# DredderGun/accbpg_and_fw

Measured on AMD Instinct MI355X. Metric: D-opt iters/sec (m=2048,n=32768), higher is better.
Workload: dtype f64; 1 GPU; D_opt_design(2048,32768) abpg_gain gamma=2 fp64, one independent instance per GPU; instances=1, instances_per_gpu=1, seeds=1..1, window=transient: iterations 5..161 from x0 = 1/n, linear_gram=False

## Files before the change

### accbpg_and_fw_amd/_lib.py

```python
from __future__ import annotations

import ctypes as C
import os

_HERE = os.path.dirname(os.path.abspath(__file__))
LIB_PATH = os.environ.get("ACCBPG_HIP_LIB") or os.path.join(_HERE, "lib", "libaccbpg_hip.so")

OK, ERR_ASSERT, ERR_NOT_PD, ERR_HIP, ERR_ARG = 0, 1, 2, 3, 4

_lib = None


class FwProbe(C.Structure):
    _fields_ = [("i", C.c_int64), ("j", C.c_int64), ("w_i", C.c_double), ("w_j", C.c_double),
                ("x_j", C.c_double), ("logdet_H", C.c_double), ("q_prev", C.c_double)]


class FwDivProbe(C.Structure):
    _fields_ = [("i", C.c_int64), ("w_i", C.c_double), ("x_i", C.c_double), ("sum_w", C.c_double),
                ("sum_w2", C.c_double), ("slope", C.c_double), ("div", C.c_double), ("min_x", C.c_double),
                ("sum_u2", C.c_double)]


class FwStep(C.Structure):
    _fields_ = [("i", C.c_int64), ("j", C.c_int64), ("w_i", C.c_double), ("w_j", C.c_double), ("x_j", C.c_double),
                ("q_prev", C.c_double), ("p", C.c_int64), ("xscale", C.c_double), ("xadd", C.c_double),
                ("hcoef", C.c_double), ("hdiv", C.c_double), ("kind", C.c_int32), ("status", C.c_int32)]


FW_RUN_MAX = 1024
FW_APPLIED, FW_STOPPED, FW_BAD_PIVOT, FW_NOT_RUN = 0, 1, 2, 3

_P = C.c_void_p
_SIGS = {
    "accbpg_abi_version": (C.c_int, []),
    "accbpg_last_error": (C.c_char_p, []),
    "accbpg_dopt_create": (C.c_int, [_P, C.c_int64, C.c_int64, C.c_int64, _P, C.POINTER(_P), C.c_int]),
    "accbpg_dopt_destroy": (C.c_int, [_P]),
    "accbpg_dopt_set_stream": (C.c_int, [_P, _P]),
    "accbpg_dopt_func_grad": (C.c_int, [_P, _P, C.c_int, C.POINTER(C.c_double), _P]),
    "accbpg_dopt_func_grad_begin": (C.c_int, [_P, _P, C.c_int, _P]),
    "accbpg_dopt_func_grad_end": (C.c_int, [_P, C.POINTER(C.c_double)]),
    "accbpg_dopt_eval_gap_ms": (C.c_int, [_P, _P, C.POINTER(C.c_double)]),
    "accbpg_dopt_value_reuse": (C.c_int, [_P, C.c_int]),
    "accbpg_dopt_value_reuse_stats": (C.c_int, [_P, C.POINTER(C.c_int64), C.POINTER(C.c_int64)]),
    "accbpg_dopt_value_peer": (C.c_int, [_P, _P]),
    "accbpg_dopt_gram": (C.c_int, [_P, _P, _P]),
    "accbpg_dopt_factor": (C.c_int, [_P, _P, C.POINTER(C.c_double)]),
    "accbpg_dopt_grad": (C.c_int, [_P, _P]),
    "accbpg_tri_pack": (C.c_int, [_P, C.c_int64, _P, _P]),
    "accbpg_tri_unpack": (C.c_int, [_P, C.c_int64, _P, _P]),
    "accbpg_vec_count_bad": (C.c_int, [_P, C.c_int64, _P, _P]),
    "accbpg_dopt_shard_bounds": (C.c_int, [C.c_int64, C.c_int, C.c_int, C.POINTER(C.c_int64), C.POINTER(C.c_int64)]),
    "accbpg_shard_unique_id": (C.c_int, [_P]),
    "accbpg_dopt_shard_create": (C.c_int, [_P, C.c_int64, C.c_int, C.c_int, _P, _P, C.POINTER(_P)]),
    "accbpg_dopt_shard_func_grad": (C.c_int, [_P, _P, C.c_int, C.POINTER(C.c_double), _P]),
    "accbpg_dopt_shard_destroy": (C.c_int, [_P]),
    "accbpg_debug_shard_pad": (C.c_int, [_P, C.c_int64]),
    "accbpg_dopt_gram_lincomb": (C.c_int, [_P, C.c_double, _P, C.c_double, _P, _P]),
    "accbpg_dopt_eval_gram": (C.c_int, [_P, _P, C.c_int, C.POINTER(C.c_double), _P]),
    "accbpg_dopt_batch_create": (C.c_int, [C.POINTER(_P), C.c_int, C.c_int64, C.c_int64, C.c_int64, _P, C.POINTER(_P)]),
    "accbpg_dopt_batch_destroy": (C.c_int, [_P]),
    "accbpg_dopt_batch_set_stream": (C.c_int, [_P, _P]),
    "accbpg_dopt_batch_size": (C.c_int, [_P]),
    "accbpg_dopt_batch_is_fused": (C.c_int, [_P]),
    "accbpg_dopt_batch_chunk": (C.c_int, [_P]),
    "accbpg_dopt_batch_instance": (_P, [_P, C.c_int]),
    "accbpg_dopt_batch_func_grad": (C.c_int, [_P, _P, C.c_int64, C.POINTER(C.c_int), C.c_int, C.POINTER(C.c_double), _P,
                                              C.c_int64, C.POINTER(C.c_int)]),
    "accbpg_dopt_batch_func_grad_begin": (C.c_int, [_P, _P, C.c_int64, C.POINTER(C.c_int), C.c_int, _P, C.c_int64]),
    "accbpg_dopt_batch_func_grad_end": (C.c_int, [_P, C.POINTER(C.c_double), C.POINTER(C.c_int)]),
    "accbpg_dopt_batch_burg_simplex_div_prox": (C.c_int, [_P, _P, _P, C.c_int64, C.POINTER(C.c_double), C.c_double, _P,
                                                          C.POINTER(C.c_int), C.POINTER(C.c_int), C.POINTER(C.c_int)]),
    "accbpg_dopt_batch_ls_terms": (C.c_int, [_P, _P, _P, _P, _P, _P, C.c_int64, C.POINTER(C.c_int), C.POINTER(C.c_double),
                                             C.POINTER(C.c_int)]),
    "accbpg_dopt_batch_axpby": (C.c_int, [_P, C.POINTER(C.c_double), _P, C.POINTER(C.c_double), _P, C.c_int64,
                                          C.POINTER(C.c_int), _P]),
    "accbpg_vec_workspace_doubles": (C.c_int64, [C.c_int64]),
    "accbpg_burg_simplex_div_prox": (C.c_int, [_P, _P, C.c_double, C.c_double, C.c_int64, _P, _P,
                                               C.POINTER(C.c_int), _P]),
    "accbpg_burg_divergence": (C.c_int, [_P, _P, C.c_int64, C.POINTER(C.c_double), _P, _P]),
    "accbpg_ls_terms": (C.c_int, [_P, _P, _P, _P, _P, C.c_int64, C.POINTER(C.c_double), _P, _P]),
    "accbpg_vec_axpby": (C.c_int, [C.c_double, _P, C.c_double, _P, C.c_int64, _P, _P]),
    "accbpg_vec_dot_diff": (C.c_int, [_P, _P, _P, C.c_int64, C.POINTER(C.c_double), _P, _P]),
    "accbpg_vec_min_sum": (C.c_int, [_P, C.c_int64, C.POINTER(C.c_double), _P, _P]),
    "accbpg_vec_div_scalar": (C.c_int, [_P, C.c_double, C.c_int64, _P, _P]),
    "accbpg_vec_vertex": (C.c_int, [C.c_int64, C.c_double, C.c_double, C.c_int64, _P, _P]),
    "accbpg_vec_argminmax": (C.c_int, [_P, C.c_int64, C.POINTER(C.c_int64), C.POINTER(C.c_double), _P, _P]),
    "accbpg_dopt_vt_times": (C.c_int, [_P, _P, _P]),
    "accbpg_dopt_get_column": (C.c_int, [_P, C.c_int64, _P]),
    "accbpg_dopt_kyinit": (C.c_int, [_P, _P, C.POINTER(C.c_int64), _P]),
    "accbpg_fw_init": (C.c_int, [_P, _P, C.POINTER(C.c_double)]),
    "accbpg_fw_probe_step": (C.c_int, [_P, C.c_int, C.c_int, C.POINTER(FwProbe)]),
    "accbpg_fw_logdet_flush": (C.c_int, [_P, C.POINTER(C.c_double)]),
    "accbpg_fw_logdet_ring": (C.c_int, [_P, C.c_int, C.c_int]),
    "accbpg_fw_logdet_pending": (C.c_int, [_P]),
    "accbpg_fw_update": (C.c_int, [_P, C.c_int64, C.c_double, C.c_double, C.c_double, C.c_double]),
    "accbpg_fw_get_state": (C.c_int, [_P, _P, _P, _P]),
    "accbpg_fw_div_probe_step": (C.c_int, [_P, C.c_double, C.c_double, C.POINTER(FwDivProbe)]),
    "accbpg_fw_div_apply": (C.c_int, [_P, C.c_int64, C.c_double, C.c_double, C.c_double, C.c_double, C.c_double]),
    "accbpg_fw_logdet_snapshot": (C.c_int, [_P, C.POINTER(C.c_double)]),
    "accbpg_fw_run": (C.c_int, [_P, C.c_int, C.c_double, C.c_int, C.POINTER(FwStep), C.POINTER(C.c_int)]),
    "accbpg_dopt_batch_fw_init": (C.c_int, [_P, _P, C.c_int64, C.POINTER(C.c_int), C.POINTER(C.c_double),
                                            C.POINTER(C.c_int)]),
    "accbpg_dopt_batch_fw_probe": (C.c_int, [_P, C.c_int, C.POINTER(C.c_int), C.POINTER(FwProbe)]),
    "accbpg_dopt_batch_fw_update": (C.c_int, [_P, C.POINTER(C.c_int), C.POINTER(C.c_int64), C.POINTER(C.c_double),
                                              C.POINTER(C.c_double), C.POINTER(C.c_double), C.POINTER(C.c_double)]),
    "accbpg_dopt_batch_fw_run": (C.c_int, [_P, C.c_int, C.POINTER(C.c_double), C.c_int, C.POINTER(C.c_int),
                                           C.POINTER(FwStep), C.POINTER(C.c_int)]),
    "accbpg_dopt_batch_kyinit": (C.c_int, [_P, _P, C.POINTER(C.c_int64), _P]),
    "accbpg_poisson_create": (C.c_int, [_P, C.c_int64, C.c_int64, C.c_int64, _P, _P, C.POINTER(_P)]),
    "accbpg_poisson_destroy": (C.c_int, [_P]),
    "accbpg_poisson_set_stream": (C.c_int, [_P, _P]),
    "accbpg_poisson_func_grad": (C.c_int, [_P, _P, C.c_int, C.POINTER(C.c_double), _P]),
    "accbpg_poisson_get_ax": (C.c_int, [_P, _P]),
    "accbpg_kldiv_create": (C.c_int, [_P, C.c_int64, C.c_int64, C.c_int64, _P, _P, C.POINTER(_P)]),
    "accbpg_kldiv_destroy": (C.c_int, [_P]),
    "accbpg_kldiv_set_stream": (C.c_int, [_P, _P]),
    "accbpg_kldiv_func_grad": (C.c_int, [_P, _P, C.c_int, C.POINTER(C.c_double), _P]),
    "accbpg_kldiv_get_ax": (C.c_int, [_P, _P]),
    "accbpg_shannon_div_prox": (C.c_int, [C.c_int, _P, _P, C.c_double, C.c_double, C.c_int64, _P, _P, _P]),
    "accbpg_shannon_ls_terms": (C.c_int, [_P, _P, _P, _P, _P, C.c_int64, C.c_double, C.POINTER(C.c_double), _P, _P]),
    "accbpg_shannon_divergence": (C.c_int, [_P, _P, C.c_int64, C.c_double, C.POINTER(C.c_double), _P, _P]),
    "accbpg_symnmf_create": (C.c_int, [_P, C.c_int64, C.c_int64, C.c_int64, C.c_double, _P, C.POINTER(_P)]),
    "accbpg_symnmf_destroy": (C.c_int, [_P]),
    "accbpg_symnmf_set_stream": (C.c_int, [_P, _P]),
    "accbpg_symnmf_func_grad": (C.c_int, [_P, _P, C.c_int, C.POINTER(C.c_double), _P]),
    "accbpg_symnmf_plan": (C.c_int, [_P, C.POINTER(C.c_int64)]),
    "accbpg_quartic_prox_stage": (C.c_int, [_P, _P, C.c_double, C.c_double, C.c_int, C.c_double, C.c_int64, _P,
                                            C.POINTER(C.c_double), _P, _P]),
    "accbpg_quartic_ls_terms": (C.c_int, [_P, _P, _P, _P, _P, C.c_int64, C.POINTER(C.c_double), _P, _P]),
    "accbpg_lmo_l2_ball": (C.c_int, [_P, C.c_int, _P, C.c_double, C.c_double, C.c_double, C.c_int64, _P,
                                     C.POINTER(C.c_double), _P, _P]),
    "accbpg_lmo_linf_ball": (C.c_int, [_P, C.c_int, _P, C.c_double, C.c_double, C.c_int64, _P, _P]),
    "accbpg_burg_reg_div_prox": (C.c_int, [C.c_int, _P, _P, C.c_double, C.c_double, C.c_int64, _P, _P]),
    "accbpg_vec_dot": (C.c_int, [_P, _P, C.c_int64, C.POINTER(C.c_double), _P, _P]),
    "accbpg_combine_ls_terms": (C.c_int, [C.c_int, C.c_double, _P, C.c_double, _P, C.c_double, _P, _P, C.c_int64, _P,
                                          C.POINTER(C.c_double), _P, _P]),
    "accbpg_burg_simplex_prox_acc": (C.c_int, [_P, C.c_double, _P, C.c_double, C.c_double, C.c_int64, _P, _P, _P,
                                               C.POINTER(C.c_int), _P]),
    "accbpg_lmo_l2_ball_pos": (C.c_int, [_P, _P, C.c_double, C.c_double, C.c_int64, _P, C.POINTER(C.c_double), _P, _P]),
    "accbpg_dopt_profile_enable": (C.c_int, [_P, C.c_int]),
    "accbpg_dopt_profile_read": (C.c_int, [_P, C.c_int, C.POINTER(C.c_double), C.POINTER(C.c_int64)]),
    "accbpg_dopt_profile_reset": (C.c_int, [_P]),
    "accbpg_debug_pipe_probe": (C.c_int, [C.c_int, C.c_int, C.POINTER(C.c_double), _P]),
    "accbpg_mfma_f64_peak": (C.c_int, [C.c_int, C.POINTER(C.c_double), _P]),
    "accbpg_dopt_factor_in_small_launches": (C.c_int, [_P, C.c_int]),
    "accbpg_debug_chol_variant": (C.c_int, [_P, C.c_int]),
    "accbpg_debug_plan_flags": (C.c_int, [C.c_int]),
    "accbpg_debug_gemm_loop": (C.c_int, [C.c_int]),
    "accbpg_debug_prox_variant": (C.c_int, [C.c_int]),
    "accbpg_debug_prox_state": (C.c_int, [C.POINTER(C.c_int)]),
    "accbpg_debug_chol_trace": (C.c_int, [_P, _P, C.c_int, C.POINTER(C.c_int64)]),
    "accbpg_debug_gram_variant": (C.c_int, [_P, _P, C.c_int, C.c_int, C.POINTER(C.c_double)]),
    "accbpg_debug_grad_variant": (C.c_int, [_P, _P, C.c_int, C.c_int, C.POINTER(C.c_double)]),
    "accbpg_test_gemm": (C.c_int, [_P, C.c_int64, _P, C.c_int64, _P, C.c_int64, C.c_int64, C.c_int64,
                                   C.c_int64, C.c_int, C.c_double, C.c_double, C.c_int, _P]),
}

EXPORTS = tuple(sorted(_SIGS))


def load():
    global _lib
    if _lib is not None:
        return _lib
    if not os.path.exists(LIB_PATH):
        raise ImportError(
            "accbpg_and_fw_amd: %s is missing -- build it with "
            "`make -C accbpg_and_fw_amd/csrc` or `python -c 'import __graft_entry__ as g; g.build()'`. "
            "There is no CPU fallback." % LIB_PATH)
    lib = C.CDLL(LIB_PATH)
    for name, (res, args) in _SIGS.items():
        fn = getattr(lib, name)
        fn.restype = res
        fn.argtypes = args
    _lib = lib
    return lib


def last_error():
    msg = load().accbpg_last_error()
    return msg.decode() if msg else ""


def check(rc, what, assert_msg=None):
    if rc == OK:
        return
    if rc == ERR_ASSERT:
        raise AssertionError(assert_msg or last_error() or what)
    if rc == ERR_NOT_PD:
        raise ValueError("HXHT is singular or not positive definite")
    if rc == ERR_ARG:
        raise ValueError("%s: bad argument (%s)" % (what, last_error()))
    raise RuntimeError("%s: HIP error: %s" % (what, last_error()))
```

### accbpg_and_fw_amd/algorithms.py

```python
from __future__ import annotations

import math
import time

import numpy as np
import torch

from .functions import (BurgEntropy, BurgEntropySimplex, ShannonEntropy, SquaredL2Norm, SumOf2nd4thPowers,
                        combine_ls_terms, from_dev, ls_terms, shannon_ls_terms, to_dev, vec_axpby, vec_div_scalar,
                        vec_dot_diff)
from .utils import get_random_float


def _divergences(h, g, x, y, z, z_prev):
    if isinstance(h, BurgEntropy):
        return ls_terms(g, x, y, z, z_prev)
    if isinstance(h, ShannonEntropy):
        return shannon_ls_terms(g, x, y, z, z_prev, h.delta)
    if isinstance(h, SumOf2nd4thPowers):
        return h.ls_terms(g, x, y, z, z_prev)
    lin = vec_dot_diff(g, x, y) if g is not None else 0.0
    return lin, h.divergence(x, y), (h.divergence(z, z_prev) if z is not None else 0.0)


def _lin(f):
    return bool(getattr(f, "_lin", False))


def _value(f, x, combo=None):
    return f.func_grad_combo(x, combo, 0) if _lin(f) else f(x)


def _value_begin(f, x, combo):
    if (not _lin(f)) and getattr(f, "_overlap", False) and not getattr(f, "_prof", False) \
            and isinstance(x, torch.Tensor) and x.is_cuda:
        if getattr(f, "_memo_on", False):
            hit = f._memo_get(x)
            if hit is not None:
                return ("value", hit)
        return ("ticket", f.value_async(x))
    return ("value", _value(f, x, combo))


def _can_speculate(f, x, checkdiv):
    return (not checkdiv) and (not _lin(f)) and getattr(f, "_spec", False) and getattr(f, "_overlap", False) \
        and not getattr(f, "_prof", False) and hasattr(f, "grad_async") and isinstance(x, torch.Tensor) and x.is_cuda


def _value_end(f, pending):
    kind, payload = pending
    return f.value_wait(payload) if kind == "ticket" else payload


def _stamp(f, pending, t_start, t_known):
    if pending[0] == "ticket":
        return time.time() - t_start - f.value_lead_seconds()
    return t_known - t_start


def _drain(gen):
    while True:
        try:
            next(gen)
        except StopIteration as stop:
            return stop.value


def BPG(f, h, L, x0, maxitrs, epsilon=1e-14, linesearch=True, ls_ratio=1.2,
        verbose=True, verbskip=1):
    return _drain(BPG_steps(f, h, L, x0, maxitrs, epsilon, linesearch, ls_ratio, verbose, verbskip))


def BPG_steps(f, h, L, x0, maxitrs, epsilon=1e-14, linesearch=True, ls_ratio=1.2,
              verbose=True, verbskip=1):
    if verbose:
        print("\nBPG_LS method for min_{x in C} F(x) = f(x) + Psi(x)")
        print("     k      F(x)         Lk       time")

    t_start = time.time()
    F = np.zeros(maxitrs)
    Ls = np.ones(maxitrs) * L
    T = np.zeros(maxitrs)

    x, as_numpy = to_dev(x0)
    x = x.clone()
    k = -1
    for k in range(maxitrs):
        fx, g = f.func_grad(x)
        F[k] = fx + h.extra_Psi(x)
        T[k] = time.time() - t_start

        if linesearch:
            L = L / ls_ratio
            trial = h.div_prox_map(x, g, L)
            while True:
                lin, dist, _ = _divergences(h, g, trial, x, None, None)
                if not (f(trial) > fx + lin + L * dist):
                    break
                L = L * ls_ratio
                trial = h.div_prox_map(x, g, L)
            x = trial
        else:
            x = h.div_prox_map(x, g, L)

        Ls[k] = L
        if verbose and k % verbskip == 0:
            print("{0:6d}  {1:10.3e}  {2:10.3e}  {3:6.1f}".format(k, F[k], L, T[k]))

        if k > 0 and abs(F[k] - F[k - 1]) < epsilon:
            break
        yield k

    return from_dev(x, as_numpy), F[0:k + 1], Ls[0:k + 1], T[0:k + 1]


def solve_theta(theta, gamma, gainratio=1):
    ckg = theta ** gamma / gainratio
    cta = theta
    eps = 1e-6 * theta
    phi = cta ** gamma - ckg * (1 - cta)
    while abs(phi) > eps:
        drv = gamma * cta ** (gamma - 1) + ckg
        cta = cta - phi / drv
        phi = cta ** gamma - ckg * (1 - cta)
    return cta


def ABPG(f, h, L, x0, gamma, maxitrs, epsilon=1e-14, theta_eq=False,
         restart=False, restart_rule='g', verbose=True, verbskip=1):
    return _drain(ABPG_steps(f, h, L, x0, gamma, maxitrs, epsilon, theta_eq, restart, restart_rule,
                             verbose, verbskip))


def ABPG_steps(f, h, L, x0, gamma, maxitrs, epsilon=1e-14, theta_eq=False,
               restart=False, restart_rule='g', verbose=True, verbskip=1):
    if verbose:
        print("\nABPG method for minimize_{x in C} F(x) = f(x) + Psi(x)")
        print("     k      F(x)       theta" +
              "        TSG       D(x+,y)     D(z+,z)     time")

    t_start = time.time()
    F = np.zeros(maxitrs)
    G = np.zeros(maxitrs)
    T = np.zeros(maxitrs)

    x, as_numpy = to_dev(x0)
    x = x.clone()
    z = x.clone()
    theta = 1.0
    kk = 0
    xcombo = None
    k = -1
    for k in range(maxitrs):
        pending = _value_begin(f, x, xcombo)
        t_known = time.time()

        z_prev, x_prev = z, x
        if theta_eq and kk > 0:
            theta = solve_theta(theta, gamma)
        else:
            theta = gamma / (kk + gamma)

        y = vec_axpby(1 - theta, x, theta, z_prev)
        if _lin(f):
            g = f.func_grad_combo(y, (1 - theta, x_prev, theta, z_prev), 1)
        else:
            g = f.gradient(y)
        F[k] = _value_end(f, pending) + h.extra_Psi(x_prev)
        T[k] = _stamp(f, pending, t_start, t_known)
        z = h.div_prox_map(z_prev, g, theta ** (gamma - 1) * L)
        x = vec_axpby(1 - theta, x, theta, z)
        if _lin(f):
            f.ensure_gram(z)
            xcombo = (1 - theta, x_prev, theta, z)

        _, dxy, dzz = _divergences(h, None, x, y, z, z_prev)
        Gdr = dxy / dzz / theta ** gamma

        G[k] = Gdr
        if verbose and k % verbskip == 0:
            print("{0:6d}  {1:10.3e}  {2:10.3e}  {3:10.3e}  {4:10.3e}  {5:10.3e}  {6:6.1f}".format(
                k, F[k], theta, Gdr, dxy, dzz, T[k]))

        kk += 1
        if restart and k > 0:
            if (restart_rule == 'f' and F[k] > F[k - 1]) or \
               (restart_rule == 'g' and vec_dot_diff(g, x, x_prev) > 0):
                theta = 1.0
                kk = 0
                z = x

        if dzz < epsilon:
            break
        yield k

    return from_dev(x, as_numpy), F[0:k + 1], G[0:k + 1], T[0:k + 1]


def ABPG_gain(f, h, L, x0, gamma, maxitrs, epsilon=1e-14, G0=1,
              ls_inc=1.2, ls_dec=1.2, theta_eq=True, checkdiv=False,
              restart=False, restart_rule='g', verbose=True, verbskip=1):
    return _drain(ABPG_gain_steps(f, h, L, x0, gamma, maxitrs, epsilon, G0, ls_inc, ls_dec, theta_eq,
                                  checkdiv, restart, restart_rule, verbose, verbskip))


def ABPG_gain_steps(f, h, L, x0, gamma, maxitrs, epsilon=1e-14, G0=1,
                    ls_inc=1.2, ls_dec=1.2, theta_eq=True, checkdiv=False,
                    restart=False, restart_rule='g', verbose=True, verbskip=1):
    if verbose:
        print("\nABPG_gain method for min_{x in C} F(x) = f(x) + Psi(x)")
        print("     k      F(x)       theta         Gk" +
              "         TSG       D(x+,y)     D(z+,z)      Gavg       time")

    t_start = time.time()
    F = np.zeros(maxitrs)
    Gain = np.ones(maxitrs) * G0
    Gdiv = np.zeros(maxitrs)
    Gavg = np.zeros(maxitrs)
    T = np.zeros(maxitrs)

    x, as_numpy = to_dev(x0)
    x = x.clone()
    z = x.clone()
    G = G0
    sumlogG = gamma * np.log(G)
    theta = 1.0
    kk = 0
    Gdr = 0.0
    xcombo = None
    retries_before = 0
    k = -1
    for k in range(maxitrs):
        pending = _value_begin(f, x, xcombo)
        t_known = time.time()

        z_prev, x_prev = z, x
        G_prev, theta_prev = G, theta
        G = G / ls_dec

        def theta_for(Gt):
            if kk == 0:
                return theta
            if theta_eq:
                return solve_theta(theta_prev, gamma, Gt / G_prev)
            alpha = Gt / G_prev
            return theta_prev * ((1 + alpha * (gamma - 1)) / (gamma * alpha + theta_prev))

        ahead = _can_speculate(f, x_prev, checkdiv)
        started = None
        failed = 0
        searching = True
        while searching:
            theta = theta_for(G)
            if started is not None:
                y, ticket = started
                started = None
                fy, g = f.grad_wait(ticket)
            else:
                y = vec_axpby(1 - theta, x_prev, theta, z_prev)
                if _lin(f):
                    fy, g = f.func_grad_combo(y, (1 - theta, x_prev, theta, z_prev), 2)
                else:
                    fy, g = f.func_grad(y)
            if pending is not None:
                F[k] = _value_end(f, pending) + h.extra_Psi(x_prev)
                T[k] = _stamp(f, pending, t_start, t_known)
                pending = None
            z = h.div_prox_map(z_prev, g, theta ** (gamma - 1) * G * L)
            x = vec_axpby(1 - theta, x_prev, theta, z)
            if _lin(f):
                f.ensure_gram(z)
                xcombo = (1 - theta, x_prev, theta, z)

            lin, dxy, dzz = _divergences(h, g, x, y, z, z_prev)
            if dzz < epsilon:
                break

            Gdr = dxy / dzz / theta ** gamma

            if checkdiv:
                searching = (Gdr > G)
            else:
                if ahead and failed < retries_before:
                    theta_next = theta_for(G * ls_inc)
                    y_next = vec_axpby(1 - theta_next, x_prev, theta_next, z_prev)
                    started = (y_next, f.grad_async(y_next))
                searching = (_value(f, x, xcombo) > fy + lin + theta ** gamma * G * L * dzz)

            if searching:
                G = G * ls_inc
                failed += 1
            elif started is not None:
                f.grad_drop(started[1])
                started = None
        retries_before = failed

        Gain[k] = G
        Gdiv[k] = Gdr
        sumlogG += np.log(G)
        Gavg[k] = np.exp(sumlogG / (gamma + k))
        if verbose and k % verbskip == 0:
            print("{0:6d}  {1:10.3e}  {2:10.3e}  {3:10.3e}  {4:10.3e}  {5:10.3e}  {6:10.3e}  {7:10.3e}  {8:6.1f}".format(
                k, F[k], theta, G, Gdr, dxy, dzz, Gavg[k], T[k]))

        kk += 1
        if restart:
            if (restart_rule == 'f' and F[k] > F[k - 1]) or \
               (restart_rule == 'g' and vec_dot_diff(g, x, x_prev) > 0):
                theta = 1.0
                kk = 0
                z = x

        if dzz < epsilon:
            break
        yield k

    return (from_dev(x, as_numpy), F[0:k + 1], Gain[0:k + 1], Gdiv[0:k + 1],
            Gavg[0:k + 1], T[0:k + 1])


def ABPG_expo(f, h, L, x0, gamma0, maxitrs, epsilon=1e-14, delta=0.2,
              theta_eq=True, checkdiv=False, Gmargin=10, restart=False,
              restart_rule='g', verbose=True, verbskip=1):
    return _drain(ABPG_expo_steps(f, h, L, x0, gamma0, maxitrs, epsilon, delta, theta_eq, checkdiv, Gmargin,
                                  restart, restart_rule, verbose, verbskip))


def ABPG_expo_steps(f, h, L, x0, gamma0, maxitrs, epsilon=1e-14, delta=0.2,
                    theta_eq=True, checkdiv=False, Gmargin=10, restart=False,
                    restart_rule='g', verbose=True, verbskip=1):
    if verbose:
        print("\nABPG_expo method for min_{x in C} F(x) = f(x) + Psi(x)")
        print("     k      F(x)       theta       gamma" +
              "        TSG       D(x+,y)     D(z+,z)     time")

    t_start = time.time()
    F = np.zeros(maxitrs)
    G = np.zeros(maxitrs)
    Gamma = np.ones(maxitrs) * gamma0
    T = np.zeros(maxitrs)

    gamma = gamma0
    x, as_numpy = to_dev(x0)
    x = x.clone()
    z = x.clone()
    theta = 1.0
    kk = 0
    k = -1
    for k in range(maxitrs):
        F[k] = f(x) + h.extra_Psi(x)
        T[k] = time.time() - t_start

        z_prev, x_prev = z, x
        if theta_eq and kk > 0:
            theta = solve_theta(theta, gamma)
        else:
            theta = gamma / (kk + gamma)

        y = vec_axpby(1 - theta, x_prev, theta, z_prev)
        fy, g = f.func_grad(y)

        trying = True
        while trying:
            z = h.div_prox_map(z_prev, g, theta ** (gamma - 1) * L)
            x = vec_axpby(1 - theta, x_prev, theta, z)
            lin, dxy, dzz = _divergences(h, g, x, y, z, z_prev)
            Gdr = dxy / dzz / theta ** gamma

            if checkdiv:
                trying = (dxy > Gmargin * (theta ** gamma) * dzz)
            else:
                trying = (f(x) > fy + lin + theta ** gamma * L * dzz)

            if trying and gamma > 1:
                gamma = max(gamma - delta, 1)
            else:
                trying = False

        G[k] = Gdr
        Gamma[k] = gamma
        if verbose and k % verbskip == 0:
            print("{0:6d}  {1:10.3e}  {2:10.3e}  {3:10.3e}  {4:10.3e}  {5:10.3e}  {6:10.3e}  {7:6.1f}".format(
                k, F[k], theta, gamma, Gdr, dxy, dzz, T[k]))

        kk += 1
        if restart:
            if (restart_rule == 'f' and F[k] > F[k - 1]) or \
               (restart_rule == 'g' and vec_dot_diff(g, x, x_prev) > 0):
                theta = 1.0
                kk = 0
                z = x

        if dzz < epsilon:
            break
        yield k

    return from_dev(x, as_numpy), F[0:k + 1], Gamma[0:k + 1], G[0:k + 1], T[0:k + 1]


def ABDA(f, h, L, x0, gamma, maxitrs, epsilon=1e-14, theta_eq=True,
         verbose=True, verbskip=1):
    return _drain(ABDA_steps(f, h, L, x0, gamma, maxitrs, epsilon, theta_eq, verbose, verbskip))


def ABDA_steps(f, h, L, x0, gamma, maxitrs, epsilon=1e-14, theta_eq=True,
               verbose=True, verbskip=1):
    if verbose:
        print("\nABDA method for min_{x in C} F(x) = f(x) + Psi(x)")
        print("     k      F(x)       theta" +
              "        TSG       D(x+,y)     D(z+,z)     time")

    t_start = time.time()
    F = np.zeros(maxitrs)
    G = np.zeros(maxitrs)
    T = np.zeros(maxitrs)

    x, as_numpy = to_dev(x0)
    x = x.clone()
    z = x.clone()
    theta = 1.0
    kk = 0
    gavg = torch.zeros_like(x)
    csum = 0
    k = -1
    for k in range(maxitrs):
        F[k] = f(x) + h.extra_Psi(x)
        T[k] = time.time() - t_start

        z_prev, x_prev = z, x
        if theta_eq and kk > 0:
            theta = solve_theta(theta, gamma)
        else:
            theta = gamma / (kk + gamma)

        y = vec_axpby(1 - theta, x_prev, theta, z_prev)
        g = f.gradient(y)
        wgt = theta ** (1 - gamma)
        gavg = vec_axpby(1.0, gavg, wgt, g)
        csum = csum + wgt
        z = h.prox_map(vec_div_scalar(gavg, csum), L / csum)
        x = vec_axpby(1 - theta, x_prev, theta, z)

        _, dxy, dzz = _divergences(h, None, x, y, z, z_prev)
        Gdr = dxy / dzz / theta ** gamma

        G[k] = Gdr
        if verbose and k % verbskip == 0:
            print("{0:6d}  {1:10.3e}  {2:10.3e}  {3:10.3e}  {4:10.3e}  {5:10.3e}  {6:6.1f}".format(
                k, F[k], theta, Gdr, dxy, dzz, T[k]))

        kk += 1
        if dzz < epsilon:
            break
        yield k

    return from_dev(x, as_numpy), F[0:k + 1], G[0:k + 1], T[0:k + 1]


FUSED_INEXACT = True


def _fusable(h):
    return FUSED_INEXACT and isinstance(h, (BurgEntropy, SquaredL2Norm))


def _combine(h, a, u, b, v, c, g=None, x=None):
    if _fusable(h):
        return combine_ls_terms(h, a, u, b, v, c, g, x)
    w = vec_axpby(a, u, b, v)
    if c != 1:
        w = vec_div_scalar(w, c)
    if x is None:
        return w, None, None
    lin, dist, _ = _divergences(h, g, w, x, None, None)
    return w, lin, dist


def _doubled(L):
    L = L * 2
    if L is None or not math.isfinite(L):
        raise ValueError("L cannot be None or infinity")
    return L


def AIBM(f, h, L, x0, gamma, maxitrs, epsilon=1e-14, verbose=True, noise=0, verbskip=1):
    return _drain(AIBM_steps(f, h, L, x0, gamma, maxitrs, epsilon, verbose, noise, verbskip))


def AIBM_steps(f, h, L, x0, gamma, maxitrs, epsilon=1e-14, verbose=True, noise=0, verbskip=1):
    if verbose:
        print("\nAIBM method for min_{x in C} F(x) = f(x) + Psi(x)")
        print("     k      F(x)       L       time")

    t_start = time.time()
    F = np.zeros(maxitrs)
    G = np.zeros(maxitrs)
    T = np.zeros(maxitrs)
    p = 2

    x0d, as_numpy = to_dev(x0)
    x = z = h.prox_map(torch.zeros(x0d.shape[0], dtype=torch.float64, device=x0d.device), 1)

    delta = get_random_float(noise)
    fx, g = f.func_grad(x, flag=2)
    y = h.prox_map(g, 1)
    lin, dist, _ = _divergences(h, g, y, x, None, None)
    fy = f(y)
    while True:
        alpha = 1 / L
        if fy <= fx + lin + L * dist + epsilon + delta:
            break
        L = _doubled(L)

    B = A = alpha
    xi_grad = vec_axpby(alpha, g, 0.0, g)

    F[0] = fx + h.extra_Psi(x)
    G[0] = L
    T[0] = time.time() - t_start

    acc_prox = FUSED_INEXACT and isinstance(h, BurgEntropySimplex)
    k = 0
    for k in range(1, maxitrs):
        L /= 2
        delta = get_random_float(noise)
        while True:
            alpha = (1 / L) * (1 + k / (2 * p)) ** ((p - 1) * (gamma - 1))
            B = (L * alpha ** gamma) ** (1 / (gamma - 1))
            x = vec_axpby(alpha / B, z, 1 - alpha / B, y)
            fx, grad_x = f.func_grad(x, flag=2)
            if acc_prox:
                xi_grad, z_k = h.prox_map_acc(xi_grad, alpha, grad_x)
            else:
                xi_grad = vec_axpby(1.0, xi_grad, alpha, grad_x)
                z_k = h.prox_map(xi_grad, 1)
            w, lin, dist = _combine(h, alpha / B, z_k, 1 - alpha / B, y, 1, grad_x, x)
            if f(w) <= fx + lin + L * dist + delta:
                break
            xi_grad = vec_axpby(1.0, xi_grad, -alpha, grad_x)
            L = _doubled(L)

        F[k] = fx + h.extra_Psi(x)
        T[k] = time.time() - t_start

        A += alpha
        y = vec_axpby(B / A, w, 1 - B / A, y)
        z = z_k

        if verbose and k % verbskip == 0:
            print("{0:6d}  {1:10.3e}  {2:10.3e}  {3:6.1f}".format(k, F[k], L, T[k]))

        if abs(F[k] - F[k - 1]) < 1e-9:
            break
        yield k

    return from_dev(x, as_numpy), F[0:k + 1], G[0:k + 1], T[0:k + 1]


def AdaptFGM(f, h, L, x0, maxitrs, epsilon=1e-14, verbose=True, noise=0, verbskip=1):
    return _drain(AdaptFGM_steps(f, h, L, x0, maxitrs, epsilon, verbose, noise, verbskip))


def AdaptFGM_steps(f, h, L, x0, maxitrs, epsilon=1e-14, verbose=True, noise=0, verbskip=1):
    if verbose:
        print("\nAdaptFGM method for min_{x in C} F(x) = f(x) + Psi(x)")
        print("     k      F(x)       L       time")

    t_start = time.time()
    F = np.zeros(maxitrs)
    G = np.zeros(maxitrs)
    T = np.zeros(maxitrs)

    x0d, as_numpy = to_dev(x0)
    x_k = u_k = torch.ones(x0d.shape, dtype=torch.float64, device=x0d.device)
    A_k = 0

    fxk, g = f.func_grad(x_k, flag=2)

    F[0] = fxk + h.extra_Psi(x_k)
    G[0] = L
    T[0] = time.time() - t_start

    k = 0
    for k in range(1, maxitrs):
        L /= 2
        delta = get_random_float(noise)
        while True:
            alpha = (1 + math.sqrt(1 + 4 * L * A_k)) / (2 * L)
            A = L * alpha ** 2
            y, _, _ = _combine(h, alpha, u_k, A_k, x_k, A)
# ... 89 lines not shown
```

### accbpg_and_fw_amd/csrc/capi.hip

```cpp
#include <stdarg.h>
#include <string.h>
#include <stdlib.h>
#include <algorithm>

#include "internal.h"
#include "reduce.hpp"

namespace accbpg {

static thread_local char g_err[512] = "";

void set_last_error(const char* fmt, ...) {
    va_list ap;
    va_start(ap, fmt);
    vsnprintf(g_err, sizeof(g_err), fmt, ap);
    va_end(ap);
}

void note_tiles_fallback(const char* where) {
    static bool said = false;
    if (said) return;
    said = true;
    fprintf(stderr, "libaccbpg_hip: %s: the one-launch Cholesky abandoned a wait (another process on this GPU, or fewer "
                    "workgroups resident than the occupancy query promised); this handle factors with one launch per block "
                    "column from now on\n", where);
}

static int read_status(accbpg_dopt* h) {
    ACC_HIP(hipMemcpyAsync(h->hpin, h->dscal, sizeof(double) * STATUS_DOUBLES, hipMemcpyDeviceToHost, h->stream));
    ACC_HIP(hipStreamSynchronize(h->stream));
    return ACCBPG_OK;
}

}

using namespace accbpg;

extern "C" int accbpg_abi_version(void) { return 3; }
extern "C" const char* accbpg_last_error(void) { return g_err; }

namespace accbpg {
int dopt_init(accbpg_dopt* h) {
    const int64_t m = h->m, n = h->n;
    ACC_HIP(hipGetDevice(&h->device));
    hipDeviceProp_t prop;
    ACC_HIP(hipGetDeviceProperties(&prop, h->device));
    h->num_cu = prop.multiProcessorCount;
    h->vec_ok = ((reinterpret_cast<uintptr_t>(h->V) & 15) == 0) && ((h->ldv & 1) == 0);
    h->big = (m >= 768) || (h->force_big && h->vec_ok && m >= 256 && (m % 256 == 0) && (n % 128 == 0));
    const size_t mm = sizeof(double) * (size_t)m * (size_t)m;
    ACC_HIP(hipMalloc(&h->Lbuf, mm));
    ACC_HIP(hipMalloc(&h->Wbuf, mm));
    ACC_HIP(hipMalloc(&h->Tbuf, mm));
    ACC_HIP(hipMemset(h->Lbuf, 0, mm));
    ACC_HIP(hipMemset(h->Wbuf, 0, mm));
    ACC_HIP(hipMemset(h->Tbuf, 0, mm));
    if (h->dscal_ext) {
        h->dscal = h->dscal_ext;
    } else {
        ACC_HIP(hipMalloc(&h->dscal, sizeof(double) * 24));
        ACC_HIP(hipMemset(h->dscal, 0, sizeof(double) * 24));
    }
    h->dflag = reinterpret_cast<int*>(h->dscal + 16);
    ACC_HIP(hipHostMalloc(&h->hpin, sizeof(double) * 32, hipHostMallocDefault));
    const int64_t vws = std::max<int64_t>(vec_ws_doubles(n), 64 * n);
    ACC_HIP(hipMalloc(&h->vws, sizeof(double) * (size_t)vws));
    ACC_HIP(hipEventCreate(&h->ev_done));
    return build_plans(h);
}
}

extern "C" int accbpg_dopt_create(const double* V_dev, int64_t m, int64_t n, int64_t ldv, void* stream,
                                  accbpg_dopt** out, int is_shard) {
    if (!V_dev || !out || m <= 0 || n <= 0 || ldv < n) {
        set_last_error("accbpg_dopt_create: bad arguments (m=%lld n=%lld ldv=%lld)", (long long)m, (long long)n,
                       (long long)ldv);
        return ACCBPG_ERR_ARG;
    }
    if (!is_shard && !(m < n)) {
        set_last_error("DOptimalObj: need m < n");
        return ACCBPG_ERR_ASSERT;
    }
    accbpg_dopt* h = new accbpg_dopt();
    h->V = V_dev; h->m = m; h->n = n; h->ldv = ldv; h->stream = (hipStream_t)stream;
    const int rc = dopt_init(h);
    if (rc != ACCBPG_OK) {
        accbpg_dopt_destroy(h);
        return rc;
    }
    *out = h;
    return ACCBPG_OK;
}

extern "C" int accbpg_dopt_destroy(accbpg_dopt* h) {
    if (!h) return ACCBPG_OK;
    for (accbpg_dopt* l : h->val_linked) l->val_peer = nullptr;
    if (h->val_peer) {
        auto& lk = h->val_peer->val_linked;
        lk.erase(std::remove(lk.begin(), lk.end(), h), lk.end());
    }
    hipFree(h->val_copy);
    hipFree(h->Vblk);
    hipFree(h->Lbuf); hipFree(h->Wbuf); hipFree(h->Tbuf); hipFree(h->slabs); hipFree(h->tiles); hipFree(h->wg_ranges); hipFree(h->gram_cstart); hipFree(h->gram_contrib);
    if (!h->dscal_ext) hipFree(h->dscal);
    hipFree(h->vws); hipFree(h->xbuf); hipFree(h->ops); hipFree(h->chol_op); hipFree(h->red); hipFree(h->Pbuf);
    hipFree(h->fw_x); hipFree(h->fw_w); hipFree(h->fw_H); hipFree(h->fw_hv);
    hipFree(h->chol_jobs); hipFree(h->chol_ready); hipFree(h->chol_aux); hipFree(h->chol_hand); hipFree(h->Gbuf);
    hipFree(h->fw_run);
    if (h->fw_steps_pin) hipHostFree(h->fw_steps_pin);
    hipFree(h->fw_div_ws);
    if (h->fw_div_pin) hipHostFree(h->fw_div_pin);
    if (h->hpin) hipHostFree(h->hpin);
    if (h->ev_done) hipEventDestroy(h->ev_done);
    for (auto& sl : h->fw_ring) {
        if (sl.stream) hipStreamSynchronize(sl.stream);
        if (sl.aux) accbpg_dopt_destroy(sl.aux);
        if (sl.stream) hipStreamDestroy(sl.stream);
        if (sl.ev_snap) hipEventDestroy(sl.ev_snap);
    }
    for (auto& p : h->prof)
        for (auto e : p.ev) hipEventDestroy(e);
    delete h;
    return ACCBPG_OK;
}

extern "C" int accbpg_dopt_set_stream(accbpg_dopt* h, void* stream) {
    if (!h) return ACCBPG_ERR_ARG;
    h->stream = (hipStream_t)stream;
    return ACCBPG_OK;
}

extern "C" int accbpg_dopt_gram(accbpg_dopt* h, const double* x_dev, double* gram_dev) {
    if (!h || !x_dev || !gram_dev) return ACCBPG_ERR_ARG;
    return launch_gram(h, x_dev, gram_dev);
}

extern "C" int accbpg_dopt_factor(accbpg_dopt* h, const double* gram_dev, double* f_host) {
    if (!h || !gram_dev) return ACCBPG_ERR_ARG;
    ACC_TRY(launch_cholesky(h, h->Lbuf, nullptr, nullptr, gram_dev));
    ACC_TRY(read_status(h));
    const int* fl = reinterpret_cast<const int*>(h->hpin + 16);
    if (fl[FLAG_ABORT]) {
        if (gram_dev == h->Lbuf) {
            set_last_error("accbpg_dopt_factor: in-place factorisation was abandoned; pass the Gram matrix in a buffer of its own");
            return ACCBPG_ERR_HIP;
        }
        h->chol_tiles_off = true;
        note_tiles_fallback("accbpg_dopt_factor");
        return accbpg_dopt_factor(h, gram_dev, f_host);
    }
    if (fl[FLAG_NOT_PD]) {
        set_last_error("HXHT is singular or not positive definite");
        return ACCBPG_ERR_NOT_PD;
    }
    if (f_host) *f_host = -h->hpin[0];
    return ACCBPG_OK;
}

extern "C" int accbpg_dopt_grad(accbpg_dopt* h, double* g_dev) {
    if (!h || !g_dev) return ACCBPG_ERR_ARG;
    ACC_TRY(launch_trtri(h));
    ACC_TRY(launch_colnorm(h, h->Wbuf, g_dev, -1.0));
    return ACCBPG_OK;
}

namespace accbpg {
__global__ __launch_bounds__(256) void value_compare_kernel(const unsigned long long* __restrict__ a,
                                                           const unsigned long long* __restrict__ b, int64_t n, int stamp,
                                                           int* __restrict__ word) {
    const int64_t stride = (int64_t)gridDim.x * 256;
    bool differ = false;
    for (int64_t i = (int64_t)blockIdx.x * 256 + threadIdx.x; i < n; i += stride) differ |= a[i] != b[i];
    if (differ) *word = stamp;
}

static void value_forget(accbpg_dopt* h) {
    h->val_valid = false;
    h->val_pending = false;
}

static int value_alloc(accbpg_dopt* h) {
    if (h->val_copy) return ACCBPG_OK;
    double* p = nullptr;
    ACC_HIP(hipMalloc(&p, sizeof(double) * ((size_t)h->n + 2)));
    if (hipMemsetAsync(p + h->n, 0, sizeof(double) * 2, h->stream) != hipSuccess) {
        hipFree(p);
        set_last_error("accbpg_dopt_func_grad: could not clear the compare word");
        return ACCBPG_ERR_HIP;
    }
    h->val_copy = p;
    return ACCBPG_OK;
}

static int value_matches(accbpg_dopt* h, const accbpg_dopt* rec, const double* x, bool* same) {
    ACC_TRY(value_alloc(h));
    int* word = reinterpret_cast<int*>(h->val_copy + h->n);
    int* pin = reinterpret_cast<int*>(h->hpin + 28);
    const int stamp = h->val_gen = h->val_gen % 1000000000 + 1;
    const int64_t nb = std::min<int64_t>((h->n + 255) / 256, 1024);
    value_compare_kernel<<<(unsigned)nb, 256, 0, h->stream>>>(reinterpret_cast<const unsigned long long*>(x),
                                                             reinterpret_cast<const unsigned long long*>(rec->val_copy),
                                                             h->n, stamp, word);
    ACC_HIP(hipGetLastError());
    ACC_HIP(hipMemcpyAsync(pin, word, sizeof(int), hipMemcpyDeviceToHost, h->stream));
    ACC_HIP(hipStreamSynchronize(h->stream));
    ++h->val_compares;
    *same = *pin != stamp;
    return ACCBPG_OK;
}

static int func_grad_begin(accbpg_dopt* h, const double* x_dev, int flag, double* g_dev, bool lookup) {
    h->last_x = x_dev; h->last_flag = flag; h->last_g = g_dev;
    h->val_pending = false;
    h->val_hit = false;
    const bool record = flag == 0 && h->val_reuse;
    if (record) {
        accbpg_dopt* const recs[2] = {h, h->val_peer};
        for (int r = 0; lookup && r < 2; ++r) {
            const accbpg_dopt* rec = recs[r];
            if (!rec || !rec->val_valid || rec->val_x != x_dev) continue;
            bool same = false;
            ACC_TRY(value_matches(h, rec, x_dev, &same));
            if (!same) continue;
            h->val_hit = true;
            h->val_answer = rec->val_f;
            ++h->val_answered;
            ACC_HIP(hipEventRecord(h->ev_done, h->stream));
            return ACCBPG_OK;
        }
        h->val_valid = false;
    }
    double* gram = chol_tiles_usable(h) ? h->Gbuf : h->Lbuf;
    ACC_TRY(launch_gram(h, x_dev, gram));
    if (record) ACC_TRY(value_alloc(h));
    ACC_TRY(launch_cholesky(h, h->Lbuf, flag != 0 ? h->Wbuf : nullptr, x_dev, gram, record ? h->val_copy : nullptr));
    if (flag != 0) {
        ACC_TRY(launch_trtri(h));
        ACC_TRY(launch_colnorm(h, h->Wbuf, g_dev, -1.0));
    }
    h->val_pending = record;
    ACC_HIP(hipMemcpyAsync(h->hpin, h->dscal, sizeof(double) * STATUS_DOUBLES, hipMemcpyDeviceToHost, h->stream));
    ACC_HIP(hipEventRecord(h->ev_done, h->stream));
    return ACCBPG_OK;
}

static int func_grad_end(accbpg_dopt* h, double* f_host) {
    if (h->val_hit) {
        h->val_hit = false;
        ACC_HIP(hipEventSynchronize(h->ev_done));
        if (f_host) *f_host = h->val_answer;
        return ACCBPG_OK;
    }
    ACC_HIP(hipStreamSynchronize(h->stream));
    const int* fl = reinterpret_cast<const int*>(h->hpin + 16);
    if (fl[FLAG_ABORT] && !h->chol_tiles_off) {
        h->chol_tiles_off = true;
        note_tiles_fallback("accbpg_dopt_func_grad");
        ACC_TRY(func_grad_begin(h, h->last_x, h->last_flag, h->last_g, false));
        return func_grad_end(h, f_host);
    }
    if (fl[FLAG_NEG_X]) {
        set_last_error("DOptimalObj: x needs to be nonnegative");
        return ACCBPG_ERR_ASSERT;
    }
    if (fl[FLAG_NOT_PD]) {
        set_last_error("HXHT is singular or not positive definite");
        return ACCBPG_ERR_NOT_PD;
    }
    if (h->val_pending) {
        h->val_pending = false;
        h->val_x = h->last_x;
        h->val_f = -h->hpin[0];
        h->val_valid = true;
    }
    if (f_host) *f_host = -h->hpin[0];
    return ACCBPG_OK;
}
}

extern "C" int accbpg_dopt_func_grad_begin(accbpg_dopt* h, const double* x_dev, int flag, double* g_dev) {
    if (!h || !x_dev || flag < 0 || flag > 2) return ACCBPG_ERR_ARG;
    if (flag != 0 && !g_dev) return ACCBPG_ERR_ARG;
    const int rc = func_grad_begin(h, x_dev, flag, g_dev, true);
    if (rc != ACCBPG_OK) {
        value_forget(h);
        h->val_hit = false;
    }
    return rc;
}

extern "C" int accbpg_dopt_eval_gap_ms(accbpg_dopt* first, accbpg_dopt* second, double* ms_host) {
    if (!first || !second || !ms_host) return ACCBPG_ERR_ARG;
    float ms = 0.f;
    const hipError_t e = hipEventElapsedTime(&ms, first->ev_done, second->ev_done);
    if (e != hipSuccess) {
        (void)hipGetLastError();
        float back = 0.f;
        if (hipEventElapsedTime(&back, second->ev_done, first->ev_done) != hipSuccess) {
            (void)hipGetLastError();
            set_last_error("accbpg_dopt_eval_gap_ms: no completed evaluation on one of the handles");
            return ACCBPG_ERR_ARG;
        }
        ms = -back;
    }
    *ms_host = (double)ms;
    return ACCBPG_OK;
}

extern "C" int accbpg_dopt_func_grad_end(accbpg_dopt* h, double* f_host) {
    if (!h) return ACCBPG_ERR_ARG;
    const int rc = func_grad_end(h, f_host);
    if (rc != ACCBPG_OK) value_forget(h);
    return rc;
}

extern "C" int accbpg_dopt_func_grad(accbpg_dopt* h, const double* x_dev, int flag, double* f_host, double* g_dev) {
    ACC_TRY(accbpg_dopt_func_grad_begin(h, x_dev, flag, g_dev));
    return accbpg_dopt_func_grad_end(h, f_host);
}

extern "C" int accbpg_dopt_value_reuse(accbpg_dopt* h, int on) {
    if (!h) return ACCBPG_ERR_ARG;
    h->val_reuse = on != 0;
    value_forget(h);
    return ACCBPG_OK;
}

extern "C" int accbpg_dopt_value_reuse_stats(accbpg_dopt* h, int64_t* compares_host, int64_t* answered_host) {
    if (!h) return ACCBPG_ERR_ARG;
    if (compares_host) *compares_host = h->val_compares;
    if (answered_host) *answered_host = h->val_answered;
    return ACCBPG_OK;
}

extern "C" int accbpg_dopt_value_peer(accbpg_dopt* h, accbpg_dopt* peer) {
    if (!h || peer == h) return ACCBPG_ERR_ARG;
    if (peer && (peer->V != h->V || peer->m != h->m || peer->n != h->n || peer->ldv != h->ldv)) {
        set_last_error("accbpg_dopt_value_peer: the two handles are not over the same matrix");
        return ACCBPG_ERR_ARG;
    }
    if (h->val_peer) {
        auto& lk = h->val_peer->val_linked;
        lk.erase(std::remove(lk.begin(), lk.end(), h), lk.end());
    }
    h->val_peer = peer;
    if (peer) peer->val_linked.push_back(h);
    return ACCBPG_OK;
}

namespace accbpg {
__global__ void lincomb_kernel(double a, const double* __restrict__ G1, double b, const double* __restrict__ G2,
                               int64_t total, double* __restrict__ out) {
    const int64_t stride = (int64_t)gridDim.x * blockDim.x * 2;
    for (int64_t e = 2 * ((int64_t)blockIdx.x * blockDim.x + threadIdx.x); e < total; e += stride) {
        if (e + 1 < total) {
            const double2 u = *reinterpret_cast<const double2*>(G1 + e);
            const double2 v = *reinterpret_cast<const double2*>(G2 + e);
            double2 r;
            r.x = a * u.x + b * v.x;
            r.y = a * u.y + b * v.y;
            *reinterpret_cast<double2*>(out + e) = r;
        } else {
            out[e] = a * G1[e] + b * G2[e];
        }
    }
}
}

namespace accbpg {
__global__ __launch_bounds__(256) void tri_pack_kernel(const double* __restrict__ G, int64_t m, double* __restrict__ packed,
                                                      int unpack, double* __restrict__ Gout) {
    const int64_t r = blockIdx.x;
    const int64_t base = r * (r + 1) / 2;
    for (int64_t c = threadIdx.x; c <= r; c += 256) {
        if (unpack) Gout[r * m + c] = packed[base + c];
        else packed[base + c] = G[r * m + c];
    }
}
__global__ __launch_bounds__(1024) void count_bad_kernel(const double* __restrict__ x, int64_t n, double* __restrict__ count) {
    __shared__ int sh[16];
    int c = 0;
    for (int64_t i = threadIdx.x; i < n; i += 1024) c += !(x[i] >= 0.0);
    c = wave_sum(c);
    if ((threadIdx.x & 63) == 0) sh[threadIdx.x >> 6] = c;
    __syncthreads();
    if (threadIdx.x == 0) {
        int t = 0;
        for (int i = 0; i < 16; ++i) t += sh[i];
        count[0] = (double)t;
    }
}
}

extern "C" int accbpg_tri_pack(const double* G_dev, int64_t m, double* packed_dev, void* stream) {
    if (!G_dev || !packed_dev || m <= 0) return ACCBPG_ERR_ARG;
    tri_pack_kernel<<<(unsigned)m, 256, 0, (hipStream_t)stream>>>(G_dev, m, packed_dev, 0, nullptr);
    ACC_HIP(hipGetLastError());
    return ACCBPG_OK;
}

extern "C" int accbpg_tri_unpack(const double* packed_dev, int64_t m, double* G_dev, void* stream) {
    if (!G_dev || !packed_dev || m <= 0) return ACCBPG_ERR_ARG;
    tri_pack_kernel<<<(unsigned)m, 256, 0, (hipStream_t)stream>>>(nullptr, m, const_cast<double*>(packed_dev), 1, G_dev);
    ACC_HIP(hipGetLastError());
    return ACCBPG_OK;
}

extern "C" int accbpg_vec_count_bad(const double* x_dev, int64_t n, double* count_dev, void* stream) {
    if (!x_dev || !count_dev || n <= 0) return ACCBPG_ERR_ARG;
    count_bad_kernel<<<1, 1024, 0, (hipStream_t)stream>>>(x_dev, n, count_dev);
    ACC_HIP(hipGetLastError());
    return ACCBPG_OK;
}

extern "C" int accbpg_dopt_gram_lincomb(accbpg_dopt* h, double a, const double* G1_dev, double b,
                                        const double* G2_dev, double* out_dev) {
    if (!h || !G1_dev || !G2_dev || !out_dev) return ACCBPG_ERR_ARG;
    const int64_t total = h->m * h->m;
    lincomb_kernel<<<2048, 256, 0, h->stream>>>(a, G1_dev, b, G2_dev, total, out_dev);
    ACC_HIP(hipGetLastError());
    return ACCBPG_OK;
}

extern "C" int accbpg_dopt_eval_gram(accbpg_dopt* h, const double* gram_dev, int flag, double* f_host, double* g_dev) {
    if (!h || !gram_dev || flag < 0 || flag > 2) return ACCBPG_ERR_ARG;
    if (flag != 0 && !g_dev) return ACCBPG_ERR_ARG;
    ACC_TRY(launch_cholesky(h, h->Lbuf, flag != 0 ? h->Wbuf : nullptr, nullptr, gram_dev));
    if (flag != 0) {
        ACC_TRY(launch_trtri(h));
        ACC_TRY(launch_colnorm(h, h->Wbuf, g_dev, -1.0));
    }
    ACC_TRY(read_status(h));
    const int* fl = reinterpret_cast<const int*>(h->hpin + 16);
    if (fl[FLAG_ABORT]) {
        if (gram_dev == h->Lbuf) {
            set_last_error("accbpg_dopt_eval_gram: in-place factorisation was abandoned; pass the Gram matrix in a buffer of its own");
            return ACCBPG_ERR_HIP;
        }
        h->chol_tiles_off = true;
        note_tiles_fallback("accbpg_dopt_eval_gram");
        return accbpg_dopt_eval_gram(h, gram_dev, flag, f_host, g_dev);
    }
    if (fl[FLAG_NOT_PD]) {
        set_last_error("HXHT is singular or not positive definite");
        return ACCBPG_ERR_NOT_PD;
    }
    if (f_host) *f_host = -h->hpin[0];
    return ACCBPG_OK;
}

extern "C" int accbpg_dopt_profile_enable(accbpg_dopt* h, int enable) {
    if (!h) return ACCBPG_ERR_ARG;
    h->prof_on = enable != 0;
    return ACCBPG_OK;
}

extern "C" int accbpg_dopt_profile_reset(accbpg_dopt* h) {
    if (!h) return ACCBPG_ERR_ARG;
    ACC_HIP(hipStreamSynchronize(h->stream));
    for (auto& p : h->prof) { p.used = 0; p.total_ms = 0.0; p.launches = 0; }
    return ACCBPG_OK;
}

extern "C" int accbpg_dopt_profile_read(accbpg_dopt* h, int which, double* total_ms_host, int64_t* launches_host) {
    if (!h || which < 0 || which >= PROF_COUNT) return ACCBPG_ERR_ARG;
    ACC_HIP(hipStreamSynchronize(h->stream));
    ProfSlot& p = h->prof[which];
    double tot = 0.0;
    for (size_t i = 0; i + 1 < p.used; i += 2) {
        float ms = 0.f;
        ACC_HIP(hipEventElapsedTime(&ms, p.ev[i], p.ev[i + 1]));
        tot += ms;
    }
    p.total_ms = tot;
    if (total_ms_host) *total_ms_host = tot;
    if (launches_host) *launches_host = p.launches;
    return ACCBPG_OK;
}

extern "C" int accbpg_mfma_f64_peak(int iters, double* tflops_host, void* stream) {
    if (!tflops_host || iters <= 0) return ACCBPG_ERR_ARG;
    return mfma_peak(iters, tflops_host, (hipStream_t)stream);
}

extern "C" int accbpg_debug_pipe_probe(int iters, int mode, double* ms_host, void* stream) {
    if (!ms_host || iters <= 0) return ACCBPG_ERR_ARG;
    return pipe_probe(iters, mode, ms_host, (hipStream_t)stream);
}

extern "C" int accbpg_test_gemm(const double* A_dev, int64_t lda, const double* B_dev, int64_t ldb, double* C_dev,
                                int64_t ldc, int64_t M, int64_t N, int64_t K, int b_kmajor, double alpha,
                                double beta, int config, void* stream) {
    if (!A_dev || !B_dev || !C_dev || M <= 0 || N <= 0 || K <= 0) return ACCBPG_ERR_ARG;
    return launch_test_gemm(A_dev, lda, B_dev, ldb, C_dev, ldc, M, N, K, b_kmajor, alpha, beta, config,
                            (hipStream_t)stream);
}

extern "C" int accbpg_dopt_factor_in_small_launches(accbpg_dopt* h, int on) {
    if (!h || on < 0 || on > 2) return ACCBPG_ERR_ARG;
    const int64_t T = (h->m + NB - 1) / NB;
    value_forget(h);
    h->chol_tiles_off = on == 1 || (on == 2 && T * (T + 1) / 2 >= h->num_cu);
    return ACCBPG_OK;
}

extern "C" int accbpg_debug_plan_flags(int flags) {
    set_plan_flags(flags);
    return ACCBPG_OK;
}

extern "C" int accbpg_debug_gemm_loop(int variant) {
    return set_gemm_loop(variant);
}

extern "C" int accbpg_debug_chol_variant(accbpg_dopt* h, int bits) {
    if (!h) return ACCBPG_ERR_ARG;
    value_forget(h);
    h->chol_dbg = bits & 63;
    h->chol_tiles_off = (bits & 64) != 0;
    if (bits & 2048) h->chol_tiles_off = true;
    h->chol_stall_test = (bits & 128) ? 1 : 0;
    h->chol_spin_limit = (bits & 128) ? 200000 : 20000000;
    h->kern_variant = (bits >> 30) & 3;
    if (bits & 256) h->use_glds = false;
    if (bits & 512) h->use_glds = true;
    if (bits & 2048) {
        h->chol_two_level_T = (bits >> 12) & 0xfff;
        if ((bits >> 24) & 0x3f) h->chol_nk = (bits >> 24) & 0x3f;
    }
    return ACCBPG_OK;
}

extern "C" int accbpg_debug_chol_trace(accbpg_dopt* h, const double* gram_dev, int with_inverse, int64_t* stamps_host) {
    if (!h || !gram_dev || !stamps_host) return ACCBPG_ERR_ARG;
    if (!chol_tiles_usable(h)) {
        set_last_error("accbpg_debug_chol_trace: the one-launch Cholesky is not in use for this handle");
        return ACCBPG_ERR_ARG;
    }
    const int T = (int)((h->m + NB - 1) / NB);
    const size_t bytes = sizeof(long long) * (size_t)T * 32;
    if (!h->chol_trace) ACC_HIP(hipMalloc(&h->chol_trace, bytes));
    ACC_HIP(hipMemsetAsync(h->chol_trace, 0, bytes, h->stream));
    int rc = launch_cholesky(h, h->Lbuf, with_inverse ? h->Wbuf : nullptr, nullptr, gram_dev);
    if (rc == ACCBPG_OK) {
        hipError_t e = hipMemcpyAsync(stamps_host, h->chol_trace, bytes, hipMemcpyDeviceToHost, h->stream);
        if (e == hipSuccess) e = hipStreamSynchronize(h->stream);
        if (e != hipSuccess) rc = ACCBPG_ERR_HIP;
    }
    hipFree(h->chol_trace);
    h->chol_trace = nullptr;
    return rc;
}

extern "C" int accbpg_debug_gram_variant(accbpg_dopt* h, const double* x_dev, int variant, int iters, double* ms_host) {
    if (!h || !x_dev || !ms_host || iters <= 0) return ACCBPG_ERR_ARG;
    value_forget(h);
    return debug_gram_variant(h, x_dev, variant, iters, ms_host);
}

extern "C" int accbpg_debug_grad_variant(accbpg_dopt* h, double* g_dev, int variant, int iters, double* ms_host) {
    if (!h || !g_dev || !ms_host || iters <= 0) return ACCBPG_ERR_ARG;
    value_forget(h);
    return debug_grad_variant(h, g_dev, variant, iters, ms_host);
}
```

### accbpg_and_fw_amd/csrc/dopt_kernels.hip

```cpp
#include <atomic>
#include <mutex>
#include <unordered_map>
#include <type_traits>

#include "internal.h"
#include "mfma_tile.hpp"

namespace accbpg {

struct GramSeg {
    int64_t row0, col0, kb, ke;
    bool dual, whole;
};
constexpr int GRAM_RMAX = 4;
template <class T>
__device__ __forceinline__ GramSeg gram_segment(const TileRC* __restrict__ tiles, int64_t kiters, int64_t it,
                                                int64_t it1) {
    const int e = (int)(it / kiters);
    const int64_t off = it - (int64_t)e * kiters;
    const TileRC tr = tiles[e];
    GramSeg g;
    if (tr.d1 < 0) {
        g.row0 = (int64_t)tr.rb * T::BM; g.col0 = (int64_t)tr.cb * T::BN;
        g.kb = off; g.ke = min(kiters, off + (it1 - it));
// ... 2255 lines not shown
                    it += ue - off;
                    ++seg;
                }
            }
            nslot = std::max(nslot, seg);
        }
        h->gram_nslot = nslot;
        std::vector<int32_t> cstart(cl.size() + 1, 0), contrib;
        for (size_t i = 0; i < cl.size(); ++i) {
            std::sort(cl[i].begin(), cl[i].end(), [](const Contrib& a, const Contrib& b) { return a.kb < b.kb; });
            for (const Contrib& c : cl[i]) { contrib.push_back(c.w); contrib.push_back(c.slot); }
            cstart[i + 1] = (int32_t)(contrib.size() / 2);
        }
        if (contrib.empty()) contrib.push_back(0);
        ACC_HIP(hipMalloc(&h->wg_ranges, sizeof(int64_t) * ranges.size()));
        ACC_HIP(hipMemcpy(h->wg_ranges, ranges.data(), sizeof(int64_t) * ranges.size(), hipMemcpyHostToDevice));
        ACC_HIP(hipMalloc(&h->gram_cstart, sizeof(int32_t) * cstart.size()));
        ACC_HIP(hipMemcpy(h->gram_cstart, cstart.data(), sizeof(int32_t) * cstart.size(), hipMemcpyHostToDevice));
        ACC_HIP(hipMalloc(&h->gram_contrib, sizeof(int32_t) * contrib.size()));
        ACC_HIP(hipMemcpy(h->gram_contrib, contrib.data(), sizeof(int32_t) * contrib.size(), hipMemcpyHostToDevice));
    }
    ACC_HIP(hipMalloc(&h->slabs, sizeof(double) * (size_t)grid * h->gram_nslot * BM * BN));

    const int T = (int)((m + NB - 1) / NB);
    h->ops_host.clear();
    h->merge_stages.clear();
    std::vector<RedOp> reds;
    constexpr int64_t KP = 256, KSPLIT_MIN = 512;
    ACC_HIP(hipMalloc(&h->Pbuf, sizeof(double) * (size_t)m * m));
    for (int span = 1; span < T; span *= 2) {
        std::vector<GemmOp> first, second;
        for (int g = 0; g + span < T; g += 2 * span) {
            const int64_t r1 = (int64_t)g * NB;
            const int64_t s1 = (int64_t)span * NB;
            const int64_t r2 = r1 + s1;
            const int64_t s2 = std::min<int64_t>((int64_t)span * NB, m - r2);
            GemmOp a{};
            a.A = h->Lbuf + r2 * m + r1; a.lda = m;
            a.B = h->Wbuf + r1 * m + r1; a.ldb = m;
            a.C = h->Tbuf + r2 * m + r1; a.ldc = m;
            a.M = (int)s2; a.N = (int)s1; a.K = (int)s1; a.lower_only = 0; a.alpha = 1.0; a.beta = 0.0;
            a.tri = 1;
            GemmOp b{};
            b.A = h->Wbuf + r2 * m + r2; b.lda = m;
            b.B = h->Tbuf + r2 * m + r1; b.ldb = m;
            b.C = h->Wbuf + r2 * m + r1; b.ldc = m;
            b.M = (int)s2; b.N = (int)s1; b.K = (int)s2; b.lower_only = 0; b.alpha = -1.0; b.beta = 0.0;
            b.tri = 2;
            first.push_back(a);
            second.push_back(b);
        }
        for (std::vector<GemmOp>* list : {&first, &second}) {
            bool split = !list->empty();
            size_t pdoubles = 0;
            for (const GemmOp& o : *list) {
                split = split && o.K >= KSPLIT_MIN && o.K % KP == 0 && (o.N % 2 == 0) && (o.ldc % 2 == 0);
                pdoubles += (size_t)(o.K / KP) * o.M * o.N;
            }
            split = split && pdoubles <= (size_t)m * m;
            accbpg_dopt::MergeStage st{0, (int)h->ops_host.size(), 0, 0, 0};
            accbpg_dopt::MergeStage rs{1, (int)reds.size(), 0, 0, 0};
            double* pb = h->Pbuf;
            for (const GemmOp& o : *list) {
                st.maxm = std::max(st.maxm, o.M); st.maxn = std::max(st.maxn, o.N);
                if (!split) { h->ops_host.push_back(o); continue; }
                const int ns = (int)(o.K / KP);
                RedOp r{o.C, pb, o.ldc, o.M, o.N, ns, 0};
                reds.push_back(r);
                rs.maxm = std::max(rs.maxm, o.M * o.N);
                for (int p = 0; p < ns; ++p) {
                    GemmOp q = o;
                    q.A = o.A + p * KP;
                    q.B = o.B + p * KP * o.ldb;
                    q.K = (int)KP;
                    q.koff = (int)(p * KP);
                    q.C = pb; q.ldc = o.N;
                    pb += (size_t)o.M * o.N;
                    h->ops_host.push_back(q);
                }
            }
            st.end = (int)h->ops_host.size();
            h->merge_stages.push_back(st);
            if (split) { rs.end = (int)reds.size(); h->merge_stages.push_back(rs); }
        }
    }
    if (!h->ops_host.empty()) {
        ACC_HIP(hipMalloc(&h->ops, sizeof(GemmOp) * h->ops_host.size()));
        ACC_HIP(hipMemcpy(h->ops, h->ops_host.data(), sizeof(GemmOp) * h->ops_host.size(), hipMemcpyHostToDevice));
    }
    h->red_host = reds;
    if (!reds.empty()) {
        ACC_HIP(hipMalloc(&h->red, sizeof(RedOp) * reds.size()));
        ACC_HIP(hipMemcpy(h->red, reds.data(), sizeof(RedOp) * reds.size(), hipMemcpyHostToDevice));
    }
    ACC_HIP(hipMalloc(&h->chol_op, sizeof(GemmOp) * (size_t)(T + 1)));

    if (T <= CT_TMAX) {
        std::vector<CholJob> jobs;
        for (int d2 = 0; d2 < T; ++d2) jobs.push_back(CholJob{d2, d2});
        for (int j = 0; j < T; ++j)
            for (int i = j + 2; i < T; ++i) jobs.push_back(CholJob{i, j});
        ACC_TRY(set_lds(chol_tiles_kernel, CT_LDS_BYTES));
        int per_cu = 0;
        ACC_HIP(hipOccupancyMaxActiveBlocksPerMultiprocessor(&per_cu, chol_tiles_kernel, NTHREADS, CT_LDS_BYTES));
        h->chol_tiles_grid = (int)jobs.size();
        h->chol_slots = std::min(per_cu, 2) * h->num_cu;
        h->chol_tiles_ok = per_cu >= 1 && (int64_t)jobs.size() <= (int64_t)h->chol_slots;
        if (h->chol_tiles_ok) {
            ACC_HIP(hipMalloc(&h->chol_jobs, sizeof(CholJob) * jobs.size()));
            ACC_HIP(hipMemcpy(h->chol_jobs, jobs.data(), sizeof(CholJob) * jobs.size(), hipMemcpyHostToDevice));
            ACC_HIP(hipMalloc(&h->chol_ready, sizeof(int) * (size_t)(T * T + 5 * T)));
            ACC_HIP(hipMemset(h->chol_ready, 0, sizeof(int) * (size_t)(T * T + 5 * T)));
            ACC_HIP(hipMalloc(&h->chol_hand, sizeof(double) * (size_t)T * NB * NB));
            ACC_HIP(hipMalloc(&h->chol_aux, sizeof(double) * (size_t)T * CT_AUX));
            ACC_HIP(hipMalloc(&h->Gbuf, sizeof(double) * (size_t)m * m));
            ACC_HIP(hipMemset(h->Gbuf, 0, sizeof(double) * (size_t)m * m));
        }
    }

    ACC_TRY(set_lds(gram_streamk_kernel<TileBig<false, true>>, TileBig<false>::LDS_BYTES));
    ACC_TRY(set_lds(gram_streamk_kernel<TileBig<false, false>>, TileBig<false>::LDS_BYTES));
    ACC_TRY(set_lds(gram_streamk_kernel<TileSmall<false, true>>, TileSmall<false>::LDS_BYTES));
    ACC_TRY(set_lds(gram_streamk_kernel<TileSmall<false, false>>, TileSmall<false>::LDS_BYTES));
    ACC_TRY(set_lds(colnorm_kernel<TileBig<true, true>>, TileBig<true>::LDS_BYTES));
    ACC_TRY(set_lds(colnorm_kernel<TileBig<true, false>>, TileBig<true>::LDS_BYTES));
    ACC_TRY(set_lds(colnorm_kernel<TileSmall<true, true>>, TileSmall<true>::LDS_BYTES));
    ACC_TRY(set_lds(colnorm_kernel<TileSmall<true, false>>, TileSmall<true>::LDS_BYTES));
    ACC_TRY(set_lds_gemm_ops());
    ACC_TRY(set_lds(chol_step_kernel, CHOL_LDS_BYTES));
    ACC_TRY(set_lds(chol_syrk_kernel, SYRK_LDS_BYTES));
    ACC_TRY(set_lds(gemm_big_kernel<TileBig<true>>, TileBig<true>::LDS_BYTES));
    ACC_TRY(set_lds(gemm_big_kernel<TileBig<false>>, TileBig<false>::LDS_BYTES));
    return ACCBPG_OK;
}

template <class T>
static int gram_launch_t(accbpg_dopt* h, const double* x, double* gram) {
    if constexpr (!T::EDGE && T::BM == 256) {
        if (h->use_glds || h->has_duals) {
            const int64_t nc = h->gram_chunks > 1 ? h->gram_nc : h->n;
            for (int c = 0; c < h->gram_chunks; ++c) {
                const double* Vc = h->Vblk ? h->Vblk + (int64_t)c * h->m * nc : h->V + (int64_t)c * nc;
                const int64_t ldc = h->Vblk ? nc : h->ldv;
                const double* xc = x + (int64_t)c * nc;
                const double beta = c == 0 ? 0.0 : 1.0;
                const int all_slabs = h->gram_chunks > 1 ? 1 : 0;
                prof_begin(h, PROF_GRAM);
#define ACC_GRAM_ARGS Vc, ldc, h->m, nc, xc, h->tiles, h->wg_ranges, h->kiters, h->gram_nslot, h->slabs, gram, h->m, all_slabs
                if (h->kern_variant == 1)
                    ACC_LAUNCH_LDS((gram_streamk_glds_kernel<T, GRAM_GV ^ 128>), h->gram_grid, NTHREADS, T::G_LDS_BYTES, h->stream, ACC_GRAM_ARGS);
                else if (h->kern_variant == 3)
                    ACC_LAUNCH_LDS((gram_streamk_glds_kernel<T, 0>), h->gram_grid, NTHREADS, T::G_LDS_BYTES, h->stream, ACC_GRAM_ARGS);
                else if (h->kern_variant == 2)
                    ACC_LAUNCH_LDS((gram_streamk_glds_kernel<T, (GRAM_GV ^ 128) | 256>), h->gram_grid, NTHREADS, T::G_LDS_BYTES, h->stream, ACC_GRAM_ARGS);
                else
                    ACC_LAUNCH_LDS((gram_streamk_glds_kernel<T, GRAM_GV>), h->gram_grid, NTHREADS, T::G_LDS_BYTES, h->stream, ACC_GRAM_ARGS);
#undef ACC_GRAM_ARGS
                ACC_HIP(hipGetLastError());
                prof_end(h, PROF_GRAM);
                prof_begin(h, PROF_GRAMFIX);
                gram_fixup_kernel<T><<<h->ntiles * 2 * T::MI * FIX_PJ, NTHREADS, 0, h->stream>>>(
                    h->tiles, h->gram_cstart, h->gram_contrib, h->gram_nslot, h->slabs, gram, h->m, h->m, beta);
                prof_end(h, PROF_GRAMFIX);
            }
            return ACCBPG_OK;
        }
    }
    prof_begin(h, PROF_GRAM);
    gram_streamk_kernel<T><<<h->gram_grid, NTHREADS, T::LDS_BYTES, h->stream>>>(
        h->V, h->ldv, h->m, h->n, x, h->tiles, h->wg_ranges, h->kiters, h->gram_nslot, h->slabs, gram, h->m, h->vec_ok);
    ACC_HIP(hipGetLastError());
    prof_end(h, PROF_GRAM);
    prof_begin(h, PROF_GRAMFIX);
    gram_fixup_kernel<T><<<h->ntiles * 2 * T::MI * FIX_PJ, NTHREADS, 0, h->stream>>>(h->tiles, h->gram_cstart, h->gram_contrib, h->gram_nslot,
                                                                h->slabs, gram, h->m, h->m, 0.0);
    prof_end(h, PROF_GRAMFIX);
    return ACCBPG_OK;
}

int debug_gram_variant(accbpg_dopt* h, const double* x, int var, int iters, double* ms_out) {
    using T = TileBig<false, false>;
    if (!h->big) return ACCBPG_ERR_ARG;
    if (h->has_duals && var < 10) return ACCBPG_ERR_ARG;
    hipEvent_t a, b;
    ACC_HIP(hipEventCreate(&a));
    ACC_HIP(hipEventCreate(&b));
    auto launch = [&]() -> int {
#define ACC_LAUNCH_VAR(VV)                                                                                       \
    gram_streamk_kernel<T, VV><<<h->gram_grid, NTHREADS, T::LDS_BYTES, h->stream>>>(                             \
        h->V, h->ldv, h->m, h->n, x, h->tiles, h->wg_ranges, h->kiters, h->gram_nslot, h->slabs, h->Tbuf, h->m, h->vec_ok)
#define ACC_LAUNCH_G(GG)                                                                                         \
    ACC_LAUNCH_LDS((gram_streamk_glds_kernel<T, GG>), h->gram_grid, NTHREADS, T::G_LDS_BYTES, h->stream,          \
        h->V, h->ldv, h->m, h->n, x, h->tiles, h->wg_ranges, h->kiters, h->gram_nslot, h->slabs, h->Tbuf, h->m, 0)
        switch (var) {
            case 10: ACC_LAUNCH_G(0); break;
            case 11: ACC_LAUNCH_G(1); break;
            case 12: ACC_LAUNCH_G(2); break;
            case 13: ACC_LAUNCH_G(3); break;
            case 14: ACC_LAUNCH_G(4); break;
            case 15: ACC_LAUNCH_G(8); break;
            case 16: ACC_LAUNCH_G(7); break;
            case 17: ACC_LAUNCH_G(16); break;
            case 18: ACC_LAUNCH_G(32); break;
            case 19: ACC_LAUNCH_G(96); break;
            case 20: ACC_LAUNCH_G(97); break;
            case 21: ACC_LAUNCH_G(98); break;
            case 22: ACC_LAUNCH_G(100); break;
            case 23: ACC_LAUNCH_G(104); break;
            case 24: ACC_LAUNCH_G(103); break;
            case 25: ACC_LAUNCH_G(102); break;
            case 26: ACC_LAUNCH_G(101); break;
            case 27: ACC_LAUNCH_G(99); break;
            case 28: ACC_LAUNCH_G(224); break;
            case 29: ACC_LAUNCH_G(352); break;
            case 0: ACC_LAUNCH_VAR(0); break;
            case 1: ACC_LAUNCH_VAR(1); break;
            case 2: ACC_LAUNCH_VAR(2); break;
            case 3: ACC_LAUNCH_VAR(3); break;
            default: ACC_LAUNCH_VAR(4); break;
        }
#undef ACC_LAUNCH_VAR
        return ACCBPG_OK;
    };
    ACC_TRY(set_lds(gram_streamk_kernel<T, 1>, T::LDS_BYTES));
    ACC_TRY(set_lds(gram_streamk_kernel<T, 2>, T::LDS_BYTES));
    ACC_TRY(set_lds(gram_streamk_kernel<T, 3>, T::LDS_BYTES));
    ACC_TRY(set_lds(gram_streamk_kernel<T, 4>, T::LDS_BYTES));
    ACC_TRY(launch());
    ACC_HIP(hipEventRecord(a, h->stream));
    for (int i = 0; i < iters; ++i) ACC_TRY(launch());
    ACC_HIP(hipEventRecord(b, h->stream));
    ACC_HIP(hipEventSynchronize(b));
    float ms = 0.f;
    ACC_HIP(hipEventElapsedTime(&ms, a, b));
    *ms_out = ms / iters;
    hipEventDestroy(a);
    hipEventDestroy(b);
    ACC_HIP(hipGetLastError());
    return ACCBPG_OK;
}

int launch_gram(accbpg_dopt* h, const double* x, double* gram) {
    bool xal = (reinterpret_cast<uintptr_t>(x) & 15) == 0;
    if (!xal && (h->has_duals || h->gram_chunks > 1)) {
        if (!h->xbuf) ACC_HIP(hipMalloc(&h->xbuf, sizeof(double) * (size_t)h->n));
        ACC_TRY(device_copy(h->xbuf, x, (size_t)h->n, h->stream));
        x = h->xbuf;
        xal = true;
    }
    if (h->big) {
        const bool interior = h->vec_ok && xal && (h->m % 256 == 0) && (h->n % BK == 0);
        if (interior) ACC_TRY((gram_launch_t<TileBig<false, false>>(h, x, gram)));
        else ACC_TRY((gram_launch_t<TileBig<false, true>>(h, x, gram)));
    } else {
        const bool interior = h->vec_ok && xal && (h->m % 64 == 0) && (h->n % BK == 0);
        if (interior) ACC_TRY((gram_launch_t<TileSmall<false, false>>(h, x, gram)));
        else ACC_TRY((gram_launch_t<TileSmall<false, true>>(h, x, gram)));
    }
    ACC_HIP(hipGetLastError());
    return ACCBPG_OK;
}

__global__ __launch_bounds__(256) void copy_kernel(double* __restrict__ dst, const double* __restrict__ src, size_t n) {
    const size_t stride = (size_t)gridDim.x * 256;
    for (size_t i = (size_t)blockIdx.x * 256 + threadIdx.x; i < n; i += stride) dst[i] = src[i];
}
int device_copy(double* dst, const double* src, size_t ndoubles, hipStream_t s) {
    if (ndoubles == 0 || dst == src) return ACCBPG_OK;
    size_t nb = (ndoubles + 255) / 256;
    if (nb > 4096) nb = 4096;
    copy_kernel<<<(unsigned)nb, 256, 0, s>>>(dst, src, ndoubles);
    ACC_HIP(hipGetLastError());
    return ACCBPG_OK;
}

int launch_gemm_ops(const GemmOp* ops_dev, int nops, int maxM, int maxN, bool b_kmajor, hipStream_t s) {
    if (nops <= 0 || maxM <= 0 || maxN <= 0) return ACCBPG_OK;
    dim3 grid((maxN + 63) / 64, (maxM + 63) / 64, nops);
    return with_gemm_loop([&](auto loop) -> int {
        constexpr int LOOP = decltype(loop)::value;
        if (b_kmajor)
            gemm_ops_kernel<TileSmall<true>, LOOP><<<grid, NTHREADS, TileSmall<true>::LDS_BYTES, s>>>(ops_dev);
        else
            gemm_ops_kernel<TileSmall<false>, LOOP><<<grid, NTHREADS, TileSmall<false>::LDS_BYTES, s>>>(ops_dev);
        ACC_HIP(hipGetLastError());
        return ACCBPG_OK;
    });
}

static std::mutex g_tiles_mu;
constexpr int TILES_RING = 16;
struct TilesRing {
    hipEvent_t ev[TILES_RING] = {};
    hipStream_t stream[TILES_RING] = {};
    int grid[TILES_RING] = {};
    long long issued = 0;
};
static TilesRing g_tiles[64];

bool chol_tiles_usable(const accbpg_dopt* h) {
    return h->chol_tiles_ok && !h->chol_tiles_off && (h->chol_dbg & 63) == 0;
}

static int launch_chol_tiles(accbpg_dopt* h, const double* src, double* A, double* Winv) {
    const int64_t m = h->m;
    const int T = (int)((m + NB - 1) / NB);
    CholInst ci;
    ci.src = src; ci.L = A; ci.Ldiag = h->Tbuf; ci.Winv = Winv; ci.logdet = h->dscal; ci.flags = h->dflag;
    ci.ready = h->chol_ready; ci.aux = h->chol_aux; ci.hand = h->chol_hand; ci.trace = h->chol_trace;
    const int dev = (h->device >= 0 && h->device < 64) ? h->device : 0;
    std::lock_guard<std::mutex> lk(g_tiles_mu);
    TilesRing& ring = g_tiles[dev];
    {
        int gmax = h->chol_tiles_grid;
        for (int i = 0; i < TILES_RING; ++i) gmax = std::max(gmax, ring.grid[i]);
        int together = std::max(1, h->chol_slots) / std::max(1, gmax);
        if (together > TILES_RING - 1) together = TILES_RING - 1;
        if (together < 1) together = 1;
        for (long long back = together; back <= TILES_RING && back <= ring.issued; ++back) {
            const int slot = (int)((ring.issued - back) % TILES_RING);
            if (ring.ev[slot] && ring.stream[slot] != h->stream) ACC_HIP(hipStreamWaitEvent(h->stream, ring.ev[slot], 0));
        }
    }
    chol_tiles_kernel<<<dim3(h->chol_tiles_grid, 1), NTHREADS, CT_LDS_BYTES, h->stream>>>(
        ci, nullptr, reinterpret_cast<const CholJob*>(h->chol_jobs), m, m, T, h->chol_spin_limit, h->chol_stall_test, BatchAct{});
    ACC_HIP(hipGetLastError());
    {
        const int slot = (int)(ring.issued % TILES_RING);
        if (!ring.ev[slot]) ACC_HIP(hipEventCreateWithFlags(&ring.ev[slot], hipEventDisableTiming));
        ACC_HIP(hipEventRecord(ring.ev[slot], h->stream));
        ring.stream[slot] = h->stream;
        ring.grid[slot] = h->chol_tiles_grid;
        ++ring.issued;
    }
    return ACCBPG_OK;
}

int launch_cholesky(accbpg_dopt* h, double* A, double* Winv, const double* xcheck, const double* src, double* xkeep) {
    const int64_t m = h->m;
    const int T = (int)((m + NB - 1) / NB);
    if (src == nullptr) src = A;
    const bool tiles = chol_tiles_usable(h);
    prof_begin(h, PROF_CHOL);
    zero_scalars_kernel<<<1, (xcheck || tiles) ? 512 : 64, 0, h->stream>>>(h->dscal, h->dflag, xcheck, h->n,
                                                                         tiles ? h->chol_ready : nullptr, tiles ? T * T + 5 * T : 0,
                                                                         xcheck ? xkeep : nullptr);
    if (tiles) {
        ACC_TRY(launch_chol_tiles(h, src, A, Winv));
        h->diag_inv_ready = (Winv != nullptr);
        prof_end(h, PROF_CHOL);
        return ACCBPG_OK;
    }
    if (src != A) ACC_TRY(device_copy(A, src, (size_t)m * m, h->stream));
    const int nkp = (T >= h->chol_two_level_T) ? h->chol_nk : T;
    for (int k0 = 0; k0 < T; k0 += nkp) {
        const int kend = std::min(k0 + nkp, T) - 1;
        for (int kc = k0; kc <= kend; ++kc) {
            const int pend = (kc > k0) ? 1 : 0;
            const int npanel = T - kc;
            const int R = T - (kc + 1);
            int nupd = 0;
            if (pend) nupd = (kend >= T - 1) ? R * (R + 1) / 2 : R * (kend - kc);
            chol_step_kernel<<<npanel + nupd, NTHREADS, CHOL_LDS_BYTES, h->stream>>>(
                A, m, m, kc, pend, kend, T, h->dscal, h->dflag, h->chol_dbg, Winv, h->Tbuf);
        }
        const int Rr = T - (kend + 1);
        if (Rr > 0)
            chol_syrk_kernel<<<Rr * (Rr + 1) / 2, NTHREADS, SYRK_LDS_BYTES, h->stream>>>(A, m, m, k0, kend - k0 + 1, T);
    }
    h->diag_inv_ready = (Winv != nullptr);
    prof_end(h, PROF_CHOL);
    ACC_HIP(hipGetLastError());
    return ACCBPG_OK;
}

int launch_trtri(accbpg_dopt* h) {
    const int64_t m = h->m;
    const int T = (int)((m + NB - 1) / NB);
    prof_begin(h, PROF_TRTRI);
    if (!h->diag_inv_ready) trtri_diag_kernel<<<T, 64, 0, h->stream>>>(h->Tbuf, m, h->Wbuf, m, m);
    h->diag_inv_ready = false;
    for (const accbpg_dopt::MergeStage& st : h->merge_stages) {
        if (st.kind == 0) {
            ACC_TRY(launch_gemm_ops(h->ops + st.begin, st.end - st.begin, st.maxm, st.maxn, true, h->stream));
        } else {
            int gx = (int)std::min<int64_t>(1024, ((int64_t)st.maxm / 2 + 255) / 256);
            gemm_reduce_kernel<<<dim3(gx, st.end - st.begin), 256, 0, h->stream>>>(h->red + st.begin);
        }
    }
    prof_end(h, PROF_TRTRI);
    ACC_HIP(hipGetLastError());
    return ACCBPG_OK;
}

template <class T>
static void colnorm_launch_t(accbpg_dopt* h, const double* W, double* out, double sign, bool vw) {
    const int grid = (int)((h->n + T::BN - 1) / T::BN);
    colnorm_kernel<T><<<grid, NTHREADS, T::LDS_BYTES, h->stream>>>(W, h->m, h->V, h->ldv, h->m, h->n, out, sign, vw,
                                                                  h->vec_ok);
}

int launch_colnorm(accbpg_dopt* h, const double* W, double* out, double sign) {
    prof_begin(h, PROF_GRAD);
    const bool vw = ((reinterpret_cast<uintptr_t>(W) & 15) == 0) && ((h->m & 1) == 0);
    if (h->big) {
        const bool interior = vw && h->vec_ok && (h->m % 256 == 0) && (h->n % 128 == 0);
        if (interior && h->use_glds) {
            using T = TileBig<true, false>;
            const int grid = (int)(h->n / T::BN), lds = T::G_LDS_BYTES + 4 * T::BN * 8;
            if (h->kern_variant == 1)
                ACC_LAUNCH_LDS((colnorm_glds_kernel<T, COLNORM_CV ^ 256>), grid, NTHREADS, lds, h->stream, W, h->m, h->V, h->ldv, h->m, h->n, out, sign);
            else if (h->kern_variant == 2)
                ACC_LAUNCH_LDS((colnorm_glds_kernel<T, 96>), grid, NTHREADS, lds, h->stream, W, h->m, h->V, h->ldv, h->m, h->n, out, sign);
            else if (h->kern_variant == 3)
                ACC_LAUNCH_LDS((colnorm_glds_kernel<T, COLNORM_CV | 512>), grid, NTHREADS, lds, h->stream, W, h->m, h->V, h->ldv, h->m, h->n, out, sign);
            else
                ACC_LAUNCH_LDS((colnorm_glds_kernel<T, COLNORM_CV>), grid, NTHREADS, lds, h->stream, W, h->m, h->V, h->ldv, h->m, h->n, out, sign);
        } else if (interior) colnorm_launch_t<TileBig<true, false>>(h, W, out, sign, vw);
        else colnorm_launch_t<TileBig<true, true>>(h, W, out, sign, vw);
    } else {
        const bool interior = vw && h->vec_ok && (h->m % 64 == 0) && (h->n % 64 == 0);
        if (interior) colnorm_launch_t<TileSmall<true, false>>(h, W, out, sign, vw);
        else colnorm_launch_t<TileSmall<true, true>>(h, W, out, sign, vw);
    }
    prof_end(h, PROF_GRAD);
    ACC_HIP(hipGetLastError());
    return ACCBPG_OK;
}

int launch_gram_batch(accbpg_dopt_batch* b, const BatchAct& act, const double* xbase, int64_t ldx) {
    using T = TileBig<false, false>;
    accbpg_dopt* h0 = b->inst[0];
    static bool lds_set = false;
    if (!lds_set) {
        ACC_TRY(set_lds(gram_streamk_glds_batch_kernel<T>, T::G_LDS_BYTES));
        lds_set = true;
    }
    prof_begin(h0, PROF_GRAM);
    gram_streamk_glds_batch_kernel<T><<<dim3(h0->gram_grid, act.n), NTHREADS, T::G_LDS_BYTES, b->stream>>>(
        b->table, act, h0->ldv, h0->m, h0->n, xbase, ldx, h0->tiles, h0->wg_ranges, h0->kiters, h0->gram_nslot, h0->m);
    prof_end(h0, PROF_GRAM);
    prof_begin(h0, PROF_GRAMFIX);
    gram_fixup_batch_kernel<T><<<dim3(h0->ntiles * 2 * T::MI * FIX_PJ, act.n), NTHREADS, 0, b->stream>>>(
        b->table, act, h0->tiles, h0->gram_cstart, h0->gram_contrib, h0->gram_nslot, h0->m, h0->m);
    prof_end(h0, PROF_GRAMFIX);
    ACC_HIP(hipGetLastError());
    return ACCBPG_OK;
}

int launch_cholesky_batch(accbpg_dopt_batch* b, const BatchAct& act, bool with_inverse, const double* xbase, int64_t ldx) {
    accbpg_dopt* h0 = b->inst[0];
    const int64_t m = h0->m;
    const int T = (int)((m + NB - 1) / NB);
    prof_begin(h0, PROF_CHOL);
    zero_scalars_batch_kernel<<<act.n, 512, 0, b->stream>>>(b->table, act, xbase, ldx, h0->n, T * T + 5 * T);
    const int dev = (b->device >= 0 && b->device < 64) ? b->device : 0;
    const int grid_all = h0->chol_tiles_grid * act.n;
    std::lock_guard<std::mutex> lk(g_tiles_mu);
    TilesRing& ring = g_tiles[dev];
    {
        int gmax = grid_all;
        for (int i = 0; i < TILES_RING; ++i) gmax = std::max(gmax, ring.grid[i]);
        int together = std::max(1, h0->chol_slots) / std::max(1, gmax);
        if (together > TILES_RING - 1) together = TILES_RING - 1;
        if (together < 1) together = 1;
        for (long long back = together; back <= TILES_RING && back <= ring.issued; ++back) {
            const int slot = (int)((ring.issued - back) % TILES_RING);
            if (ring.ev[slot] && ring.stream[slot] != b->stream) ACC_HIP(hipStreamWaitEvent(b->stream, ring.ev[slot], 0));
        }
    }
    chol_tiles_kernel<<<dim3(h0->chol_tiles_grid, act.n), NTHREADS, CT_LDS_BYTES, b->stream>>>(
        CholInst{}, b->chol_table[with_inverse ? 1 : 0], reinterpret_cast<const CholJob*>(h0->chol_jobs), m, m, T,
        h0->chol_spin_limit, 0, act);
    prof_end(h0, PROF_CHOL);
    ACC_HIP(hipGetLastError());
    {
        const int slot = (int)(ring.issued % TILES_RING);
        if (!ring.ev[slot]) ACC_HIP(hipEventCreateWithFlags(&ring.ev[slot], hipEventDisableTiming));
        ACC_HIP(hipEventRecord(ring.ev[slot], b->stream));
        ring.stream[slot] = b->stream;
        ring.grid[slot] = grid_all;
        ++ring.issued;
    }
    return ACCBPG_OK;
}

int launch_trtri_batch(accbpg_dopt_batch* b, const BatchAct& act) {
    accbpg_dopt* h0 = b->inst[0];
    prof_begin(h0, PROF_TRTRI);
    for (const accbpg_dopt::MergeStage& st : h0->merge_stages) {
        const int count = st.end - st.begin;
        if (count <= 0) continue;
        if (st.kind == 0) {
            dim3 grid((st.maxn + 63) / 64, (st.maxm + 63) / 64, count * act.n);
            ACC_TRY(with_gemm_loop([&](auto loop) -> int {
                gemm_ops_batch_kernel<TileSmall<true>, decltype(loop)::value><<<grid, NTHREADS, TileSmall<true>::LDS_BYTES, b->stream>>>(
                    b->ops_all, b->ops_per_inst, st.begin, count, act);
                return ACCBPG_OK;
            }));
        } else {
            int gx = (int)std::min<int64_t>(1024, ((int64_t)st.maxm / 2 + 255) / 256);
            gemm_reduce_batch_kernel<<<dim3(gx, count * act.n), 256, 0, b->stream>>>(b->red_all, b->red_per_inst, st.begin, count, act);
        }
    }
    prof_end(h0, PROF_TRTRI);
    ACC_HIP(hipGetLastError());
    return ACCBPG_OK;
}

int debug_grad_variant(accbpg_dopt* h, double* out, int var, int iters, double* ms_out) {
    using T = TileBig<true, false>;
    const bool vw = ((reinterpret_cast<uintptr_t>(h->Wbuf) & 15) == 0) && ((h->m & 1) == 0);
    if (!h->big || !h->use_glds || !vw || !h->vec_ok || h->m % 256 != 0 || h->n % 128 != 0) return ACCBPG_ERR_ARG;
    const int grid = (int)(h->n / T::BN), lds = T::G_LDS_BYTES + 4 * T::BN * 8;
    if (var != 0 && var != 3 && (var < 10 || var > 13)) return ACCBPG_ERR_ARG;
    hipEvent_t a, b;
    ACC_HIP(hipEventCreate(&a));
    if (hipEventCreate(&b) != hipSuccess) {
        hipEventDestroy(a);
        return ACCBPG_ERR_HIP;
    }
    auto launch = [&]() -> int {
#define ACC_LAUNCH_C(CC) \
    ACC_LAUNCH_LDS((colnorm_glds_kernel<T, CC>), grid, NTHREADS, lds, h->stream, h->Wbuf, h->m, h->V, h->ldv, h->m, h->n, out, -1.0)
        switch (var) {
            case 0: ACC_LAUNCH_C(COLNORM_CV); break;
            case 3: ACC_LAUNCH_C(COLNORM_CV | 512); break;
            case 10: ACC_LAUNCH_C(COLNORM_CV | 512 | 1); break;
            case 11: ACC_LAUNCH_C(COLNORM_CV | 512 | 2); break;
            case 12: ACC_LAUNCH_C(COLNORM_CV | 512 | 4); break;
            case 13: ACC_LAUNCH_C(COLNORM_CV | 512 | 8); break;
            default: return ACCBPG_ERR_ARG;
        }
#undef ACC_LAUNCH_C
        return ACCBPG_OK;
    };
    auto timed = [&]() -> int {
        ACC_TRY(launch());
        ACC_HIP(hipEventRecord(a, h->stream));
        for (int i = 0; i < iters; ++i) ACC_TRY(launch());
        ACC_HIP(hipEventRecord(b, h->stream));
        ACC_HIP(hipEventSynchronize(b));
        float ms = 0.f;
        ACC_HIP(hipEventElapsedTime(&ms, a, b));
        *ms_out = ms / iters;
        ACC_HIP(hipGetLastError());
        return ACCBPG_OK;
    };
    const int rc = timed();
    hipEventDestroy(a);
    hipEventDestroy(b);
    return rc;
}

int launch_colnorm_batch(accbpg_dopt_batch* b, const BatchAct& act, double* gbase, int64_t ldg, double sign) {
    using T = TileBig<true, false>;
    accbpg_dopt* h0 = b->inst[0];
    static bool lds_set = false;
    if (!lds_set) {
        ACC_TRY(set_lds(colnorm_glds_batch_kernel<T>, T::G_LDS_BYTES + 4 * T::BN * 8));
        lds_set = true;
    }
    prof_begin(h0, PROF_GRAD);
    colnorm_glds_batch_kernel<T><<<dim3((unsigned)(h0->n / T::BN), act.n), NTHREADS, T::G_LDS_BYTES + 4 * T::BN * 8, b->stream>>>(
        b->table, act, h0->m, h0->ldv, h0->m, h0->n, gbase, ldg, sign);
    prof_end(h0, PROF_GRAD);
    ACC_HIP(hipGetLastError());
    return ACCBPG_OK;
}

int launch_test_gemm(const double* A, int64_t lda, const double* B, int64_t ldb, double* C, int64_t ldc, int64_t M,
                     int64_t N, int64_t K, int b_kmajor, double alpha, double beta, int config, hipStream_t s) {
    GemmOp op{};
    op.A = A; op.B = B; op.C = C; op.lda = lda; op.ldb = ldb; op.ldc = ldc;
    op.M = (int)M; op.N = (int)N; op.K = (int)K; op.lower_only = 0; op.alpha = alpha; op.beta = beta;
    if (config == 1) {
        if (b_kmajor) {
            using T = TileBig<true>;
            ACC_TRY(set_lds(gemm_big_kernel<T>, T::LDS_BYTES));
            dim3 grid((unsigned)((N + T::BN - 1) / T::BN), (unsigned)((M + T::BM - 1) / T::BM));
            gemm_big_kernel<T><<<grid, NTHREADS, T::LDS_BYTES, s>>>(op);
        } else {
            using T = TileBig<false>;
            ACC_TRY(set_lds(gemm_big_kernel<T>, T::LDS_BYTES));
            dim3 grid((unsigned)((N + T::BN - 1) / T::BN), (unsigned)((M + T::BM - 1) / T::BM));
            gemm_big_kernel<T><<<grid, NTHREADS, T::LDS_BYTES, s>>>(op);
        }
    } else {
        GemmOp* d = nullptr;
        ACC_HIP(hipMalloc(&d, sizeof(GemmOp)));
        ACC_HIP(hipMemcpyAsync(d, &op, sizeof(GemmOp), hipMemcpyHostToDevice, s));
        ACC_TRY(set_lds_gemm_ops());
        int rc = launch_gemm_ops(d, 1, (int)M, (int)N, b_kmajor != 0, s);
        hipStreamSynchronize(s);
        hipFree(d);
        return rc;
    }
    ACC_HIP(hipGetLastError());
    return ACCBPG_OK;
}

int pipe_probe(int iters, int mode, double* ms_out, hipStream_t s) {
    int dev = 0;
    hipDeviceProp_t prop;
    ACC_HIP(hipGetDevice(&dev));
    ACC_HIP(hipGetDeviceProperties(&prop, dev));
    double* sink = nullptr;
    ACC_HIP(hipMalloc(&sink, 8));
    hipEvent_t a, b;
    ACC_HIP(hipEventCreate(&a));
    ACC_HIP(hipEventCreate(&b));
    pipe_probe_kernel<<<prop.multiProcessorCount, NTHREADS, 0, s>>>(iters / 10 + 1, mode, sink);
    ACC_HIP(hipEventRecord(a, s));
    pipe_probe_kernel<<<prop.multiProcessorCount, NTHREADS, 0, s>>>(iters, mode, sink);
    ACC_HIP(hipEventRecord(b, s));
    ACC_HIP(hipEventSynchronize(b));
    float ms = 0.f;
    ACC_HIP(hipEventElapsedTime(&ms, a, b));
    *ms_out = ms;
    hipEventDestroy(a); hipEventDestroy(b); hipFree(sink);
    return ACCBPG_OK;
}

int mfma_peak(int iters, double* tflops, hipStream_t s) {
    int dev = 0;
    hipDeviceProp_t prop;
    ACC_HIP(hipGetDevice(&dev));
    ACC_HIP(hipGetDeviceProperties(&prop, dev));
    const int blocks = prop.multiProcessorCount;
    double* sink = nullptr;
    ACC_HIP(hipMalloc(&sink, 8));
    hipEvent_t a, b;
    ACC_HIP(hipEventCreate(&a));
    ACC_HIP(hipEventCreate(&b));
    mfma_peak_kernel<<<blocks, NTHREADS, 0, s>>>(iters / 10 + 1, sink);
    ACC_HIP(hipEventRecord(a, s));
    mfma_peak_kernel<<<blocks, NTHREADS, 0, s>>>(iters, sink);
    ACC_HIP(hipEventRecord(b, s));
    ACC_HIP(hipEventSynchronize(b));
    float ms = 0.f;
    ACC_HIP(hipEventElapsedTime(&ms, a, b));
    const double flops = (double)blocks * 4.0 * (double)iters * 8.0 * 2048.0;
    *tflops = flops / (ms * 1e-3) * 1e-12;
    hipEventDestroy(a);
    hipEventDestroy(b);
    hipFree(sink);
    return ACCBPG_OK;
}

}
```

### accbpg_and_fw_amd/csrc/internal.h

```cpp
#pragma once
#include <hip/hip_runtime.h>
#include <stdint.h>
#include <stdio.h>
#include <vector>

#include "../../include/accbpg_hip.h"

namespace accbpg {

void set_last_error(const char* fmt, ...);
void note_tiles_fallback(const char* where);

#define ACC_HIP(call)                                                                         \
    do {                                                                                      \
        hipError_t e__ = (call);                                                              \
        if (e__ != hipSuccess) {                                                              \
            ::accbpg::set_last_error("%s:%d: %s -> %s", __FILE__, __LINE__, #call,            \
                                     hipGetErrorString(e__));                                 \
            return ACCBPG_ERR_HIP;                                                            \
        }                                                                                     \
    } while (0)

#define ACC_TRY(call)                       \
    do {                                    \
        int rc__ = (call);                  \
        if (rc__ != ACCBPG_OK) return rc__; \
    } while (0)

struct GemmOp {
    const double* A;
    const double* B;
    double* C;
    int64_t lda, ldb, ldc;
    int32_t M, N, K;
    int32_t lower_only;
    int32_t tri;
    int32_t koff;
    double alpha, beta;
};

struct RedOp {
    double* C;
    const double* P;
    int64_t ldc;
    int32_t M, N, ns, pad;
};

struct TileRC {
    int32_t rb, cb;
    int32_t d1 = -1, d2 = -1;
};

constexpr int BATCH_MAX = ACCBPG_BATCH_MAX;
struct BatchAct {
    int n = 0;
    int idx[BATCH_MAX] = {};
};
struct BatchInst {
    const double* V;
    double* slabs;
    double* gram;
    double* Lbuf;
    double* Wbuf;
    double* Tbuf;
    double* dscal;
    int* dflag;
    int* chol_ready;
};

struct FwInst {
    double* x;
    double* w;
    double* H;
    double* hv;
    const double* V;
    double* vws;
    double* q;
    double* rec;
    int64_t vec_ok;
};
struct ValIdx {
    double v;
    int64_t i;
};
constexpr int FW_PART_MAX = 512;
constexpr int AWAY_NB = 128;
constexpr int FW_DIV_CAP = 512;
__host__ __device__ inline double* fw_vp_of(const FwInst& t, int64_t m) { return t.hv + m; }
__host__ __device__ inline ValIdx* fw_part_of(const FwInst& t, int64_t m) { return reinterpret_cast<ValIdx*>(t.hv + 2 * m); }
__host__ __device__ inline ValIdx* fw_part2_of(const FwInst& t, int64_t m) { return fw_part_of(t, m) + 2 * FW_PART_MAX; }
__host__ __device__ inline ValIdx* fw_mxslot_of(const FwInst& t, int64_t m) { return fw_part2_of(t, m) + AWAY_NB; }
constexpr size_t fw_scratch_doubles(int64_t m) { return (size_t)(2 * m + 2 * (2 * FW_PART_MAX) + 16 + 2 * AWAY_NB + 4); }
__host__ __device__ inline double* fw_rec_d(double* rec) { return rec + 4; }
__host__ __device__ inline int64_t* fw_rec_i(double* rec) { return reinterpret_cast<int64_t*>(rec + 8); }

struct FwProbeArgs {
    int n = 0;
    int idx[BATCH_MAX] = {};
    int nblk[BATCH_MAX] = {};
};
struct FwUpdArgs {
    int n = 0;
    int idx[BATCH_MAX] = {};
    unsigned long long awaymask = 0;
    int64_t p[BATCH_MAX] = {};
    double xscale[BATCH_MAX] = {}, xadd[BATCH_MAX] = {}, hcoef[BATCH_MAX] = {}, hdiv[BATCH_MAX] = {};
};

struct MinMaxRec;
struct KyInst {
    const double* V;
    double* vws;
    int64_t vec_ok;
    const double* B;
    double* Q;
    double* w;
    double* q;
    double* v;
    double* c;
    MinMaxRec* part;
    int64_t* picked;
};

struct FwRun {
    int32_t stop;
    int32_t pad;
    int64_t p;
    double xscale, xadd, hcoef, hdiv;
};

struct FwRunSlot {
    FwRun run;
    double rec[16];
};

struct CholJob { int i, j; };
struct CholInst {
    const double* src;
    double* L;
    double* Ldiag;
    double* Winv;
    double* logdet;
    int* flags;
    int* ready;
    double* aux;
    double* hand;
    long long* trace;
};

constexpr int NB = 64;
constexpr int FLAG_NOT_PD = 0;
constexpr int FLAG_NEG_X = 1;
constexpr int FLAG_NONPOS = 2;
constexpr int FLAG_BAD_G = 3;
constexpr int FLAG_ABORT = 4;
constexpr int STATUS_DOUBLES = 20;
constexpr int ACCBPG_RETRY = 100;

enum ProfKind { PROF_GRAM = 0, PROF_CHOL = 1, PROF_TRTRI = 2, PROF_GRAD = 3, PROF_GRAMFIX = 4, PROF_FWV = 5, PROF_COUNT = 6 };

struct ProfSlot {
    std::vector<hipEvent_t> ev;
    size_t used = 0;
    double total_ms = 0.0;
    int64_t launches = 0;
};

}

struct accbpg_dopt {
    const double* V = nullptr;
    int64_t m = 0, n = 0, ldv = 0;
    hipStream_t stream = nullptr;
    int device = 0;
    int num_cu = 256;
    bool big = false;
    bool force_big = false;
    int gram_grid_cap = 0;
    double* dscal_ext = nullptr;
    bool vec_ok = false;

    double* Lbuf = nullptr;
    double* Wbuf = nullptr;
    double* Tbuf = nullptr;
    double* slabs = nullptr;
    accbpg::TileRC* tiles = nullptr;
    int64_t* wg_ranges = nullptr;
    int32_t* gram_cstart = nullptr;
    int32_t* gram_contrib = nullptr;
    int ntiles = 0, gram_grid = 0, gram_per = 0, gram_nslot = 2;
    int64_t kiters = 0;
    int gram_chunks = 1;
    int64_t gram_nc = 0;
    double* Vblk = nullptr;
    double* dscal = nullptr;
    int* dflag = nullptr;
    double* hpin = nullptr;
    double* vws = nullptr;
    double* xbuf = nullptr;

    accbpg::GemmOp* ops = nullptr;
    std::vector<accbpg::GemmOp> ops_host;
    std::vector<accbpg::RedOp> red_host;
    struct MergeStage { int kind, begin, end, maxm, maxn; };
    std::vector<MergeStage> merge_stages;
    accbpg::RedOp* red = nullptr;
    double* Pbuf = nullptr;
    accbpg::GemmOp* chol_op = nullptr;

    double *fw_x = nullptr, *fw_w = nullptr, *fw_H = nullptr, *fw_hv = nullptr;
    double* fw_hpin_dev = nullptr;
    accbpg::FwInst fw{};
    bool fw_ready = false;
    struct FwSlot {
        accbpg_dopt* aux = nullptr;
        hipStream_t stream = nullptr;
        hipEvent_t ev_snap = nullptr;
        bool pending = false;
    };
    std::vector<FwSlot> fw_ring;
    int fw_ring_depth = 1;
    int fw_ring_small = 2;
    long long fw_ring_issued = 0, fw_ring_collected = 0;
    int fw_part_nblk = 0;
    bool fw_part_away = false;
    accbpg::FwRunSlot* fw_run = nullptr;
    accbpg_fw_step* fw_steps_pin = nullptr;
    accbpg_fw_step* fw_steps_dev = nullptr;
    double* fw_div_ws = nullptr;
    double* fw_div_pin = nullptr;
    double* fw_div_pin_dev = nullptr;
    int64_t fw_div_i = -1;

    bool use_glds = true;
    int kern_variant = 0;
    bool diag_inv_ready = false;
    bool has_duals = false;
    int chol_nk = 8;
    int chol_two_level_T = 64;
    int chol_dbg = 0;
    bool chol_tiles_ok = false;
    bool chol_tiles_off = false;
    int chol_stall_test = 0;
    long long chol_spin_limit = 20000000;
    int chol_tiles_grid = 0;
    int chol_slots = 0;
    void* chol_jobs = nullptr;
    int* chol_ready = nullptr;
    double* chol_aux = nullptr;
    double* chol_hand = nullptr;
    long long* chol_trace = nullptr;
    double* Gbuf = nullptr;
    const double* last_x = nullptr;
    double* last_g = nullptr;
    int last_flag = 0;
    hipEvent_t ev_done = nullptr;
    bool val_reuse = true;
    bool val_valid = false;
    bool val_pending = false;
    bool val_hit = false;
    const double* val_x = nullptr;
    double* val_copy = nullptr;
    double val_f = 0.0;
    double val_answer = 0.0;
    int val_gen = 0;
    int64_t val_compares = 0, val_answered = 0;
    accbpg_dopt* val_peer = nullptr;
    std::vector<accbpg_dopt*> val_linked;
    bool prof_on = false;
    accbpg::ProfSlot prof[accbpg::PROF_COUNT];
};

struct accbpg_dopt_batch {
    int K = 0;
    std::vector<accbpg_dopt*> inst;
    hipStream_t stream = nullptr;
    int device = 0;
    bool fast = false;
    int chunk = 0;
    accbpg::BatchInst* table = nullptr;
    accbpg::CholInst* chol_table[2] = {nullptr, nullptr};
    accbpg::GemmOp* ops_all = nullptr;
    accbpg::RedOp* red_all = nullptr;
    int ops_per_inst = 0, red_per_inst = 0;
    double* dscal_all = nullptr;
    double* hpin = nullptr;
    int* vflags = nullptr;
    double* vout = nullptr;
    double* vpart = nullptr;
    double* vws = nullptr;
    double* vpin = nullptr;
    accbpg::FwInst* fw_table = nullptr;
    accbpg::FwRunSlot* fw_runs = nullptr;
    accbpg_fw_step* fw_bsteps_pin = nullptr;
    accbpg_fw_step* fw_bsteps_dev = nullptr;
    accbpg::BatchAct pend_act;
    const double* pend_x = nullptr;
    double* pend_g = nullptr;
    int64_t pend_ldx = 0, pend_ldg = 0;
    int pend_flag = 0;
    bool pend_fused = false;
};
struct BatchVals { double v[accbpg::BATCH_MAX]; };

namespace accbpg {

int launch_gram_batch(accbpg_dopt_batch* b, const BatchAct& act, const double* xbase, int64_t ldx);
int launch_cholesky_batch(accbpg_dopt_batch* b, const BatchAct& act, bool with_inverse, const double* xbase, int64_t ldx);
int launch_trtri_batch(accbpg_dopt_batch* b, const BatchAct& act);
int launch_colnorm_batch(accbpg_dopt_batch* b, const BatchAct& act, double* gbase, int64_t ldg, double sign);

int dopt_init(accbpg_dopt* h);
int launch_gram(accbpg_dopt* h, const double* x, double* gram);
int launch_cholesky(accbpg_dopt* h, double* A , double* Winv = nullptr ,
                    const double* xcheck = nullptr ,
                    const double* src = nullptr ,
                    double* xkeep = nullptr );
bool chol_tiles_usable(const accbpg_dopt* h);
int launch_trtri(accbpg_dopt* h);
int launch_colnorm(accbpg_dopt* h, const double* W, double* out, double sign);
int launch_gemm_ops(const GemmOp* ops_dev, int nops, int maxM, int maxN, bool b_kmajor, hipStream_t s);
int launch_test_gemm(const double* A, int64_t lda, const double* B, int64_t ldb, double* C, int64_t ldc,
                     int64_t M, int64_t N, int64_t K, int b_kmajor, double alpha, double beta, int config,
                     hipStream_t s);
int build_plans(accbpg_dopt* h);
void set_plan_flags(int flags);
int set_gemm_loop(int variant);
int debug_gram_variant(accbpg_dopt* h, const double* x, int var, int iters, double* ms_out);
int debug_grad_variant(accbpg_dopt* h, double* out, int var, int iters, double* ms_out);
int mfma_peak(int iters, double* tflops, hipStream_t s);
int pipe_probe(int iters, int mode, double* ms_out, hipStream_t s);

int64_t vec_ws_doubles(int64_t n);
int vec_scratch(double** pin, int** flags, double** out);

int vt_nsplit(int64_t m, int64_t n, int num_cu);
int launch_vt_times(const double* V, int64_t ldv, int64_t m, int64_t n, const double* q, double* upart, int nsplit,
                    double* u, bool vec_ok, hipStream_t s);
int launch_vt_times_batch(const KyInst* tab, int K, int64_t ldv, int64_t m, int64_t n, bool first, int nsplit,
                          hipStream_t s);
constexpr int VT_MAXSPLIT = 64;

int device_copy(double* dst, const double* src, size_t ndoubles, hipStream_t s);

void prof_begin(accbpg_dopt* h, ProfKind k);
void prof_end(accbpg_dopt* h, ProfKind k);

}
```

### accbpg_and_fw_amd/csrc/vec_kernels.hip

```cpp
#include <atomic>
#include <mutex>

#include "internal.h"
#include "reduce.hpp"

namespace accbpg {

constexpr int PB = 1024;
constexpr int RB = RED_THREADS;
constexpr int RMAXBLK = 1024;

__device__ __forceinline__ double block_sum_bcast(double v, double* sh) {
    v = wave_sum(v);
    const int lane = threadIdx.x & 63, w = threadIdx.x >> 6;
    __syncthreads();
    if (lane == 0) sh[w] = v;
    __syncthreads();
    double s = 0.0;
#pragma unroll
    for (int i = 0; i < PB / 64; ++i) s += sh[i];
    return s;
}
__device__ __forceinline__ double block_min_bcast(double v, double* sh) {
    v = wave_min(v);
// ... 205 lines not shown
    const int tid = threadIdx.x;
    const int64_t base = (int64_t)blockIdx.x * PB * EPT;
    double gg[EPT];
    const double inf = __builtin_inf();
    double lmin = inf;
    bool bad = false;
#pragma unroll
    for (int e = 0; e < EPT; ++e) {
        const int64_t i = base + tid + (int64_t)PB * e;
        double v = inf;
        if (i < n) {
            double a = g[i];
            if (y != nullptr) {
                const double yi = y[i];
                if (!(yi > 0.0)) bad = true;
                const double t = -1.0 / yi;
                a = a - L * t;
            }
            v = a / L;
        }
        gg[e] = v;
        lmin = min_nan(lmin, v);
    }
    int round = 0;
    double m0 = block_min_bcast(lmin, sh), m1 = 0.0;
    if (!pm_exchange<1>(shm, G, round++, m0, m1, xch, limit)) return;
    const double cmin = -m0;
    auto both = [&](double c, double& fc, double& fpc) -> bool {
        double s = 0.0, d = 0.0;
#pragma unroll
        for (int e = 0; e < EPT; ++e) {
            const double r = gg[e] + c;
            s += 1.0 / r;
            d += -1.0 / (r * r);
        }
        s = block_sum_bcast(s, sh);
        d = block_sum_bcast(d, sh);
        if (!pm_exchange<0>(shm, G, round++, s, d, xch, limit)) return false;
        fc = s - 1.0;
        fpc = d;
        return true;
    };
    double c = cmin + 1.0;
    int nb = 0, nn = 0;
    double fc, fpc;
    if (!both(c, fc, fpc)) return;
    while (fc < 0.0 && nb < 4096) {
        c = (cmin + c) / 2.0;
        if (!both(c, fc, fpc)) return;
        ++nb;
    }
    while (fabs(fc) > eps && nn < 4096) {
        const double step = fc / fpc;
        if ((c - (c - step)) == 0.0) break;
        c = c - step;
        if (!both(c, fc, fpc)) return;
        ++nn;
    }
#pragma unroll
    for (int e = 0; e < EPT; ++e) {
        const int64_t i = base + tid + (int64_t)PB * e;
        if (i < n) xout[i] = 1.0 / (gg[e] + c);
    }
    const int any_bad = __syncthreads_or(bad ? 1 : 0);
    if (tid == 0) {
        if (any_bad) atomicOr(flags + FLAG_NONPOS, 1);
        if (blockIdx.x == 0) { info[0] = nb; info[1] = nn; }
    }
}

__device__ __forceinline__ void ls_terms_partial_body(const double* __restrict__ g,
                                                      const double* __restrict__ x,
                                                      const double* __restrict__ y,
                                                      const double* __restrict__ z,
                                                      const double* __restrict__ z1, int64_t n,
                                                      int want_div_xy, double* __restrict__ part) {
    double s0 = 0.0, s1 = 0.0, s2 = 0.0, mn = __builtin_inf();
    const int64_t stride = (int64_t)gridDim.x * RB;
    for (int64_t i = (int64_t)blockIdx.x * RB + threadIdx.x; i < n; i += stride) {
        if (x != nullptr && y != nullptr) {
            const double xi = x[i], yi = y[i];
            if (g != nullptr) {
                const double d = xi - yi;
                s0 += g[i] * d;
            }
            if (want_div_xy) {
                const double r = xi / yi;
                s1 += r - log(r) - 1.0;
                mn = min_nan(mn, min_nan(xi, yi));
            }
        }
        if (z != nullptr) {
            const double zi = z[i], wi = z1[i];
            const double r = zi / wi;
            s2 += r - log(r) - 1.0;
            mn = min_nan(mn, min_nan(zi, wi));
        }
    }
    double v[4] = {s0, s1, s2, mn};
    block_reduce_store<RB, 4, true>(v, part + blockIdx.x * 4);
}

__global__ __launch_bounds__(RB) void ls_terms_partial_kernel(const double* __restrict__ g,
                                                             const double* __restrict__ x,
                                                             const double* __restrict__ y,
                                                             const double* __restrict__ z,
                                                             const double* __restrict__ z1, int64_t n,
                                                             int want_div_xy, double* __restrict__ part) {
    ls_terms_partial_body(g, x, y, z, z1, n, want_div_xy, part);
}
__global__ __launch_bounds__(RB) void ls_terms_partial_batch_kernel(BatchAct act, const double* __restrict__ g,
                                                                   const double* __restrict__ x,
                                                                   const double* __restrict__ y,
                                                                   const double* __restrict__ z,
                                                                   const double* __restrict__ z1, int64_t ld, int64_t n,
                                                                   double* __restrict__ part, int64_t pstride) {
    const int64_t o = (int64_t)act.idx[blockIdx.y] * ld;
    ls_terms_partial_body(g ? g + o : nullptr, x + o, y + o, z ? z + o : nullptr, z1 ? z1 + o : nullptr, n, 1,
                          part + (int64_t)act.idx[blockIdx.y] * pstride);
}

__global__ __launch_bounds__(RB) void ls_terms_final_kernel(const double* __restrict__ part, int nblk,
                                                           double* __restrict__ out) {
    reduce_final_body<RB, 4, true>(part, nblk, out);
}
__global__ __launch_bounds__(RB) void ls_terms_final_batch_kernel(BatchAct act, const double* __restrict__ part,
                                                                 int64_t pstride, int nblk, double* __restrict__ out) {
    const int inst = act.idx[blockIdx.x];
    reduce_final_body<RB, 4, true>(part + (int64_t)inst * pstride, nblk, out + 4 * inst);
}

__global__ __launch_bounds__(RB) void axpby_batch_kernel(BatchAct act, BatchVals a, const double* __restrict__ x, BatchVals b,
                                                        const double* __restrict__ z, int64_t ld, int64_t n,
                                                        double* __restrict__ out) {
    const int inst = act.idx[blockIdx.y];
    const double ai = a.v[inst], bi = b.v[inst];
    const int64_t o = (int64_t)inst * ld;
    const int64_t stride = (int64_t)gridDim.x * RB;
    for (int64_t i = (int64_t)blockIdx.x * RB + threadIdx.x; i < n; i += stride) {
        const double p = ai * x[o + i];
        const double q = bi * z[o + i];
        out[o + i] = p + q;
    }
}

__global__ __launch_bounds__(RB) void min_sum_partial_kernel(const double* __restrict__ x, int64_t n,
                                                            double* __restrict__ part) {
    double s = 0.0, mn = __builtin_inf();
    const int64_t stride = (int64_t)gridDim.x * RB;
    for (int64_t i = (int64_t)blockIdx.x * RB + threadIdx.x; i < n; i += stride) {
        const double v = x[i];
        s += v;
        mn = min_nan(mn, v);
    }
    double v[2] = {s, mn};
    block_reduce_store<RB, 2, true, 4>(v, part + blockIdx.x * 4);
}

__global__ __launch_bounds__(RB) void axpby_kernel(double a, const double* __restrict__ x, double b,
                                                  const double* __restrict__ z, int64_t n,
                                                  double* __restrict__ out) {
    const int64_t stride = (int64_t)gridDim.x * RB;
    for (int64_t i = (int64_t)blockIdx.x * RB + threadIdx.x; i < n; i += stride) {
        const double p = a * x[i];
        const double q = b * z[i];
        out[i] = p + q;
    }
}

__global__ __launch_bounds__(RB) void div_scalar_kernel(const double* __restrict__ x, double d, int64_t n,
                                                       double* __restrict__ out) {
    const int64_t stride = (int64_t)gridDim.x * RB;
    for (int64_t i = (int64_t)blockIdx.x * RB + threadIdx.x; i < n; i += stride) out[i] = x[i] / d;
}

__global__ __launch_bounds__(RB) void vertex_kernel(int64_t idx, double value, double fill, int64_t n,
                                                   double* __restrict__ out) {
    const int64_t stride = (int64_t)gridDim.x * RB;
    for (int64_t i = (int64_t)blockIdx.x * RB + threadIdx.x; i < n; i += stride) out[i] = (i == idx) ? value : fill;
}

__global__ __launch_bounds__(RB) void dot_partial_kernel(const double* __restrict__ x, const double* __restrict__ y,
                                                        int64_t n, double* __restrict__ part) {
    double s = 0.0;
    const int64_t stride = (int64_t)gridDim.x * RB;
    for (int64_t i = (int64_t)blockIdx.x * RB + threadIdx.x; i < n; i += stride) s += x[i] * y[i];
    double v[1] = {s};
    block_reduce_store<RB, 1, false, 4>(v, part + blockIdx.x * 4);
}

__global__ __launch_bounds__(RB) void burg_reg_prox_kernel(int kind, const double* __restrict__ y,
                                                          const double* __restrict__ g, double L, double lamda,
                                                          int64_t n, double* __restrict__ out,
                                                          int* __restrict__ flags) {
    const int64_t stride = (int64_t)gridDim.x * RB;
    const double lamda_L = lamda / L;
    const double four_l = 4 * lamda_L, two_l = 2 * lamda_L;
    bool bad_y = false, bad_g = false;
    for (int64_t i = (int64_t)blockIdx.x * RB + threadIdx.x; i < n; i += stride) {
        double gt = g[i];
        if (y != nullptr) {
            const double yi = y[i];
            bad_y |= !(yi > 0.0);
            const double hy = -1.0 / yi;
            const double t = L * hy;
            gt = gt - t;
        }
        double r;
        if (kind == 0) {
            bad_g |= !(gt > 0.0);
            r = L / gt;
        } else if (kind == 1) {
            bad_g |= !(gt > -lamda);
            r = L / (lamda + gt);
        } else {
            const double gg = gt / L;
            const double sq = gg * gg;
            r = (sqrt(sq + four_l) - gg) / two_l;
        }
        out[i] = r;
    }
    if (bad_y) flags[FLAG_NONPOS] = 1;
    if (bad_g) flags[FLAG_BAD_G] = 1;
}

__global__ __launch_bounds__(RB) void minmax_partial_kernel(const double* __restrict__ x, int64_t n,
                                                           MinMaxRec* __restrict__ part) {
    minmax_partial_body(x, n, part);
}
__global__ __launch_bounds__(RB) void minmax_final_kernel(const MinMaxRec* __restrict__ part, int nblk,
                                                         MinMaxRec* __restrict__ out) {
    const MinMaxRec a = minmax_final_body(part, nblk);
    if (threadIdx.x == 0) *out = a;
}

struct ScratchBlock {
    double* pin = nullptr;
    int* flags = nullptr;
    double* out = nullptr;
};
constexpr int MAX_DEV = 64;
static std::mutex g_pool_mu;
static std::vector<ScratchBlock> g_pool[MAX_DEV];
struct ThreadScratch {
    ScratchBlock blk[MAX_DEV];
    ~ThreadScratch() {
        std::lock_guard<std::mutex> lk(g_pool_mu);
        for (int d = 0; d < MAX_DEV; ++d)
            if (blk[d].pin) g_pool[d].push_back(blk[d]);
    }
};
static thread_local ThreadScratch g_tls;
static thread_local double* g_pin = nullptr;
static thread_local int* g_flags = nullptr;
static thread_local double* g_out = nullptr;

static int ensure_scratch() {
    int dev = 0;
    ACC_HIP(hipGetDevice(&dev));
    if (dev < 0 || dev >= MAX_DEV) return ACCBPG_ERR_ARG;
    ScratchBlock& b = g_tls.blk[dev];
    if (!b.pin) {
        {
            std::lock_guard<std::mutex> lk(g_pool_mu);
            if (!g_pool[dev].empty()) { b = g_pool[dev].back(); g_pool[dev].pop_back(); }
        }
        if (!b.pin) {
            ScratchBlock nb;
            ACC_HIP(hipHostMalloc(&nb.pin, 32 * sizeof(double), hipHostMallocDefault));
            if (hipMalloc(&nb.flags, 8 * sizeof(int)) != hipSuccess || hipMalloc(&nb.out, 16 * sizeof(double)) != hipSuccess) {
                hipHostFree(nb.pin); hipFree(nb.flags); hipFree(nb.out);
                set_last_error("accbpg: out of device memory for the vector-kernel scratch");
                return ACCBPG_ERR_HIP;
            }
            b = nb;
        }
    }
    g_pin = b.pin; g_flags = b.flags; g_out = b.out;
    return ACCBPG_OK;
}

int vec_scratch(double** pin, int** flags, double** out) {
    ACC_TRY(ensure_scratch());
    *pin = g_pin; *flags = g_flags; *out = g_out;
    return ACCBPG_OK;
}

static bool g_prox_multi_off = false;
static std::atomic<int> g_prox_variant{0};
static thread_local int g_prox_last[2] = {0, 0};

int64_t vec_ws_doubles(int64_t n) { return n + 4 * RMAXBLK + 64; }

static const double* finish4(const double* part, int nb, hipStream_t s) {
    return reduce_finish(ls_terms_final_kernel, part, nb, g_out, g_out, 4, g_pin, s);
}

}

using namespace accbpg;

extern "C" int64_t accbpg_vec_workspace_doubles(int64_t n) { return vec_ws_doubles(n); }

extern "C" int accbpg_burg_simplex_div_prox(const double* y_dev, const double* g_dev, double L, double eps,
                                            int64_t n, double* x_out_dev, double* ws_dev, int* info_host,
                                            void* stream) {
    if (!g_dev || !x_out_dev || n <= 0 || !ws_dev) return ACCBPG_ERR_ARG;
    if (!(L > 0.0)) return ACCBPG_ERR_ASSERT;
    const int forced = g_prox_variant.load(std::memory_order_relaxed);
    bool multi, wide;
    if (forced == 2 || forced == 3) { multi = true; wide = forced == 3; }
    else if (forced == 1) { multi = false; wide = false; }
    else {
        multi = n > (int64_t)PB * 32 && n <= (int64_t)PB * 32 * 128 && !g_prox_multi_off;
        wide = n > (int64_t)PB * 8 * 128;
    }
    const int ept = wide ? 32 : 8;
    const int64_t G64 = (n + (int64_t)PB * ept - 1) / ((int64_t)PB * ept);
    if (multi && G64 > 128) {
        set_last_error("accbpg_burg_simplex_div_prox: the forced multi-workgroup form needs more than 128 workgroups");
        return ACCBPG_ERR_ARG;
    }
    ACC_TRY(ensure_scratch());
    hipStream_t s = (hipStream_t)stream;
    int* g_info = g_flags + 4;
    if (multi) {
        const int G = (int)G64;
        ProxMultiShared shm;
        shm.part = ws_dev;
        shm.epoch = reinterpret_cast<int*>(ws_dev + 4 * G);
        shm.abortw = shm.epoch + G;
        ACC_HIP(hipMemsetAsync(ws_dev, 0, sizeof(double) * 4 * G + sizeof(int) * (G + 4), s));
        ACC_HIP(hipMemsetAsync(g_flags, 0, 8 * sizeof(int), s));
        if (wide)
            burg_prox_multi_kernel<32><<<G, PB, 0, s>>>(y_dev, g_dev, L, eps, n, x_out_dev, shm, G, g_info, g_flags, 20000000LL);
        else
            burg_prox_multi_kernel<8><<<G, PB, 0, s>>>(y_dev, g_dev, L, eps, n, x_out_dev, shm, G, g_info, g_flags, 20000000LL);
        ACC_HIP(hipGetLastError());
        g_prox_last[0] = wide ? 3 : 2; g_prox_last[1] = G;
        int* pin_m = reinterpret_cast<int*>(g_pin);
        ACC_HIP(hipMemcpyAsync(pin_m, g_flags, 6 * sizeof(int), hipMemcpyDeviceToHost, s));
        ACC_HIP(hipMemcpyAsync(pin_m + 8, shm.abortw, sizeof(int), hipMemcpyDeviceToHost, s));
        ACC_HIP(hipStreamSynchronize(s));
        if (pin_m[8] == 0) {
            if (info_host) { info_host[0] = pin_m[4]; info_host[1] = pin_m[5]; }
            if (pin_m[FLAG_NONPOS]) return ACCBPG_ERR_ASSERT;
            return ACCBPG_OK;
        }
        g_prox_multi_off = true;
    }
    int ran;
    if (forced != 1 && n <= (int64_t)PB * 2) {
        burg_prox_kernel<2><<<1, PB, 0, s>>>(y_dev, g_dev, L, eps, n, x_out_dev, ws_dev, g_info, g_flags);
        ran = 10;
    } else if (forced != 1 && n <= (int64_t)PB * 8) {
        burg_prox_kernel<8><<<1, PB, 0, s>>>(y_dev, g_dev, L, eps, n, x_out_dev, ws_dev, g_info, g_flags);
        ran = 11;
    } else if (forced != 1 && n <= (int64_t)PB * 32) {
        burg_prox_kernel<32><<<1, PB, 0, s>>>(y_dev, g_dev, L, eps, n, x_out_dev, ws_dev, g_info, g_flags);
        ran = 12;
    } else {
        burg_prox_kernel<0><<<1, PB, 0, s>>>(y_dev, g_dev, L, eps, n, x_out_dev, ws_dev, g_info, g_flags);
        ran = 1;
    }
    g_prox_last[0] = ran; g_prox_last[1] = 1;
    ACC_HIP(hipGetLastError());
    int* pin_i = reinterpret_cast<int*>(g_pin);
    ACC_HIP(hipMemcpyAsync(pin_i, g_flags, 6 * sizeof(int), hipMemcpyDeviceToHost, s));
    ACC_HIP(hipStreamSynchronize(s));
    if (info_host) { info_host[0] = pin_i[4]; info_host[1] = pin_i[5]; }
    if (pin_i[FLAG_NONPOS]) return ACCBPG_ERR_ASSERT;
    return ACCBPG_OK;
}

extern "C" int accbpg_debug_prox_variant(int variant) {
    if (variant < 0 || variant > 3) return ACCBPG_ERR_ARG;
    g_prox_variant.store(variant, std::memory_order_relaxed);
    return ACCBPG_OK;
}

extern "C" int accbpg_debug_prox_state(int* out3_host) {
    if (!out3_host) return ACCBPG_ERR_ARG;
    out3_host[0] = g_prox_last[0];
    out3_host[1] = g_prox_last[1];
    out3_host[2] = g_prox_multi_off ? 1 : 0;
    return ACCBPG_OK;
}

extern "C" int accbpg_burg_simplex_prox_acc(const double* xi_dev, double alpha, const double* g_dev, double L, double eps,
                                            int64_t n, double* xi_out_dev, double* x_out_dev, double* ws_dev,
                                            int* info_host, void* stream) {
    if (!xi_dev || !g_dev || !xi_out_dev || !x_out_dev || n <= 0 || !ws_dev) return ACCBPG_ERR_ARG;
    if (xi_out_dev == xi_dev || xi_out_dev == g_dev || x_out_dev == xi_out_dev) return ACCBPG_ERR_ARG;
    if (!(L > 0.0)) return ACCBPG_ERR_ASSERT;
    hipStream_t s = (hipStream_t)stream;
    if (n > (int64_t)PB * 32) {
        ACC_TRY(accbpg_vec_axpby(1.0, xi_dev, alpha, g_dev, n, xi_out_dev, stream));
        return accbpg_burg_simplex_div_prox(nullptr, xi_out_dev, L, eps, n, x_out_dev, ws_dev, info_host, stream);
    }
    ACC_TRY(ensure_scratch());
    int* g_info = g_flags + 4;
    if (n <= (int64_t)PB * 2)
        burg_prox_acc_kernel<2><<<1, PB, 0, s>>>(xi_dev, alpha, g_dev, L, eps, n, xi_out_dev, x_out_dev, g_info, g_flags);
    else if (n <= (int64_t)PB * 8)
        burg_prox_acc_kernel<8><<<1, PB, 0, s>>>(xi_dev, alpha, g_dev, L, eps, n, xi_out_dev, x_out_dev, g_info, g_flags);
    else
        burg_prox_acc_kernel<32><<<1, PB, 0, s>>>(xi_dev, alpha, g_dev, L, eps, n, xi_out_dev, x_out_dev, g_info, g_flags);
    ACC_HIP(hipGetLastError());
    if (!info_host) return ACCBPG_OK;
    int* pin_i = reinterpret_cast<int*>(g_pin);
    ACC_HIP(hipMemcpyAsync(pin_i, g_flags, 6 * sizeof(int), hipMemcpyDeviceToHost, s));
    ACC_HIP(hipStreamSynchronize(s));
    info_host[0] = pin_i[4]; info_host[1] = pin_i[5];
    return ACCBPG_OK;
}

extern "C" int accbpg_ls_terms(const double* g_dev, const double* x_dev, const double* y_dev, const double* z_dev,
                               const double* z1_dev, int64_t n, double* out_host, double* ws_dev, void* stream) {
    if (n <= 0 || !out_host || !ws_dev) return ACCBPG_ERR_ARG;
    if ((z_dev == nullptr) != (z1_dev == nullptr)) return ACCBPG_ERR_ARG;
    ACC_TRY(ensure_scratch());
    hipStream_t s = (hipStream_t)stream;
    const int nb = red_blocks(n, RMAXBLK);
    double* part = ws_dev + n;
    ls_terms_partial_kernel<<<nb, RB, 0, s>>>(g_dev, x_dev, y_dev, z_dev, z1_dev, n, 1, part);
    const double* o = finish4(part, nb, s);
    if (!o) return ACCBPG_ERR_HIP;
    out_host[0] = o[0]; out_host[1] = o[1]; out_host[2] = o[2];
    if (!(o[3] > 0.0)) return ACCBPG_ERR_ASSERT;
    return ACCBPG_OK;
}

extern "C" int accbpg_burg_divergence(const double* x_dev, const double* y_dev, int64_t n, double* out_host,
                                      double* ws_dev, void* stream) {
    if (!x_dev || !y_dev) return ACCBPG_ERR_ARG;
    double o[3];
    int rc = accbpg_ls_terms(nullptr, x_dev, y_dev, nullptr, nullptr, n, o, ws_dev, stream);
    if (out_host) out_host[0] = o[1];
    return rc;
}

extern "C" int accbpg_vec_dot_diff(const double* g_dev, const double* x_dev, const double* y_dev, int64_t n,
                                   double* out_host, double* ws_dev, void* stream) {
    if (!g_dev || !x_dev || !y_dev || n <= 0 || !out_host || !ws_dev) return ACCBPG_ERR_ARG;
    ACC_TRY(ensure_scratch());
    hipStream_t s = (hipStream_t)stream;
    const int nb = red_blocks(n, RMAXBLK);
    double* part = ws_dev + n;
    ls_terms_partial_kernel<<<nb, RB, 0, s>>>(g_dev, x_dev, y_dev, nullptr, nullptr, n, 0, part);
    const double* o = finish4(part, nb, s);
    if (!o) return ACCBPG_ERR_HIP;
    out_host[0] = o[0];
    return ACCBPG_OK;
}

extern "C" int accbpg_vec_min_sum(const double* x_dev, int64_t n, double* out_host, double* ws_dev, void* stream) {
    if (!x_dev || n <= 0 || !out_host || !ws_dev) return ACCBPG_ERR_ARG;
    ACC_TRY(ensure_scratch());
    hipStream_t s = (hipStream_t)stream;
    const int nb = red_blocks(n, RMAXBLK);
    double* part = ws_dev + n;
    min_sum_partial_kernel<<<nb, RB, 0, s>>>(x_dev, n, part);
    const double* o = finish4(part, nb, s);
    if (!o) return ACCBPG_ERR_HIP;
    out_host[0] = o[3];
    out_host[1] = o[0];
    return ACCBPG_OK;
}

extern "C" int accbpg_vec_axpby(double a, const double* x_dev, double b, const double* z_dev, int64_t n,
                                double* out_dev, void* stream) {
    if (!x_dev || !z_dev || !out_dev || n <= 0) return ACCBPG_ERR_ARG;
    hipStream_t s = (hipStream_t)stream;
    axpby_kernel<<<ew_blocks(n), RB, 0, s>>>(a, x_dev, b, z_dev, n, out_dev);
    ACC_HIP(hipGetLastError());
    return ACCBPG_OK;
}

extern "C" int accbpg_vec_div_scalar(const double* x_dev, double d, int64_t n, double* out_dev, void* stream) {
    if (!x_dev || !out_dev || n <= 0) return ACCBPG_ERR_ARG;
    div_scalar_kernel<<<ew_blocks(n), RB, 0, (hipStream_t)stream>>>(x_dev, d, n, out_dev);
    ACC_HIP(hipGetLastError());
    return ACCBPG_OK;
}

extern "C" int accbpg_vec_vertex(int64_t idx, double value, double fill, int64_t n, double* out_dev, void* stream) {
    if (!out_dev || n <= 0 || idx < 0 || idx >= n) return ACCBPG_ERR_ARG;
    vertex_kernel<<<ew_blocks(n), RB, 0, (hipStream_t)stream>>>(idx, value, fill, n, out_dev);
    ACC_HIP(hipGetLastError());
    return ACCBPG_OK;
}

extern "C" int accbpg_vec_argminmax(const double* x_dev, int64_t n, int64_t* idx_host, double* val_host,
                                    double* ws_dev, void* stream) {
    if (!x_dev || n <= 0 || !idx_host || !ws_dev) return ACCBPG_ERR_ARG;
    ACC_TRY(ensure_scratch());
    hipStream_t s = (hipStream_t)stream;
    int nb = red_blocks(n, RMAXBLK);
    if (nb > 128) nb = 128;
    MinMaxRec* part = reinterpret_cast<MinMaxRec*>(ws_dev + n + (n & 1));
    MinMaxRec* out = reinterpret_cast<MinMaxRec*>(g_out + 8);
    minmax_partial_kernel<<<nb, RB, 0, s>>>(x_dev, n, part);
    minmax_final_kernel<<<1, RB, 0, s>>>(part, nb, out);
    ACC_HIP(hipGetLastError());
    ACC_HIP(hipMemcpyAsync(g_pin + 16, out, sizeof(MinMaxRec), hipMemcpyDeviceToHost, s));
    ACC_HIP(hipStreamSynchronize(s));
    const MinMaxRec* r = reinterpret_cast<const MinMaxRec*>(g_pin + 16);
    idx_host[0] = r->imin;
    idx_host[1] = r->imax;
    if (val_host) { val_host[0] = r->vmin; val_host[1] = r->vmax; }
    return ACCBPG_OK;
}

extern "C" int accbpg_vec_dot(const double* x_dev, const double* y_dev, int64_t n, double* out_host, double* ws_dev,
                              void* stream) {
    if (!x_dev || !y_dev || n <= 0 || !out_host || !ws_dev) return ACCBPG_ERR_ARG;
    ACC_TRY(ensure_scratch());
    hipStream_t s = (hipStream_t)stream;
    const int nb = red_blocks(n, RMAXBLK);
    double* part = ws_dev + n;
    dot_partial_kernel<<<nb, RB, 0, s>>>(x_dev, y_dev, n, part);
    const double* o = finish4(part, nb, s);
    if (!o) return ACCBPG_ERR_HIP;
    out_host[0] = o[0];
    return ACCBPG_OK;
}

extern "C" int accbpg_burg_reg_div_prox(int kind, const double* y_dev, const double* g_dev, double L, double lamda,
                                        int64_t n, double* x_out_dev, void* stream) {
    if (!g_dev || !x_out_dev || n <= 0 || kind < 0 || kind > 2) return ACCBPG_ERR_ARG;
    if (!(L > 0.0)) {
        set_last_error("prox_map only takes positive L");
        return ACCBPG_ERR_ASSERT;
    }
    if (kind != 0 && !(lamda >= 0.0)) return ACCBPG_ERR_ARG;
    ACC_TRY(ensure_scratch());
    hipStream_t s = (hipStream_t)stream;
    ACC_HIP(hipMemsetAsync(g_flags, 0, 8 * sizeof(int), s));
    burg_reg_prox_kernel<<<ew_blocks(n), RB, 0, s>>>(kind, y_dev, g_dev, L, lamda, n, x_out_dev, g_flags);
    ACC_HIP(hipGetLastError());
    int* pin_i = reinterpret_cast<int*>(g_pin);
    ACC_HIP(hipMemcpyAsync(pin_i, g_flags, 4 * sizeof(int), hipMemcpyDeviceToHost, s));
    ACC_HIP(hipStreamSynchronize(s));
    if (pin_i[FLAG_NONPOS]) {
        set_last_error("Either y or L is not positive.");
        return ACCBPG_ERR_ASSERT;
    }
    if (pin_i[FLAG_BAD_G]) {
        set_last_error(kind == 1 ? "Not getting positive solution." : "BurgEntropy prox_map only takes positive value.");
        return ACCBPG_ERR_ASSERT;
    }
    return ACCBPG_OK;
}


static int batch_vec_scratch(accbpg_dopt_batch* b) {
    if (b->vflags) return ACCBPG_OK;
    ACC_HIP(hipMalloc(&b->vflags, sizeof(int) * 8 * (size_t)b->K));
    ACC_HIP(hipMemset(b->vflags, 0, sizeof(int) * 8 * (size_t)b->K));
    ACC_HIP(hipMalloc(&b->vout, sizeof(double) * 4 * (size_t)b->K));
    ACC_HIP(hipMalloc(&b->vpart, sizeof(double) * 4 * RMAXBLK * (size_t)b->K));
    ACC_HIP(hipHostMalloc(&b->vpin, sizeof(double) * 8 * (size_t)b->K, hipHostMallocDefault));
    return ACCBPG_OK;
}

static BatchAct batch_active(const accbpg_dopt_batch* b, const int* active_host) {
    BatchAct act;
    for (int i = 0; i < b->K && i < BATCH_MAX; ++i)
        if (!active_host || active_host[i]) act.idx[act.n++] = i;
    return act;
}

extern "C" int accbpg_dopt_batch_burg_simplex_div_prox(accbpg_dopt_batch* b, const double* y_dev, const double* g_dev,
                                                       int64_t ld, const double* L_host, double eps, double* x_out_dev,
                                                       const int* active_host, int* status_host, int* info_host) {
    if (!b || !g_dev || !x_out_dev || !L_host || !status_host || b->K > BATCH_MAX) return ACCBPG_ERR_ARG;
    const int64_t n = b->inst[0]->n;
    if (ld < n) return ACCBPG_ERR_ARG;
    ACC_TRY(batch_vec_scratch(b));
    BatchAct all = batch_active(b, active_host), act;
    BatchVals Ls;
    for (int a = 0; a < all.n; ++a) {
        const int i = all.idx[a];
        Ls.v[i] = L_host[i];
        if (!(L_host[i] > 0.0)) status_host[i] = ACCBPG_ERR_ASSERT;
        else { status_host[i] = ACCBPG_OK; act.idx[act.n++] = i; }
    }
    if (act.n == 0) return ACCBPG_OK;
    hipStream_t s = b->stream;
    if (n > (int64_t)PB * 32) {
        if (!b->vws) ACC_HIP(hipMalloc(&b->vws, sizeof(double) * (size_t)vec_ws_doubles(n)));
        for (int a = 0; a < act.n; ++a) {
            const int i = act.idx[a];
            int info[2] = {0, 0};
            const int rc = accbpg_burg_simplex_div_prox(y_dev ? y_dev + (size_t)i * ld : nullptr, g_dev + (size_t)i * ld,
                                                        L_host[i], eps, n, x_out_dev + (size_t)i * ld, b->vws, info, s);
            if (rc == ACCBPG_ERR_ASSERT) status_host[i] = ACCBPG_ERR_ASSERT;
            else if (rc != ACCBPG_OK) return rc;
            if (info_host) { info_host[2 * i] = info[0]; info_host[2 * i + 1] = info[1]; }
        }
        return ACCBPG_OK;
    }
    if (n <= (int64_t)PB * 2)
        burg_prox_batch_kernel<2><<<act.n, PB, 0, s>>>(act, y_dev, g_dev, ld, Ls, eps, n, x_out_dev, nullptr, b->vflags);
    else if (n <= (int64_t)PB * 8)
        burg_prox_batch_kernel<8><<<act.n, PB, 0, s>>>(act, y_dev, g_dev, ld, Ls, eps, n, x_out_dev, nullptr, b->vflags);
    else
        burg_prox_batch_kernel<32><<<act.n, PB, 0, s>>>(act, y_dev, g_dev, ld, Ls, eps, n, x_out_dev, nullptr, b->vflags);
    ACC_HIP(hipGetLastError());
    int* pin_i = reinterpret_cast<int*>(b->vpin);
    ACC_HIP(hipMemcpyAsync(pin_i, b->vflags, sizeof(int) * 8 * (size_t)b->K, hipMemcpyDeviceToHost, s));
    ACC_HIP(hipStreamSynchronize(s));
    for (int a = 0; a < act.n; ++a) {
        const int i = act.idx[a];
        if (pin_i[8 * i + FLAG_NONPOS]) status_host[i] = ACCBPG_ERR_ASSERT;
        if (info_host) { info_host[2 * i] = pin_i[8 * i + 4]; info_host[2 * i + 1] = pin_i[8 * i + 5]; }
    }
    return ACCBPG_OK;
}

extern "C" int accbpg_dopt_batch_ls_terms(accbpg_dopt_batch* b, const double* g_dev, const double* x_dev, const double* y_dev,
                                          const double* z_dev, const double* z1_dev, int64_t ld, const int* active_host,
                                          double* out_host, int* status_host) {
    if (!b || !x_dev || !y_dev || !out_host || !status_host || b->K > BATCH_MAX) return ACCBPG_ERR_ARG;
    if ((z_dev == nullptr) != (z1_dev == nullptr)) return ACCBPG_ERR_ARG;
    const int64_t n = b->inst[0]->n;
    if (ld < n) return ACCBPG_ERR_ARG;
    ACC_TRY(batch_vec_scratch(b));
    const BatchAct act = batch_active(b, active_host);
    if (act.n == 0) return ACCBPG_OK;
    hipStream_t s = b->stream;
    const int nb = red_blocks(n, RMAXBLK);
    ls_terms_partial_batch_kernel<<<dim3(nb, act.n), RB, 0, s>>>(act, g_dev, x_dev, y_dev, z_dev, z1_dev, ld, n, b->vpart,
                                                                4 * RMAXBLK);
    ls_terms_final_batch_kernel<<<act.n, RB, 0, s>>>(act, b->vpart, 4 * RMAXBLK, nb, b->vout);
    ACC_HIP(hipGetLastError());
    ACC_HIP(hipMemcpyAsync(b->vpin, b->vout, sizeof(double) * 4 * (size_t)b->K, hipMemcpyDeviceToHost, s));
    ACC_HIP(hipStreamSynchronize(s));
    for (int a = 0; a < act.n; ++a) {
        const int i = act.idx[a];
        out_host[3 * i] = b->vpin[4 * i]; out_host[3 * i + 1] = b->vpin[4 * i + 1]; out_host[3 * i + 2] = b->vpin[4 * i + 2];
        status_host[i] = (b->vpin[4 * i + 3] > 0.0) ? ACCBPG_OK : ACCBPG_ERR_ASSERT;
    }
    return ACCBPG_OK;
}

extern "C" int accbpg_dopt_batch_axpby(accbpg_dopt_batch* b, const double* a_host, const double* x_dev, const double* b_host,
                                       const double* z_dev, int64_t ld, const int* active_host, double* out_dev) {
    if (!b || !a_host || !b_host || !x_dev || !z_dev || !out_dev || b->K > BATCH_MAX) return ACCBPG_ERR_ARG;
    const int64_t n = b->inst[0]->n;
    if (ld < n) return ACCBPG_ERR_ARG;
    const BatchAct act = batch_active(b, active_host);
    if (act.n == 0) return ACCBPG_OK;
    BatchVals av, bv;
    for (int i = 0; i < b->K; ++i) { av.v[i] = a_host[i]; bv.v[i] = b_host[i]; }
    int64_t nb = (n + RB - 1) / RB;
    if (nb > 256) nb = 256;
    axpby_batch_kernel<<<dim3((unsigned)nb, act.n), RB, 0, b->stream>>>(act, av, x_dev, bv, z_dev, ld, n, out_dev);
    ACC_HIP(hipGetLastError());
    return ACCBPG_OK;
}
```

### accbpg_and_fw_amd/functions.py

```python
from __future__ import annotations

import ctypes as C
import threading

import numpy as np
import torch

from . import _lib


def _device():
    if not torch.cuda.is_available():
        raise RuntimeError("accbpg_and_fw_amd needs an AMD GPU (torch.cuda is not available); "
                           "there is no CPU fallback")
    return torch.device("cuda", torch.cuda.current_device())


def to_dev(a):
    if isinstance(a, torch.Tensor):
        if a.dtype != torch.float64:
            a = a.to(torch.float64)
        if not a.is_cuda:
            return a.to(_device()).contiguous(), False
        return a.contiguous(), False
    arr = np.ascontiguousarray(np.asarray(a, dtype=np.float64))
    return torch.from_numpy(arr).to(_device()), True


def from_dev(t, as_numpy):
    return t.cpu().numpy() if as_numpy else t


def _stream():
    return C.c_void_p(torch.cuda.current_stream().cuda_stream)


def _ptr(t):
    return C.c_void_p(t.data_ptr()) if t is not None else C.c_void_p(0)


class _Workspace:
    _local = threading.local()
    _KEEP = 8

    @classmethod
    def get(cls, n, device):
        cache = getattr(cls._local, "cache", None)
        if cache is None:
            cache = cls._local.cache = {}
        key = (device.index, int(n))
        ws = cache.pop(key, None)
        if ws is None:
            size = _lib.load().accbpg_vec_workspace_doubles(int(n))
            ws = torch.empty(size, dtype=torch.float64, device=device)
            while len(cache) >= cls._KEEP:
                cache.pop(next(iter(cache)))
        cache[key] = ws
        return ws


_WS = object()


def _call(name, ref, *args, assert_msg=None):
    with torch.cuda.device(ref.device):
        args = [_ptr(_Workspace.get(ref.numel(), ref.device)) if a is _WS else a for a in args]
        rc = getattr(_lib.load(), name)(*args, _stream())
    _lib.check(rc, name, assert_msg)


class RSmoothFunction:

    def __call__(self, x):
        assert 0, "RSmoothFunction: __call__(x) is not defined"

    def gradient(self, x):
        assert 0, "RSmoothFunction: gradient(x) is not defined"

    def func_grad(self, x, flag):
        assert 0, "RSmoothFunction: func_grad(x, flag) is not defined"


class DOptimalObj(RSmoothFunction):

    def __init__(self, H, _shard=False, _borrowed=None):
        self.H = H
        self.m = H.shape[0]
        self.n = H.shape[1]
        assert _shard or self.m < self.n, "DOptimalObj: need m < n"
        self._V, _ = to_dev(H)
        lib = _lib.load()
        if _borrowed is not None:
            h, self._owner = _borrowed
            self._owned = False
        else:
            h = C.c_void_p()
            with torch.cuda.device(self._V.device):
                rc = lib.accbpg_dopt_create(_ptr(self._V), self.m, self.n, self._V.stride(0), _stream(), C.byref(h),
                                            1 if _shard else 0)
            _lib.check(rc, "accbpg_dopt_create")
            self._owned = True
        self._h = h
        self._lib = lib
        self.calls = {"value": 0, "grad": 0}
        self._overlap = True
        self._spec = False
        self.spec_unused = 0
        self._prof = False
        self._lin = False
        self._gcache = []
        self._gcache_cap = 5
        self._lin_refresh = 50
        self.gram_launches = 0
        self.gram_combos = 0
        self.value_hits = 0
        self._reuse = True

    def __del__(self):
        for name in ("_h", "_h2"):
            h = getattr(self, name, None)
            if name == "_h" and not getattr(self, "_owned", True):
                continue
            if h:
                try:
                    self._lib.accbpg_dopt_destroy(h)
                except Exception:
                    pass
                setattr(self, name, None)

    def overlap_values(self, enable=True):
        self._overlap = bool(enable)
        return self

    def value_async(self, x):
        assert x.numel() == self.n, "DOptimalObj: x.size not equal to n"
        self._side_handle()
        with torch.cuda.device(self._V.device):
            self._side.wait_stream(torch.cuda.current_stream())
            rc = self._lib.accbpg_dopt_func_grad_begin(self._h2, _ptr(x), 0, None)
        _lib.check(rc, "accbpg_dopt_func_grad_begin")
        return x

    def value_wait(self, ticket):
        fval = C.c_double(0.0)
        with torch.cuda.device(self._V.device):
            rc = self._lib.accbpg_dopt_func_grad_end(self._h2, C.byref(fval))
        _lib.check(rc, "accbpg_dopt_func_grad_end", "DOptimalObj: x needs to be nonnegative")
        self.calls["value"] += 1
        self._memo_put(ticket, fval.value)
        return fval.value

    def speculate(self, enable=True):
        self._spec = bool(enable)
        return self

    def memoize_values(self, enable=True):
        self._memo_on = bool(enable)
        self._memo = None
        return self

    def reuse_values(self, enable=True):
        self._reuse = bool(enable)
        for h in self._handles():
            self._lib.accbpg_dopt_value_reuse(h, 1 if enable else 0)
        return self

    @property
    def values_reused(self):
        total = 0
        for h in self._handles():
            cmp_, ans = C.c_int64(0), C.c_int64(0)
            self._lib.accbpg_dopt_value_reuse_stats(h, C.byref(cmp_), C.byref(ans))
            total += ans.value
        return total

    def _memo_get(self, x):
        memo = getattr(self, "_memo", None)
        if getattr(self, "_memo_on", False) and memo is not None and memo[0] is x and memo[1] == x._version:
            self.value_hits += 1
            self.calls["value"] += 1
            return memo[2]
        return None

    def _memo_put(self, x, value):
        if getattr(self, "_memo_on", False) and isinstance(x, torch.Tensor):
            self._memo = (x, x._version, value)

    def _side_handle(self):
        if getattr(self, "_h2", None) is None:
            h2 = C.c_void_p()
            with torch.cuda.device(self._V.device):
                self._side = torch.cuda.Stream(device=self._V.device)
                rc = self._lib.accbpg_dopt_create(_ptr(self._V), self.m, self.n, self._V.stride(0),
                                                  C.c_void_p(self._side.cuda_stream), C.byref(h2), 1)
            _lib.check(rc, "accbpg_dopt_create")
            self._h2 = h2
            self._lib.accbpg_dopt_factor_in_small_launches(h2, 2)
            self._lib.accbpg_dopt_value_reuse(h2, 1 if self._reuse else 0)
            _lib.check(self._lib.accbpg_dopt_value_peer(h2, self._h), "accbpg_dopt_value_peer")
            _lib.check(self._lib.accbpg_dopt_value_peer(self._h, h2), "accbpg_dopt_value_peer")
            if self._prof:
                self._lib.accbpg_dopt_profile_enable(self._h2, 1)
        return self._h2

    def grad_async(self, y):
        h2 = self._side_handle()
        g = torch.empty(self.n, dtype=torch.float64, device=self._V.device)
        with torch.cuda.device(self._V.device):
            self._side.wait_stream(torch.cuda.current_stream())
            y.record_stream(self._side)
            g.record_stream(self._side)
            rc = self._lib.accbpg_dopt_func_grad_begin(h2, _ptr(y), 2, _ptr(g))
        _lib.check(rc, "accbpg_dopt_func_grad_begin")
        return (y, g)

    def grad_wait(self, ticket):
        y, g = ticket
        fval = C.c_double(0.0)
        with torch.cuda.device(self._V.device):
            rc = self._lib.accbpg_dopt_func_grad_end(self._h2, C.byref(fval))
            torch.cuda.current_stream().wait_stream(self._side)
        _lib.check(rc, "accbpg_dopt_func_grad_end", "DOptimalObj: x needs to be nonnegative")
        self.calls["grad"] += 1
        return fval.value, g

    def grad_drop(self, ticket):
        self.spec_unused += 1

    def value_lead_seconds(self):
        ms = C.c_double(0.0)
        rc = self._lib.accbpg_dopt_eval_gap_ms(self._h2, self._h, C.byref(ms))
        return max(0.0, ms.value * 1e-3) if rc == _lib.OK else 0.0

    @property
    def device(self):
        return self._V.device

    @property
    def V_dev(self):
        return self._V

    def __call__(self, x):
        return self.func_grad(x, flag=0)

    def gradient(self, x):
        return self.func_grad(x, flag=1)

    def func_grad(self, x, flag=2):
        assert (x.numel() if isinstance(x, torch.Tensor) else x.size) == self.n, \
            "DOptimalObj: x.size not equal to n"
        if flag == 0 and isinstance(x, torch.Tensor):
            hit = self._memo_get(x)
            if hit is not None:
                return hit
        xd, was_np = to_dev(x)
        fval = C.c_double(0.0)
        g = None
        with torch.cuda.device(self._V.device):
            self._lib.accbpg_dopt_set_stream(self._h, _stream())
            if flag != 0:
                g = torch.empty(self.n, dtype=torch.float64, device=self._V.device)
            rc = self._lib.accbpg_dopt_func_grad(self._h, _ptr(xd), int(flag), C.byref(fval), _ptr(g))
        _lib.check(rc, "accbpg_dopt_func_grad", "DOptimalObj: x needs to be nonnegative")
        self.calls["value" if flag == 0 else "grad"] += 1
        if flag == 0:
            self._memo_put(x, fval.value)
            return fval.value
        g = from_dev(g, was_np)
        return g if flag == 1 else (fval.value, g)

    def linear_gram(self, enable=True, refresh=50, capacity=5):
        self._lin = bool(enable)
        self._lin_refresh = int(refresh)
        self._gcache_cap = int(capacity)
        self._gcache = []
        return self

    def _gram_lookup(self, vec):
        for idx, ent in enumerate(self._gcache):
            if ent[0] is vec:
                self._gcache.append(self._gcache.pop(idx))
                return ent
        return None

    def ensure_gram(self, x):
        with torch.cuda.device(self._V.device):
            self._lib.accbpg_dopt_set_stream(self._h, _stream())
            if self._gram_lookup(x) is None:
                self._gram_direct(x)

    def _gram_store(self, vec, gram, age):
        self._gcache = [e for e in self._gcache if e[0] is not vec]
        self._gcache.append([vec, gram, age, None])
        if len(self._gcache) > self._gcache_cap:
            self._gcache.pop(0)

    def _gram_buffer(self):
        if len(self._gcache) >= self._gcache_cap:
            return self._gcache.pop(0)[1]
        return torch.empty(self.m, self.m, dtype=torch.float64, device=self._V.device)

    def _gram_direct(self, xd):
        gram = self._gram_buffer()
        rc = self._lib.accbpg_dopt_gram(self._h, _ptr(xd), _ptr(gram))
        _lib.check(rc, "accbpg_dopt_gram")
        self.gram_launches += 1
        self._gram_store(xd, gram, 0)
        return gram

    def func_grad_combo(self, x, combo, flag=2):
        assert x.numel() == self.n, "DOptimalObj: x.size not equal to n"
        fval = C.c_double(0.0)
        g = None
        with torch.cuda.device(self._V.device):
            self._lib.accbpg_dopt_set_stream(self._h, _stream())
            ent = self._gram_lookup(x)
            if ent is not None:
                gram = ent[1]
            else:
                gram = None
                if combo is not None:
                    a, x1, b, x2 = combo
                    e1, e2 = self._gram_lookup(x1), self._gram_lookup(x2)
                    if e1 is not None and e2 is not None and max(e1[2], e2[2]) < self._lin_refresh:
                        g1, g2, age = e1[1], e2[1], max(e1[2], e2[2]) + 1
                        gram = self._gram_buffer()
                        rc = self._lib.accbpg_dopt_gram_lincomb(self._h, float(a), _ptr(g1), float(b), _ptr(g2),
                                                                _ptr(gram))
                        _lib.check(rc, "accbpg_dopt_gram_lincomb")
                        self.gram_combos += 1
                        self._gram_store(x, gram, age)
                if gram is None:
                    gram = self._gram_direct(x)
            ent = self._gram_lookup(x)
            if flag == 0 and ent is not None and ent[3] is not None:
                self.calls["value"] += 1
                self.value_hits += 1
                return ent[3]
            if flag != 0:
                g = torch.empty(self.n, dtype=torch.float64, device=self._V.device)
            mn, _ = vec_min_sum(x)
            assert mn >= 0, "DOptimalObj: x needs to be nonnegative"
            rc = self._lib.accbpg_dopt_eval_gram(self._h, _ptr(gram), int(flag), C.byref(fval), _ptr(g))
        _lib.check(rc, "accbpg_dopt_eval_gram")
        self.calls["value" if flag == 0 else "grad"] += 1
        if ent is not None:
            ent[3] = fval.value
        if flag == 0:
            return fval.value
        return g if flag == 1 else (fval.value, g)

    def gram_into(self, x_dev, gram_dev):
        with torch.cuda.device(self._V.device):
            self._lib.accbpg_dopt_set_stream(self._h, _stream())
            rc = self._lib.accbpg_dopt_gram(self._h, _ptr(x_dev), _ptr(gram_dev))
        _lib.check(rc, "accbpg_dopt_gram")

    def factor(self, gram_dev):
        fval = C.c_double(0.0)
        with torch.cuda.device(self._V.device):
            rc = self._lib.accbpg_dopt_factor(self._h, _ptr(gram_dev), C.byref(fval))
        _lib.check(rc, "accbpg_dopt_factor")
        return fval.value

    def grad_from_factor(self, g_dev):
        with torch.cuda.device(self._V.device):
            rc = self._lib.accbpg_dopt_grad(self._h, _ptr(g_dev))
        _lib.check(rc, "accbpg_dopt_grad")

    def vt_times(self, q):
        qd, _ = to_dev(q)
        u = torch.empty(self.n, dtype=torch.float64, device=self._V.device)
        with torch.cuda.device(self._V.device):
            self._lib.accbpg_dopt_set_stream(self._h, _stream())
            rc = self._lib.accbpg_dopt_vt_times(self._h, _ptr(qd), _ptr(u))
        _lib.check(rc, "accbpg_dopt_vt_times")
        return u

    def column(self, j):
        out = torch.empty(self.m, dtype=torch.float64, device=self._V.device)
        with torch.cuda.device(self._V.device):
            rc = self._lib.accbpg_dopt_get_column(self._h, int(j), _ptr(out))
        _lib.check(rc, "accbpg_dopt_get_column")
        return out.cpu().numpy()

    def kyinit_picks(self, B, Q_out=None):
        Bd, _ = to_dev(B)
        assert Bd.shape == (self.m, self.m), "kyinit_picks: B must be m x m"
        if Q_out is not None:
            assert Q_out.is_cuda and Q_out.dtype == torch.float64 and Q_out.is_contiguous() \
                and Q_out.shape == (self.m, self.m), "kyinit_picks: Q_out must be a contiguous m x m fp64 device tensor"
        picked = np.empty(2 * self.m, dtype=np.int64)
        with torch.cuda.device(self._V.device):
            self._lib.accbpg_dopt_set_stream(self._h, _stream())
            rc = self._lib.accbpg_dopt_kyinit(self._h, _ptr(Bd), picked.ctypes.data_as(C.POINTER(C.c_int64)),
                                              _ptr(Q_out))
        _lib.check(rc, "accbpg_dopt_kyinit")
        return picked

    def _handles(self):
        return [h for h in (self._h, getattr(self, "_h2", None)) if h]

    def profile(self, enable=True):
        self._prof = bool(enable)
        for h in self._handles():
            self._lib.accbpg_dopt_profile_enable(h, 1 if enable else 0)
            self._lib.accbpg_dopt_profile_reset(h)

    def profile_read(self):
        out = {}
        for idx, name in enumerate(["gram", "cholesky", "trtri", "grad", "gram_fixup", "fw_vpass"]):
            tot, num = 0.0, 0
            for h in self._handles():
                ms, cnt = C.c_double(0.0), C.c_int64(0)
                self._lib.accbpg_dopt_profile_read(h, idx, C.byref(ms), C.byref(cnt))
                tot, num = tot + ms.value, num + cnt.value
            out[name] = (tot, num)
        return out


class PoissonRegression(RSmoothFunction):

    _create, _destroy = "accbpg_poisson_create", "accbpg_poisson_destroy"
    _set_stream, _func_grad, _get_ax = "accbpg_poisson_set_stream", "accbpg_poisson_func_grad", "accbpg_poisson_get_ax"
    _size_msg = "PoissonRegression: x.size not equal to n."
    _match_msg = "A and b sizes not matching"

    def __init__(self, A, b):
        assert A.shape[0] == b.shape[0], self._match_msg
        self.A = A
        self.b = b
        self.m = A.shape[0]
        self.n = A.shape[1]
        self._A, _ = to_dev(A)
        self._b, _ = to_dev(b)
        lib = _lib.load()
        h = C.c_void_p()
        with torch.cuda.device(self._A.device):
            rc = getattr(lib, self._create)(_ptr(self._A), self.m, self.n, self._A.stride(0), _ptr(self._b),
                                            _stream(), C.byref(h))
        _lib.check(rc, self._create)
        self._h = h
        self._lib = lib

    def __del__(self):
        h = getattr(self, "_h", None)
        if h:
            try:
                getattr(self._lib, self._destroy)(h)
            except Exception:
                pass
            self._h = None

    def __call__(self, x):
        return self.func_grad(x, flag=0)

    def gradient(self, x):
        return self.func_grad(x, flag=1)

    def func_grad(self, x, flag=2):
        size = x.numel() if isinstance(x, torch.Tensor) else x.size
        assert size == self.n, self._size_msg
        xd, was_np = to_dev(x)
        g = torch.empty(self.n, dtype=torch.float64, device=self._A.device) if flag != 0 else None
        fval = C.c_double(0.0)
        with torch.cuda.device(self._A.device):
            getattr(self._lib, self._set_stream)(self._h, _stream())
            rc = getattr(self._lib, self._func_grad)(self._h, _ptr(xd), int(flag), C.byref(fval), _ptr(g))
        _lib.check(rc, self._func_grad)
        if flag == 0:
            return fval.value
        if flag == 1:
            return from_dev(g, was_np)
        return fval.value, from_dev(g, was_np)

    def fitted(self):
        out = torch.empty(self.m, dtype=torch.float64, device=self._A.device)
# ... 476 lines not shown
```

### include/accbpg_hip.h

```cpp
#ifndef ACCBPG_HIP_H
#define ACCBPG_HIP_H

#include <stdint.h>

#ifdef __cplusplus
extern "C" {
#endif

#define ACCBPG_OK            0
#define ACCBPG_ERR_ASSERT    1
#define ACCBPG_ERR_NOT_PD    2
#define ACCBPG_ERR_HIP       3
#define ACCBPG_ERR_ARG       4

typedef struct accbpg_dopt accbpg_dopt;

int         accbpg_abi_version(void);
const char* accbpg_last_error(void);


int accbpg_dopt_create(const double* V_dev, int64_t m, int64_t n, int64_t ldv,
                       void* stream, accbpg_dopt** out, int is_shard);
int accbpg_dopt_destroy(accbpg_dopt* h);
int accbpg_dopt_set_stream(accbpg_dopt* h, void* stream);

int accbpg_dopt_func_grad(accbpg_dopt* h, const double* x_dev, int flag,
                          double* f_host, double* g_dev);

int accbpg_dopt_func_grad_begin(accbpg_dopt* h, const double* x_dev, int flag, double* g_dev);
int accbpg_dopt_func_grad_end(accbpg_dopt* h, double* f_host);

int accbpg_dopt_eval_gap_ms(accbpg_dopt* first, accbpg_dopt* second, double* ms_host);

int accbpg_dopt_value_reuse(accbpg_dopt* h, int on);
int accbpg_dopt_value_reuse_stats(accbpg_dopt* h, int64_t* compares_host, int64_t* answered_host);
int accbpg_dopt_value_peer(accbpg_dopt* h, accbpg_dopt* peer);

int accbpg_dopt_gram(accbpg_dopt* h, const double* x_dev, double* gram_dev);
int accbpg_dopt_factor(accbpg_dopt* h, const double* gram_dev, double* f_host);
int accbpg_dopt_grad(accbpg_dopt* h, double* g_dev);

int accbpg_tri_pack(const double* G_dev, int64_t m, double* packed_dev, void* stream);
int accbpg_tri_unpack(const double* packed_dev, int64_t m, double* G_dev, void* stream);
int accbpg_vec_count_bad(const double* x_dev, int64_t n, double* count_dev, void* stream);

#define ACCBPG_SHARD_ID_BYTES 128
typedef struct accbpg_dopt_shard accbpg_dopt_shard;
int accbpg_dopt_shard_bounds(int64_t n, int world, int rank, int64_t* lo, int64_t* hi);
int accbpg_shard_unique_id(void* id_out);
int accbpg_dopt_shard_create(accbpg_dopt* local, int64_t n, int world, int rank, const void* unique_id,
                             void* comm, accbpg_dopt_shard** out);
int accbpg_dopt_shard_func_grad(accbpg_dopt_shard* s, const double* x_dev, int flag, double* f_host, double* g_dev);
int accbpg_dopt_shard_destroy(accbpg_dopt_shard* s);
int accbpg_debug_shard_pad(accbpg_dopt_shard* s, int64_t extra);

int accbpg_dopt_gram_lincomb(accbpg_dopt* h, double a, const double* G1_dev, double b,
                             const double* G2_dev, double* out_dev);
int accbpg_dopt_eval_gram(accbpg_dopt* h, const double* gram_dev, int flag, double* f_host, double* g_dev);

#define ACCBPG_BATCH_MAX 64
typedef struct accbpg_dopt_batch accbpg_dopt_batch;

int accbpg_dopt_batch_create(const double* const* V_dev_host, int K, int64_t m, int64_t n, int64_t ldv, void* stream,
                             accbpg_dopt_batch** out);
int accbpg_dopt_batch_destroy(accbpg_dopt_batch* b);
int accbpg_dopt_batch_set_stream(accbpg_dopt_batch* b, void* stream);
int accbpg_dopt_batch_size(accbpg_dopt_batch* b);
int accbpg_dopt_batch_is_fused(accbpg_dopt_batch* b);
int accbpg_dopt_batch_chunk(accbpg_dopt_batch* b);
accbpg_dopt* accbpg_dopt_batch_instance(accbpg_dopt_batch* b, int i);

int accbpg_dopt_batch_func_grad(accbpg_dopt_batch* b, const double* x_dev, int64_t ldx, const int* active_host, int flag,
                                double* f_host, double* g_dev, int64_t ldg, int* status_host);
int accbpg_dopt_batch_func_grad_begin(accbpg_dopt_batch* b, const double* x_dev, int64_t ldx, const int* active_host,
                                      int flag, double* g_dev, int64_t ldg);
int accbpg_dopt_batch_func_grad_end(accbpg_dopt_batch* b, double* f_host, int* status_host);

int accbpg_dopt_batch_burg_simplex_div_prox(accbpg_dopt_batch* b, const double* y_dev, const double* g_dev, int64_t ld,
                                            const double* L_host, double eps, double* x_out_dev, const int* active_host,
                                            int* status_host, int* info_host);

int accbpg_dopt_batch_ls_terms(accbpg_dopt_batch* b, const double* g_dev, const double* x_dev, const double* y_dev,
                               const double* z_dev, const double* z1_dev, int64_t ld, const int* active_host,
                               double* out_host, int* status_host);

int accbpg_dopt_batch_axpby(accbpg_dopt_batch* b, const double* a_host, const double* x_dev, const double* b_host,
                            const double* z_dev, int64_t ld, const int* active_host, double* out_dev);

int64_t accbpg_vec_workspace_doubles(int64_t n);

int accbpg_burg_simplex_div_prox(const double* y_dev, const double* g_dev, double L, double eps,
                                 int64_t n, double* x_out_dev, double* ws_dev,
                                 int* info_host, void* stream);

int accbpg_burg_divergence(const double* x_dev, const double* y_dev, int64_t n,
                           double* out_host, double* ws_dev, void* stream);

int accbpg_ls_terms(const double* g_dev, const double* x_dev, const double* y_dev,
                    const double* z_dev, const double* z1_dev, int64_t n,
                    double* out_host, double* ws_dev, void* stream);

int accbpg_vec_axpby(double a, const double* x_dev, double b, const double* z_dev, int64_t n,
                     double* out_dev, void* stream);

int accbpg_vec_dot_diff(const double* g_dev, const double* x_dev, const double* y_dev, int64_t n,
                        double* out_host, double* ws_dev, void* stream);

int accbpg_vec_min_sum(const double* x_dev, int64_t n, double* out_host, double* ws_dev, void* stream);


int accbpg_vec_div_scalar(const double* x_dev, double d, int64_t n, double* out_dev, void* stream);

int accbpg_vec_vertex(int64_t idx, double value, double fill, int64_t n, double* out_dev, void* stream);

int accbpg_vec_argminmax(const double* x_dev, int64_t n, int64_t* idx_host, double* val_host,
                         double* ws_dev, void* stream);

int accbpg_dopt_vt_times(accbpg_dopt* h, const double* q_dev, double* u_dev);

int accbpg_dopt_get_column(accbpg_dopt* h, int64_t j, double* out_dev);

int accbpg_dopt_kyinit(accbpg_dopt* h, const double* B_dev, int64_t* picked_host, double* Q_dev);


typedef struct accbpg_fw_probe {
    int64_t i;
    int64_t j;
    double  w_i;
    double  w_j;
    double  x_j;
    double  logdet_H;
    double  q_prev;
} accbpg_fw_probe;

int accbpg_fw_init(accbpg_dopt* h, const double* x0_dev, double* logdet_gram_host);

int accbpg_fw_probe_step(accbpg_dopt* h, int away, int refresh_logdet, accbpg_fw_probe* probe_host);

int accbpg_fw_logdet_ring(accbpg_dopt* h, int depth, int small_launches);
int accbpg_fw_logdet_pending(accbpg_dopt* h);
int accbpg_fw_logdet_flush(accbpg_dopt* h, double* logdet_host);

int accbpg_fw_update(accbpg_dopt* h, int64_t p, double xscale, double xadd, double hcoef, double hdiv);

int accbpg_fw_get_state(accbpg_dopt* h, double* x_dev, double* w_dev, double* H_dev);

typedef struct accbpg_fw_div_probe {
    int64_t i;
    double  w_i, x_i;
    double  sum_w, sum_w2;
    double  slope;
    double  div;
    double  min_x;
    double  sum_u2;
} accbpg_fw_div_probe;
int accbpg_fw_div_probe_step(accbpg_dopt* h, double fill, double value, accbpg_fw_div_probe* out_host);
int accbpg_fw_div_apply(accbpg_dopt* h, int64_t p, double a, double fill, double value, double hcoef, double hdiv);

int accbpg_fw_logdet_snapshot(accbpg_dopt* h, double* collected_host);

#define ACCBPG_FW_RUN_MAX 1024
typedef struct accbpg_fw_step {
    int64_t i, j;  double w_i, w_j, x_j, q_prev;
    int64_t p;     double xscale, xadd, hcoef, hdiv;
    int32_t kind;
    int32_t status;
} accbpg_fw_step;
int accbpg_fw_run(accbpg_dopt* h, int away, double eps, int nsteps, accbpg_fw_step* steps_host, int* nrun_host);

int accbpg_dopt_batch_fw_init(accbpg_dopt_batch* b, const double* x0_dev, int64_t ldx, const int* active_host,
                              double* logdet_gram_host, int* status_host);
int accbpg_dopt_batch_fw_probe(accbpg_dopt_batch* b, int away, const int* active_host, accbpg_fw_probe* probes_host);
int accbpg_dopt_batch_fw_update(accbpg_dopt_batch* b, const int* active_host, const int64_t* p_host,
                                const double* xscale_host, const double* xadd_host, const double* hcoef_host,
                                const double* hdiv_host);

int accbpg_dopt_batch_fw_run(accbpg_dopt_batch* b, int away, const double* eps_host, int nsteps, const int* active_host,
                             accbpg_fw_step* steps_host, int* nrun_host);

int accbpg_dopt_batch_kyinit(accbpg_dopt_batch* b, const double* B_dev, int64_t* picked_host, double* Q_dev);


typedef struct accbpg_poisson accbpg_poisson;

int accbpg_poisson_create(const double* A_dev, int64_t m, int64_t n, int64_t lda, const double* b_dev,
                          void* stream, accbpg_poisson** out);
int accbpg_poisson_destroy(accbpg_poisson* h);
int accbpg_poisson_set_stream(accbpg_poisson* h, void* stream);

int accbpg_poisson_func_grad(accbpg_poisson* h, const double* x_dev, int flag, double* f_host, double* g_dev);

int accbpg_poisson_get_ax(accbpg_poisson* h, double* out_dev);


typedef struct accbpg_kldiv accbpg_kldiv;

int accbpg_kldiv_create(const double* A_dev, int64_t m, int64_t n, int64_t lda, const double* b_dev,
                        void* stream, accbpg_kldiv** out);
int accbpg_kldiv_destroy(accbpg_kldiv* h);
int accbpg_kldiv_set_stream(accbpg_kldiv* h, void* stream);

int accbpg_kldiv_func_grad(accbpg_kldiv* h, const double* x_dev, int flag, double* f_host, double* g_dev);

int accbpg_kldiv_get_ax(accbpg_kldiv* h, double* out_dev);

int accbpg_shannon_div_prox(int kind, const double* y_dev, const double* g_dev, double L, double lamda, int64_t n,
                            double* x_out_dev, double* ws_dev, void* stream);

int accbpg_shannon_ls_terms(const double* g_dev, const double* x_dev, const double* y_dev, const double* z_dev,
                            const double* z1_dev, int64_t n, double delta, double* out_host, double* ws_dev,
                            void* stream);
int accbpg_shannon_divergence(const double* x_dev, const double* y_dev, int64_t n, double delta, double* out_host,
                              double* ws_dev, void* stream);


typedef struct accbpg_symnmf accbpg_symnmf;

int accbpg_symnmf_create(const double* M_dev, int64_t n, int64_t ldm, int64_t r, double m_norm, void* stream,
                         accbpg_symnmf** out);
int accbpg_symnmf_destroy(accbpg_symnmf* h);
int accbpg_symnmf_set_stream(accbpg_symnmf* h, void* stream);

int accbpg_symnmf_func_grad(accbpg_symnmf* h, const double* X_dev, int flag, double* f_host, double* g_dev);

int accbpg_symnmf_plan(accbpg_symnmf* h, int64_t* out4);

int accbpg_quartic_prox_stage(const double* y_dev, const double* g_dev, double z, double invL, int clip,
                              double upper_bound, int64_t n, double* out_dev, double* ssq_host, double* ws_dev,
                              void* stream);

int accbpg_quartic_ls_terms(const double* g_dev, const double* x_dev, const double* y_dev, const double* z_dev,
                            const double* z1_dev, int64_t n, double* out7_host, double* ws_dev, void* stream);

int accbpg_lmo_l2_ball(const double* g_dev, int center_kind, const double* center_dev, double center_val,
                       double radius, double gnorm, int64_t n, double* out_dev, double* dist_host, double* ws_dev,
                       void* stream);

int accbpg_lmo_linf_ball(const double* g_dev, int center_kind, const double* center_dev, double center_val,
                         double radius, int64_t n, double* out_dev, void* stream);

int accbpg_burg_reg_div_prox(int kind, const double* y_dev, const double* g_dev, double L, double lamda,
                             int64_t n, double* x_out_dev, void* stream);

int accbpg_vec_dot(const double* x_dev, const double* y_dev, int64_t n, double* out_host, double* ws_dev,
                   void* stream);


int accbpg_combine_ls_terms(int kind, double a, const double* u_dev, double b, const double* v_dev, double c,
                            const double* g_dev, const double* x_dev, int64_t n, double* w_dev, double* out2_host,
                            double* ws_dev, void* stream);

int accbpg_burg_simplex_prox_acc(const double* xi_dev, double alpha, const double* g_dev, double L, double eps,
                                 int64_t n, double* xi_out_dev, double* x_out_dev, double* ws_dev, int* info_host,
                                 void* stream);

int accbpg_lmo_l2_ball_pos(const double* g_dev, const double* center_dev, double radius, double epsilon, int64_t n,
                           double* out_dev, double* info3_host, double* ws_dev, void* stream);


int accbpg_dopt_profile_enable(accbpg_dopt* h, int enable);
int accbpg_dopt_profile_read(accbpg_dopt* h, int which, double* total_ms_host, int64_t* launches_host);
int accbpg_dopt_profile_reset(accbpg_dopt* h);

int accbpg_mfma_f64_peak(int iters, double* tflops_host, void* stream);

int accbpg_debug_pipe_probe(int iters, int mode, double* ms_host, void* stream);

int accbpg_test_gemm(const double* A_dev, int64_t lda, const double* B_dev, int64_t ldb,
                     double* C_dev, int64_t ldc, int64_t M, int64_t N, int64_t K,
                     int b_kmajor, double alpha, double beta, int config, void* stream);

int accbpg_debug_gram_variant(accbpg_dopt* h, const double* x_dev, int variant, int iters, double* ms_host);
int accbpg_debug_grad_variant(accbpg_dopt* h, double* g_dev, int variant, int iters, double* ms_host);
int accbpg_dopt_factor_in_small_launches(accbpg_dopt* h, int on);

int accbpg_debug_plan_flags(int flags);

int accbpg_debug_gemm_loop(int variant);

int accbpg_debug_prox_variant(int variant);
int accbpg_debug_prox_state(int* out3_host);

int accbpg_debug_chol_variant(accbpg_dopt* h, int bits);
int accbpg_debug_chol_trace(accbpg_dopt* h, const double* gram_dev, int with_inverse, int64_t* stamps_host);

#ifdef __cplusplus
}
#endif
#endif
```

Before: 63.67 iterations/s.

## Fuse ABPG line-search trial into one device submission with single host wait

Adds a C API entry that enqueues the whole line-search trial (y axpby, gram+Cholesky+gradient, Burg simplex prox, x axpby, LS terms, value at x, optional reuse compare for f(x_k)) on one stream. All statuses are copied back in one block and the host waits once. The ABPG gain loop uses it for D-optimal objectives with BurgEntropySimplex. This removes several host-device synchronizations per iteration, along with the separate value evaluation. It adds a replay fallback path and refactors Cholesky/prox launchers to take caller-provided status buffers, at the cost of more complex control flow.

```diff
diff --git a/accbpg_and_fw_amd/_lib.py b/accbpg_and_fw_amd/_lib.py
--- a/accbpg_and_fw_amd/_lib.py
+++ b/accbpg_and_fw_amd/_lib.py
@@ -28,6 +28,12 @@
                 ("hcoef", C.c_double), ("hdiv", C.c_double), ("kind", C.c_int32), ("status", C.c_int32)]
 
 
+class TrialOut(C.Structure):
+    _fields_ = [("fy", C.c_double), ("lin", C.c_double), ("dxy", C.c_double), ("dzz", C.c_double), ("fx", C.c_double),
+                ("fk", C.c_double), ("prox_info", C.c_int32 * 2), ("fk_answered", C.c_int32), ("reserved", C.c_int32)]
+
+
+TRIAL_REPLAY = 5
 FW_RUN_MAX = 1024
 FW_APPLIED, FW_STOPPED, FW_BAD_PIVOT, FW_NOT_RUN = 0, 1, 2, 3
 
@@ -42,8 +48,11 @@
     "accbpg_dopt_func_grad_begin": (C.c_int, [_P, _P, C.c_int, _P]),
     "accbpg_dopt_func_grad_end": (C.c_int, [_P, C.POINTER(C.c_double)]),
     "accbpg_dopt_eval_gap_ms": (C.c_int, [_P, _P, C.POINTER(C.c_double)]),
+    "accbpg_dopt_burg_trial": (C.c_int, [_P, _P, _P, C.c_double, C.c_double, C.c_double, C.c_int, _P, _P, _P, _P, _P,
+                                         C.POINTER(TrialOut)]),
     "accbpg_dopt_value_reuse": (C.c_int, [_P, C.c_int]),
     "accbpg_dopt_value_reuse_stats": (C.c_int, [_P, C.POINTER(C.c_int64), C.POINTER(C.c_int64)]),
+    "accbpg_dopt_value_recorded": (C.c_int, [_P, _P]),
     "accbpg_dopt_value_peer": (C.c_int, [_P, _P]),
     "accbpg_dopt_gram": (C.c_int, [_P, _P, _P]),
     "accbpg_dopt_factor": (C.c_int, [_P, _P, C.POINTER(C.c_double)]),
diff --git a/accbpg_and_fw_amd/algorithms.py b/accbpg_and_fw_amd/algorithms.py
--- a/accbpg_and_fw_amd/algorithms.py
+++ b/accbpg_and_fw_amd/algorithms.py
@@ -6,7 +6,7 @@
 import numpy as np
 import torch
 
-from .functions import (BurgEntropy, BurgEntropySimplex, ShannonEntropy, SquaredL2Norm, SumOf2nd4thPowers,
+from .functions import (BurgEntropy, BurgEntropySimplex, DOptimalObj, ShannonEntropy, SquaredL2Norm, SumOf2nd4thPowers,
                         combine_ls_terms, from_dev, ls_terms, shannon_ls_terms, to_dev, vec_axpby, vec_div_scalar,
                         vec_dot_diff)
 from .utils import get_random_float
@@ -45,6 +45,17 @@
 def _can_speculate(f, x, checkdiv):
     return (not checkdiv) and (not _lin(f)) and getattr(f, "_spec", False) and getattr(f, "_overlap", False) \
         and not getattr(f, "_prof", False) and hasattr(f, "grad_async") and isinstance(x, torch.Tensor) and x.is_cuda
+
+
+_BURG_SIMPLEX_HOOKS = ("div_prox_map", "prox_map", "_prox", "divergence", "extra_Psi")
+
+
+def _can_one_wait(f, h, x, checkdiv):
+    if checkdiv or not isinstance(f, DOptimalObj) or not f._one_wait_ok():
+        return False
+    if type(h) is not BurgEntropySimplex or any(name in vars(h) for name in _BURG_SIMPLEX_HOOKS):
+        return False
+    return isinstance(x, torch.Tensor) and x.is_cuda and x.device == f.device
 
 
 def _value_end(f, pending):
@@ -231,12 +242,15 @@
     retries_before = 0
     k = -1
     for k in range(maxitrs):
-        pending = _value_begin(f, x, xcombo)
-        t_known = time.time()
-
         z_prev, x_prev = z, x
         G_prev, theta_prev = G, theta
         G = G / ls_dec
+
+        one_wait = _can_one_wait(f, h, x_prev, checkdiv)
+        fk_in_trial = one_wait and f.value_recorded(x_prev)
+        pending = None if fk_in_trial else _value_begin(f, x, xcombo)
+        t_known = time.time()
+        fk_due = True
 
         def theta_for(Gt):
             if kk == 0:
@@ -252,27 +266,49 @@
         searching = True
         while searching:
             theta = theta_for(G)
-            if started is not None:
-                y, ticket = started
-                started = None
-                fy, g = f.grad_wait(ticket)
+            done = None
+            if one_wait:
+                done = f.trial(x_prev, z_prev, theta, theta ** (gamma - 1) * G * L, h.eps, fk_due and pending is None)
+            if fk_due and pending is None and (done is None or not done[4].fk_answered):
+                pending = _value_begin(f, x_prev, xcombo)
+                t_known = time.time()
+            if done is not None:
+                y, g, z, x, res = done
+                fy = res.fy
+                h.last_info = (res.prox_info[0], res.prox_info[1])
+                if fk_due:
+                    if pending is None:
+                        F[k] = res.fk + h.extra_Psi(x_prev)
+                        T[k] = time.time() - t_start
+                    else:
+                        F[k] = _value_end(f, pending) + h.extra_Psi(x_prev)
+                        T[k] = _stamp(f, pending, t_start, t_known)
+                        pending = None
+                    fk_due = False
+                lin, dxy, dzz = np.float64(res.lin), np.float64(res.dxy), np.float64(res.dzz)
             else:
-                y = vec_axpby(1 - theta, x_prev, theta, z_prev)
+                if started is not None:
+                    y, ticket = started
+                    started = None
+                    fy, g = f.grad_wait(ticket)
+                else:
+                    y = vec_axpby(1 - theta, x_prev, theta, z_prev)
+                    if _lin(f):
+                        fy, g = f.func_grad_combo(y, (1 - theta, x_prev, theta, z_prev), 2)
+                    else:
+                        fy, g = f.func_grad(y)
+                if fk_due:
+                    F[k] = _value_end(f, pending) + h.extra_Psi(x_prev)
+                    T[k] = _stamp(f, pending, t_start, t_known)
+                    pending = None
+                    fk_due = False
+                z = h.div_prox_map(z_prev, g, theta ** (gamma - 1) * G * L)
+                x = vec_axpby(1 - theta, x_prev, theta, z)
                 if _lin(f):
-                    fy, g = f.func_grad_combo(y, (1 - theta, x_prev, theta, z_prev), 2)
-                else:
-                    fy, g = f.func_grad(y)
-            if pending is not None:
-                F[k] = _value_end(f, pending) + h.extra_Psi(x_prev)
-                T[k] = _stamp(f, pending, t_start, t_known)
-                pending = None
-            z = h.div_prox_map(z_prev, g, theta ** (gamma - 1) * G * L)
-            x = vec_axpby(1 - theta, x_prev, theta, z)
-            if _lin(f):
-                f.ensure_gram(z)
-                xcombo = (1 - theta, x_prev, theta, z)
-
-            lin, dxy, dzz = _divergences(h, g, x, y, z, z_prev)
+                    f.ensure_gram(z)
+                    xcombo = (1 - theta, x_prev, theta, z)
+
+                lin, dxy, dzz = _divergences(h, g, x, y, z, z_prev)
             if dzz < epsilon:
                 break
 
@@ -285,7 +321,12 @@
                     theta_next = theta_for(G * ls_inc)
                     y_next = vec_axpby(1 - theta_next, x_prev, theta_next, z_prev)
                     started = (y_next, f.grad_async(y_next))
-                searching = (_value(f, x, xcombo) > fy + lin + theta ** gamma * G * L * dzz)
+                if done is not None:
+                    f.calls["value"] += 1
+                    fx = res.fx
+                else:
+                    fx = _value(f, x, xcombo)
+                searching = (fx > fy + lin + theta ** gamma * G * L * dzz)
 
             if searching:
                 G = G * ls_inc
diff --git a/accbpg_and_fw_amd/csrc/capi.hip b/accbpg_and_fw_amd/csrc/capi.hip
--- a/accbpg_and_fw_amd/csrc/capi.hip
+++ b/accbpg_and_fw_amd/csrc/capi.hip
@@ -5,6 +5,7 @@
 
 #include "internal.h"
 #include "reduce.hpp"
+#include "trial_verdict.h"
 
 namespace accbpg {
 
@@ -100,6 +101,8 @@
         lk.erase(std::remove(lk.begin(), lk.end(), h), lk.end());
     }
     hipFree(h->val_copy);
+    hipFree(h->trial_stat);
+    if (h->trial_pin) hipHostFree(h->trial_pin);
     hipFree(h->Vblk);
     hipFree(h->Lbuf); hipFree(h->Wbuf); hipFree(h->Tbuf); hipFree(h->slabs); hipFree(h->tiles); hipFree(h->wg_ranges); hipFree(h->gram_cstart); hipFree(h->gram_contrib);
     if (!h->dscal_ext) hipFree(h->dscal);
@@ -206,6 +209,18 @@
     ACC_HIP(hipStreamSynchronize(h->stream));
     ++h->val_compares;
     *same = *pin != stamp;
+    return ACCBPG_OK;
+}
+
+static int enqueue_eval(accbpg_dopt* h, const double* x_dev, int flag, double* g_dev, double* status, bool record) {
+    double* gram = chol_tiles_usable(h) ? h->Gbuf : h->Lbuf;
+    ACC_TRY(launch_gram(h, x_dev, gram));
+    if (record) ACC_TRY(value_alloc(h));
+    ACC_TRY(launch_cholesky(h, h->Lbuf, flag != 0 ? h->Wbuf : nullptr, x_dev, gram, record ? h->val_copy : nullptr, status));
+    if (flag != 0) {
+        ACC_TRY(launch_trtri(h));
+        ACC_TRY(launch_colnorm(h, h->Wbuf, g_dev, -1.0));
+    }
     return ACCBPG_OK;
 }
 
@@ -230,14 +245,7 @@
         }
         h->val_valid = false;
     }
-    double* gram = chol_tiles_usable(h) ? h->Gbuf : h->Lbuf;
-    ACC_TRY(launch_gram(h, x_dev, gram));
-    if (record) ACC_TRY(value_alloc(h));
-    ACC_TRY(launch_cholesky(h, h->Lbuf, flag != 0 ? h->Wbuf : nullptr, x_dev, gram, record ? h->val_copy : nullptr));
-    if (flag != 0) {
-        ACC_TRY(launch_trtri(h));
-        ACC_TRY(launch_colnorm(h, h->Wbuf, g_dev, -1.0));
-    }
+    ACC_TRY(enqueue_eval(h, x_dev, flag, g_dev, h->dscal, record));
     h->val_pending = record;
     ACC_HIP(hipMemcpyAsync(h->hpin, h->dscal, sizeof(double) * STATUS_DOUBLES, hipMemcpyDeviceToHost, h->stream));
     ACC_HIP(hipEventRecord(h->ev_done, h->stream));
@@ -319,11 +327,111 @@
     return accbpg_dopt_func_grad_end(h, f_host);
 }
 
+static_assert(TRIAL_EVAL_DOUBLES == STATUS_DOUBLES && TRIAL_FLAG_NOT_PD == FLAG_NOT_PD && TRIAL_FLAG_NEG_X == FLAG_NEG_X &&
+                  TRIAL_FLAG_NONPOS == FLAG_NONPOS && TRIAL_FLAG_ABORT == FLAG_ABORT,
+              "trial_verdict.h restates the status layout");
+
+extern "C" int accbpg_dopt_burg_trial(accbpg_dopt* h, const double* x_prev_dev, const double* z_prev_dev, double theta,
+                                      double L, double eps, int want_fk, double* y_dev, double* g_dev, double* z_dev,
+                                      double* x_dev, double* ws_dev, accbpg_trial_out* out_host) {
+    if (!h || !x_prev_dev || !z_prev_dev || !y_dev || !g_dev || !z_dev || !x_dev || !ws_dev || !out_host)
+        return ACCBPG_ERR_ARG;
+    if (!(L > 0.0)) {
+        value_forget(h);
+        return ACCBPG_TRIAL_REPLAY;
+    }
+    const int64_t n = h->n;
+    hipStream_t s = h->stream;
+    if (!h->trial_stat) {
+        double* p = nullptr;
+        ACC_HIP(hipMalloc(&p, sizeof(double) * TRIAL_DOUBLES));
+        if (hipMemset(p, 0, sizeof(double) * TRIAL_DOUBLES) != hipSuccess ||
+            hipHostMalloc(&h->trial_pin, sizeof(double) * TRIAL_DOUBLES, hipHostMallocDefault) != hipSuccess) {
+            hipFree(p);
+            set_last_error("accbpg_dopt_burg_trial: could not allocate the status block");
+            return ACCBPG_ERR_HIP;
+        }
+        h->trial_stat = p;
+    }
+    double* blk = h->trial_stat;
+    h->val_pending = false;
+    h->val_hit = false;
+    const bool record = h->val_reuse;
+    TrialAsked asked = {0, 0};
+    const accbpg_dopt* rec = nullptr;
+    auto fail = [&](int rc) { value_forget(h); return rc; };
+    if (want_fk && record) {
+        accbpg_dopt* const recs[2] = {h, h->val_peer};
+        for (int r = 0; r < 2 && !rec; ++r)
+            if (recs[r] && recs[r]->val_valid && recs[r]->val_x == x_prev_dev) rec = recs[r];
+        if (rec) {
+            asked.cmp_stamp = h->val_gen = h->val_gen % 1000000000 + 1;
+            const int64_t nb = std::min<int64_t>((n + 255) / 256, 1024);
+            value_compare_kernel<<<(unsigned)nb, 256, 0, s>>>(reinterpret_cast<const unsigned long long*>(x_prev_dev),
+                                                             reinterpret_cast<const unsigned long long*>(rec->val_copy), n,
+                                                             asked.cmp_stamp, reinterpret_cast<int*>(blk + TRIAL_CMP));
+            if (hipGetLastError() != hipSuccess) return fail(ACCBPG_ERR_HIP);
+        }
+    }
+    const double rec_f = rec ? rec->val_f : 0.0;
+    if (record) h->val_valid = false;
+    bool multi = false;
+    auto enqueue = [&]() -> int {
+        ACC_TRY(accbpg_vec_axpby(1.0 - theta, x_prev_dev, theta, z_prev_dev, n, y_dev, s));
+        ACC_TRY(enqueue_eval(h, y_dev, 2, g_dev, blk + TRIAL_GRAD, false));
+        ACC_TRY(trial_prox_enqueue(z_prev_dev, g_dev, L, eps, n, z_dev, ws_dev, reinterpret_cast<int*>(blk + TRIAL_PROX),
+                                   TRIAL_PROX_GAVE_UP, s, &multi));
+        ACC_TRY(accbpg_vec_axpby(1.0 - theta, x_prev_dev, theta, z_dev, n, x_dev, s));
+        ACC_TRY(trial_ls_terms_enqueue(g_dev, x_dev, y_dev, z_dev, z_prev_dev, n, ws_dev, blk + TRIAL_LS, s));
+        ACC_TRY(enqueue_eval(h, x_dev, 0, nullptr, blk + TRIAL_VALUE, record));
+        ACC_HIP(hipMemcpyAsync(h->trial_pin, blk, sizeof(double) * TRIAL_DOUBLES, hipMemcpyDeviceToHost, s));
+        ACC_HIP(hipEventRecord(h->ev_done, s));
+        ACC_HIP(hipStreamSynchronize(s));
+        return ACCBPG_OK;
+    };
+    const int rc = enqueue();
+    if (rc != ACCBPG_OK) return fail(rc);
+    asked.prox_multi = multi ? 1 : 0;
+    const double* pin = h->trial_pin;
+    const TrialVerdict v = trial_verdict(pin, asked);
+    if (v.chol_gave_up && !h->chol_tiles_off) {
+        h->chol_tiles_off = true;
+        note_tiles_fallback("accbpg_dopt_burg_trial");
+    }
+    if (v.prox_gave_up) trial_prox_gave_up();
+    if (v.replay) return fail(ACCBPG_TRIAL_REPLAY);
+    const int* px = reinterpret_cast<const int*>(pin + TRIAL_PROX);
+    out_host->fy = -pin[TRIAL_GRAD];
+    out_host->lin = pin[TRIAL_LS]; out_host->dxy = pin[TRIAL_LS + 1]; out_host->dzz = pin[TRIAL_LS + 2];
+    out_host->fx = -pin[TRIAL_VALUE];
+    out_host->prox_info[0] = px[TRIAL_PROX_INFO]; out_host->prox_info[1] = px[TRIAL_PROX_INFO + 1];
+    out_host->fk_answered = v.fk_answered;
+    out_host->fk = v.fk_answered ? rec_f : 0.0;
+    if (asked.cmp_stamp) {
+        ++h->val_compares;
+        if (v.fk_answered) ++h->val_answered;
+    }
+    if (record) {
+        h->val_x = x_dev;
+        h->val_f = out_host->fx;
+        h->val_valid = true;
+    }
+    return ACCBPG_OK;
+}
+
 extern "C" int accbpg_dopt_value_reuse(accbpg_dopt* h, int on) {
     if (!h) return ACCBPG_ERR_ARG;
     h->val_reuse = on != 0;
     value_forget(h);
     return ACCBPG_OK;
+}
+
+extern "C" int accbpg_dopt_value_recorded(accbpg_dopt* h, const double* x_dev) {
+    if (!h || !x_dev || !h->val_reuse) return 0;
+    const accbpg_dopt* const recs[2] = {h, h->val_peer};
+    for (const accbpg_dopt* rec : recs)
+        if (rec && rec->val_valid && rec->val_x == x_dev) return 1;
+    return 0;
 }
 
 extern "C" int accbpg_dopt_value_reuse_stats(accbpg_dopt* h, int64_t* compares_host, int64_t* answered_host) {
diff --git a/accbpg_and_fw_amd/csrc/dopt_kernels.hip b/accbpg_and_fw_amd/csrc/dopt_kernels.hip
--- a/accbpg_and_fw_amd/csrc/dopt_kernels.hip
+++ b/accbpg_and_fw_amd/csrc/dopt_kernels.hip
@@ -2581,11 +2581,11 @@
     return h->chol_tiles_ok && !h->chol_tiles_off && (h->chol_dbg & 63) == 0;
 }
 
-static int launch_chol_tiles(accbpg_dopt* h, const double* src, double* A, double* Winv) {
+static int launch_chol_tiles(accbpg_dopt* h, const double* src, double* A, double* Winv, double* dscal, int* dflag) {
     const int64_t m = h->m;
     const int T = (int)((m + NB - 1) / NB);
     CholInst ci;
-    ci.src = src; ci.L = A; ci.Ldiag = h->Tbuf; ci.Winv = Winv; ci.logdet = h->dscal; ci.flags = h->dflag;
+    ci.src = src; ci.L = A; ci.Ldiag = h->Tbuf; ci.Winv = Winv; ci.logdet = dscal; ci.flags = dflag;
     ci.ready = h->chol_ready; ci.aux = h->chol_aux; ci.hand = h->chol_hand; ci.trace = h->chol_trace;
     const int dev = (h->device >= 0 && h->device < 64) ? h->device : 0;
     std::lock_guard<std::mutex> lk(g_tiles_mu);
@@ -2615,17 +2615,20 @@
     return ACCBPG_OK;
 }
 
-int launch_cholesky(accbpg_dopt* h, double* A, double* Winv, const double* xcheck, const double* src, double* xkeep) {
+int launch_cholesky(accbpg_dopt* h, double* A, double* Winv, const double* xcheck, const double* src, double* xkeep,
+                    double* status) {
     const int64_t m = h->m;
+    double* const dscal = status ? status : h->dscal;
+    int* const dflag = status ? reinterpret_cast<int*>(status + 16) : h->dflag;
     const int T = (int)((m + NB - 1) / NB);
     if (src == nullptr) src = A;
     const bool tiles = chol_tiles_usable(h);
     prof_begin(h, PROF_CHOL);
-    zero_scalars_kernel<<<1, (xcheck || tiles) ? 512 : 64, 0, h->stream>>>(h->dscal, h->dflag, xcheck, h->n,
+    zero_scalars_kernel<<<1, (xcheck || tiles) ? 512 : 64, 0, h->stream>>>(dscal, dflag, xcheck, h->n,
                                                                          tiles ? h->chol_ready : nullptr, tiles ? T * T + 5 * T : 0,
                                                                          xcheck ? xkeep : nullptr);
     if (tiles) {
-        ACC_TRY(launch_chol_tiles(h, src, A, Winv));
+        ACC_TRY(launch_chol_tiles(h, src, A, Winv, dscal, dflag));
         h->diag_inv_ready = (Winv != nullptr);
         prof_end(h, PROF_CHOL);
         return ACCBPG_OK;
@@ -2641,7 +2644,7 @@
             int nupd = 0;
             if (pend) nupd = (kend >= T - 1) ? R * (R + 1) / 2 : R * (kend - kc);
             chol_step_kernel<<<npanel + nupd, NTHREADS, CHOL_LDS_BYTES, h->stream>>>(
-                A, m, m, kc, pend, kend, T, h->dscal, h->dflag, h->chol_dbg, Winv, h->Tbuf);
+                A, m, m, kc, pend, kend, T, dscal, dflag, h->chol_dbg, Winv, h->Tbuf);
         }
         const int Rr = T - (kend + 1);
         if (Rr > 0)
diff --git a/accbpg_and_fw_amd/csrc/internal.h b/accbpg_and_fw_amd/csrc/internal.h
--- a/accbpg_and_fw_amd/csrc/internal.h
+++ b/accbpg_and_fw_amd/csrc/internal.h
@@ -265,6 +265,8 @@
     double val_answer = 0.0;
     int val_gen = 0;
     int64_t val_compares = 0, val_answered = 0;
+    double* trial_stat = nullptr;
+    double* trial_pin = nullptr;
     accbpg_dopt* val_peer = nullptr;
     std::vector<accbpg_dopt*> val_linked;
     bool prof_on = false;
@@ -315,7 +317,8 @@
 int launch_cholesky(accbpg_dopt* h, double* A , double* Winv = nullptr ,
                     const double* xcheck = nullptr ,
                     const double* src = nullptr ,
-                    double* xkeep = nullptr );
+                    double* xkeep = nullptr ,
+                    double* status = nullptr );
 bool chol_tiles_usable(const accbpg_dopt* h);
 int launch_trtri(accbpg_dopt* h);
 int launch_colnorm(accbpg_dopt* h, const double* W, double* out, double sign);
@@ -333,6 +336,11 @@
 
 int64_t vec_ws_doubles(int64_t n);
 int vec_scratch(double** pin, int** flags, double** out);
+int trial_prox_enqueue(const double* y_dev, const double* g_dev, double L, double eps, int64_t n, double* x_out_dev,
+                       double* ws_dev, int* flags8, int gave_up_idx, hipStream_t s, bool* multi);
+void trial_prox_gave_up();
+int trial_ls_terms_enqueue(const double* g_dev, const double* x_dev, const double* y_dev, const double* z_dev,
+                           const double* z1_dev, int64_t n, double* ws_dev, double* out4_dev, hipStream_t s);
 
 int vt_nsplit(int64_t m, int64_t n, int num_cu);
 int launch_vt_times(const double* V, int64_t ldv, int64_t m, int64_t n, const double* q, double* upart, int nsplit,
diff --git a/accbpg_and_fw_amd/csrc/trial_verdict.h b/accbpg_and_fw_amd/csrc/trial_verdict.h
--- /dev/null
+++ b/accbpg_and_fw_amd/csrc/trial_verdict.h
@@ -0,0 +1,54 @@
+#pragma once
+#include <stdint.h>
+
+namespace accbpg {
+
+constexpr int TRIAL_EVAL_DOUBLES = 20;
+constexpr int TRIAL_GRAD = 0;
+constexpr int TRIAL_VALUE = 20;
+constexpr int TRIAL_LS = 40;
+constexpr int TRIAL_PROX = 44;
+constexpr int TRIAL_CMP = 48;
+constexpr int TRIAL_DOUBLES = 49;
+
+constexpr int TRIAL_FLAG_NOT_PD = 0;
+constexpr int TRIAL_FLAG_NEG_X = 1;
+constexpr int TRIAL_FLAG_NONPOS = 2;
+constexpr int TRIAL_FLAG_ABORT = 4;
+constexpr int TRIAL_PROX_INFO = 4;
+constexpr int TRIAL_PROX_GAVE_UP = 6;
+
+struct TrialAsked {
+    int cmp_stamp;
+    int prox_multi;
+};
+
+struct TrialVerdict {
+    int replay;
+    int fk_answered;
+    int chol_gave_up;
+    int prox_gave_up;
+};
+
+inline const int* trial_flags(const double* blk, int eval) {
+    return reinterpret_cast<const int*>(blk + eval + 16);
+}
+
+inline TrialVerdict trial_verdict(const double* blk, TrialAsked asked) {
+    TrialVerdict v = {0, 0, 0, 0};
+    const int* fg = trial_flags(blk, TRIAL_GRAD);
+    const int* fv = trial_flags(blk, TRIAL_VALUE);
+    const int* px = reinterpret_cast<const int*>(blk + TRIAL_PROX);
+    const int* cmp = reinterpret_cast<const int*>(blk + TRIAL_CMP);
+    v.chol_gave_up = (fg[TRIAL_FLAG_ABORT] != 0) || (fv[TRIAL_FLAG_ABORT] != 0);
+    v.prox_gave_up = asked.prox_multi && px[TRIAL_PROX_GAVE_UP] != 0;
+    bool bad = v.chol_gave_up || v.prox_gave_up;
+    bad = bad || fg[TRIAL_FLAG_NEG_X] || fg[TRIAL_FLAG_NOT_PD] || fv[TRIAL_FLAG_NEG_X] || fv[TRIAL_FLAG_NOT_PD];
+    bad = bad || px[TRIAL_FLAG_NONPOS];
+    bad = bad || !(blk[TRIAL_LS + 3] > 0.0);
+    v.replay = bad ? 1 : 0;
+    v.fk_answered = (!bad && asked.cmp_stamp != 0 && cmp[0] != asked.cmp_stamp) ? 1 : 0;
+    return v;
+}
+
+}
diff --git a/accbpg_and_fw_amd/csrc/vec_kernels.hip b/accbpg_and_fw_amd/csrc/vec_kernels.hip
--- a/accbpg_and_fw_amd/csrc/vec_kernels.hip
+++ b/accbpg_and_fw_amd/csrc/vec_kernels.hip
@@ -531,11 +531,12 @@
 
 extern "C" int64_t accbpg_vec_workspace_doubles(int64_t n) { return vec_ws_doubles(n); }
 
-extern "C" int accbpg_burg_simplex_div_prox(const double* y_dev, const double* g_dev, double L, double eps,
-                                            int64_t n, double* x_out_dev, double* ws_dev, int* info_host,
-                                            void* stream) {
-    if (!g_dev || !x_out_dev || n <= 0 || !ws_dev) return ACCBPG_ERR_ARG;
-    if (!(L > 0.0)) return ACCBPG_ERR_ASSERT;
+namespace accbpg {
+struct ProxPlan {
+    bool multi, wide;
+    int forced, G;
+};
+static int prox_plan(int64_t n, ProxPlan* p) {
     const int forced = g_prox_variant.load(std::memory_order_relaxed);
     bool multi, wide;
     if (forced == 2 || forced == 3) { multi = true; wide = forced == 3; }
@@ -550,26 +551,87 @@
         set_last_error("accbpg_burg_simplex_div_prox: the forced multi-workgroup form needs more than 128 workgroups");
         return ACCBPG_ERR_ARG;
     }
+    p->multi = multi; p->wide = wide; p->forced = forced; p->G = (int)G64;
+    return ACCBPG_OK;
+}
+static int prox_enqueue_multi(const ProxPlan& p, const double* y_dev, const double* g_dev, double L, double eps, int64_t n,
+                              double* x_out_dev, double* ws_dev, int* flags, int* gave_up, hipStream_t s,
+                              int** gave_up_at) {
+    const int G = p.G;
+    int* g_info = flags + 4;
+    ProxMultiShared shm;
+    shm.part = ws_dev;
+    shm.epoch = reinterpret_cast<int*>(ws_dev + 4 * G);
+    shm.abortw = gave_up ? gave_up : shm.epoch + G;
+    ACC_HIP(hipMemsetAsync(ws_dev, 0, sizeof(double) * 4 * G + sizeof(int) * (G + 4), s));
+    ACC_HIP(hipMemsetAsync(flags, 0, 8 * sizeof(int), s));
+    if (p.wide)
+        burg_prox_multi_kernel<32><<<G, PB, 0, s>>>(y_dev, g_dev, L, eps, n, x_out_dev, shm, G, g_info, flags, 20000000LL);
+    else
+        burg_prox_multi_kernel<8><<<G, PB, 0, s>>>(y_dev, g_dev, L, eps, n, x_out_dev, shm, G, g_info, flags, 20000000LL);
+    ACC_HIP(hipGetLastError());
+    g_prox_last[0] = p.wide ? 3 : 2; g_prox_last[1] = G;
+    if (gave_up_at) *gave_up_at = shm.abortw;
+    return ACCBPG_OK;
+}
+static int prox_enqueue_single(int forced, const double* y_dev, const double* g_dev, double L, double eps, int64_t n,
+                               double* x_out_dev, double* ws_dev, int* flags, hipStream_t s) {
+    int* g_info = flags + 4;
+    int ran;
+    if (forced != 1 && n <= (int64_t)PB * 2) {
+        burg_prox_kernel<2><<<1, PB, 0, s>>>(y_dev, g_dev, L, eps, n, x_out_dev, ws_dev, g_info, flags);
+        ran = 10;
+    } else if (forced != 1 && n <= (int64_t)PB * 8) {
+        burg_prox_kernel<8><<<1, PB, 0, s>>>(y_dev, g_dev, L, eps, n, x_out_dev, ws_dev, g_info, flags);
+        ran = 11;
+    } else if (forced != 1 && n <= (int64_t)PB * 32) {
+        burg_prox_kernel<32><<<1, PB, 0, s>>>(y_dev, g_dev, L, eps, n, x_out_dev, ws_dev, g_info, flags);
+        ran = 12;
+    } else {
+        burg_prox_kernel<0><<<1, PB, 0, s>>>(y_dev, g_dev, L, eps, n, x_out_dev, ws_dev, g_info, flags);
+        ran = 1;
+    }
+    g_prox_last[0] = ran; g_prox_last[1] = 1;
+    ACC_HIP(hipGetLastError());
+    return ACCBPG_OK;
+}
+
+int trial_prox_enqueue(const double* y_dev, const double* g_dev, double L, double eps, int64_t n, double* x_out_dev,
+                       double* ws_dev, int* flags8, int gave_up_idx, hipStream_t s, bool* multi) {
+    ProxPlan p;
+    ACC_TRY(prox_plan(n, &p));
+    *multi = p.multi;
+    if (p.multi)
+        return prox_enqueue_multi(p, y_dev, g_dev, L, eps, n, x_out_dev, ws_dev, flags8, flags8 + gave_up_idx, s, nullptr);
+    return prox_enqueue_single(p.forced, y_dev, g_dev, L, eps, n, x_out_dev, ws_dev, flags8, s);
+}
+void trial_prox_gave_up() { g_prox_multi_off = true; }
+int trial_ls_terms_enqueue(const double* g_dev, const double* x_dev, const double* y_dev, const double* z_dev,
+                           const double* z1_dev, int64_t n, double* ws_dev, double* out4_dev, hipStream_t s) {
+    const int nb = red_blocks(n, RMAXBLK);
+    double* part = ws_dev + n;
+    ls_terms_partial_kernel<<<nb, RB, 0, s>>>(g_dev, x_dev, y_dev, z_dev, z1_dev, n, 1, part);
+    ls_terms_final_kernel<<<1, RB, 0, s>>>(part, nb, out4_dev);
+    ACC_HIP(hipGetLastError());
+    return ACCBPG_OK;
+}
+}
+
+extern "C" int accbpg_burg_simplex_div_prox(const double* y_dev, const double* g_dev, double L, double eps,
+                                            int64_t n, double* x_out_dev, double* ws_dev, int* info_host,
+                                            void* stream) {
+    if (!g_dev || !x_out_dev || n <= 0 || !ws_dev) return ACCBPG_ERR_ARG;
+    if (!(L > 0.0)) return ACCBPG_ERR_ASSERT;
+    ProxPlan p;
+    ACC_TRY(prox_plan(n, &p));
     ACC_TRY(ensure_scratch());
     hipStream_t s = (hipStream_t)stream;
-    int* g_info = g_flags + 4;
-    if (multi) {
-        const int G = (int)G64;
-        ProxMultiShared shm;
-        shm.part = ws_dev;
-        shm.epoch = reinterpret_cast<int*>(ws_dev + 4 * G);
-        shm.abortw = shm.epoch + G;
-        ACC_HIP(hipMemsetAsync(ws_dev, 0, sizeof(double) * 4 * G + sizeof(int) * (G + 4), s));
-        ACC_HIP(hipMemsetAsync(g_flags, 0, 8 * sizeof(int), s));
-        if (wide)
-            burg_prox_multi_kernel<32><<<G, PB, 0, s>>>(y_dev, g_dev, L, eps, n, x_out_dev, shm, G, g_info, g_flags, 20000000LL);
-        else
-            burg_prox_multi_kernel<8><<<G, PB, 0, s>>>(y_dev, g_dev, L, eps, n, x_out_dev, shm, G, g_info, g_flags, 20000000LL);
-        ACC_HIP(hipGetLastError());
-        g_prox_last[0] = wide ? 3 : 2; g_prox_last[1] = G;
+    if (p.multi) {
+        int* gave_up = nullptr;
+        ACC_TRY(prox_enqueue_multi(p, y_dev, g_dev, L, eps, n, x_out_dev, ws_dev, g_flags, nullptr, s, &gave_up));
         int* pin_m = reinterpret_cast<int*>(g_pin);
         ACC_HIP(hipMemcpyAsync(pin_m, g_flags, 6 * sizeof(int), hipMemcpyDeviceToHost, s));
-        ACC_HIP(hipMemcpyAsync(pin_m + 8, shm.abortw, sizeof(int), hipMemcpyDeviceToHost, s));
+        ACC_HIP(hipMemcpyAsync(pin_m + 8, gave_up, sizeof(int), hipMemcpyDeviceToHost, s));
         ACC_HIP(hipStreamSynchronize(s));
         if (pin_m[8] == 0) {
             if (info_host) { info_host[0] = pin_m[4]; info_host[1] = pin_m[5]; }
@@ -578,22 +640,7 @@
         }
         g_prox_multi_off = true;
     }
-    int ran;
-    if (forced != 1 && n <= (int64_t)PB * 2) {
-        burg_prox_kernel<2><<<1, PB, 0, s>>>(y_dev, g_dev, L, eps, n, x_out_dev, ws_dev, g_info, g_flags);
-        ran = 10;
-    } else if (forced != 1 && n <= (int64_t)PB * 8) {
-        burg_prox_kernel<8><<<1, PB, 0, s>>>(y_dev, g_dev, L, eps, n, x_out_dev, ws_dev, g_info, g_flags);
-        ran = 11;
-    } else if (forced != 1 && n <= (int64_t)PB * 32) {
-        burg_prox_kernel<32><<<1, PB, 0, s>>>(y_dev, g_dev, L, eps, n, x_out_dev, ws_dev, g_info, g_flags);
-        ran = 12;
-    } else {
-        burg_prox_kernel<0><<<1, PB, 0, s>>>(y_dev, g_dev, L, eps, n, x_out_dev, ws_dev, g_info, g_flags);
-        ran = 1;
-    }
-    g_prox_last[0] = ran; g_prox_last[1] = 1;
-    ACC_HIP(hipGetLastError());
+    ACC_TRY(prox_enqueue_single(p.forced, y_dev, g_dev, L, eps, n, x_out_dev, ws_dev, g_flags, s));
     int* pin_i = reinterpret_cast<int*>(g_pin);
     ACC_HIP(hipMemcpyAsync(pin_i, g_flags, 6 * sizeof(int), hipMemcpyDeviceToHost, s));
     ACC_HIP(hipStreamSynchronize(s));
diff --git a/accbpg_and_fw_amd/functions.py b/accbpg_and_fw_amd/functions.py
--- a/accbpg_and_fw_amd/functions.py
+++ b/accbpg_and_fw_amd/functions.py
@@ -89,6 +89,7 @@
         self.n = H.shape[1]
         assert _shard or self.m < self.n, "DOptimalObj: need m < n"
         self._V, _ = to_dev(H)
+        self._is_shard = bool(_shard)
         lib = _lib.load()
         if _borrowed is not None:
             h, self._owner = _borrowed
@@ -115,6 +116,8 @@
         self.gram_combos = 0
         self.value_hits = 0
         self._reuse = True
+        self._one_wait = True
+        self.one_wait_trials_run = 0
 
     def __del__(self):
         for name in ("_h", "_h2"):
@@ -173,6 +176,36 @@
             self._lib.accbpg_dopt_value_reuse_stats(h, C.byref(cmp_), C.byref(ans))
             total += ans.value
         return total
+
+    def one_wait_trials(self, enable=True):
+        self._one_wait = bool(enable)
+        return self
+
+    def _one_wait_ok(self):
+        if "func_grad" in self.__dict__ or type(self).func_grad is not DOptimalObj.func_grad:
+            return False
+        return self._one_wait and self._owned and not self._is_shard and not (self._lin or self._spec or getattr(self, "_memo_on", False))
+
+    def value_recorded(self, x):
+        return bool(self._lib.accbpg_dopt_value_recorded(self._h, _ptr(x)))
+
+    def trial(self, x_prev, z_prev, theta, L, eps, want_fk):
+        dev = self._V.device
+        y, g, z, x = (torch.empty(self.n, dtype=torch.float64, device=dev) for _ in range(4))
+        out = _lib.TrialOut()
+        with torch.cuda.device(dev):
+            self._lib.accbpg_dopt_set_stream(self._h, _stream())
+            rc = self._lib.accbpg_dopt_burg_trial(self._h, _ptr(x_prev), _ptr(z_prev), float(theta), float(L),
+                                                  float(eps), 1 if want_fk else 0, _ptr(y), _ptr(g), _ptr(z), _ptr(x),
+                                                  _ptr(_Workspace.get(self.n, dev)), C.byref(out))
+        self.one_wait_trials_run += 1
+        if rc == _lib.TRIAL_REPLAY:
+            return None
+        _lib.check(rc, "accbpg_dopt_burg_trial")
+        self.calls["grad"] += 1
+        if out.fk_answered:
+            self.calls["value"] += 1
+        return y, g, z, x, out
 
     def _memo_get(self, x):
         memo = getattr(self, "_memo", None)
diff --git a/include/accbpg_hip.h b/include/accbpg_hip.h
--- a/include/accbpg_hip.h
+++ b/include/accbpg_hip.h
@@ -34,6 +34,7 @@
 
 int accbpg_dopt_value_reuse(accbpg_dopt* h, int on);
 int accbpg_dopt_value_reuse_stats(accbpg_dopt* h, int64_t* compares_host, int64_t* answered_host);
+int accbpg_dopt_value_recorded(accbpg_dopt* h, const double* x_dev);
 int accbpg_dopt_value_peer(accbpg_dopt* h, accbpg_dopt* peer);
 
 int accbpg_dopt_gram(accbpg_dopt* h, const double* x_dev, double* gram_dev);
@@ -102,6 +103,20 @@
 
 int accbpg_vec_axpby(double a, const double* x_dev, double b, const double* z_dev, int64_t n,
                      double* out_dev, void* stream);
+
+#define ACCBPG_TRIAL_REPLAY 5
+typedef struct accbpg_trial_out {
+    double fy;
+    double lin, dxy, dzz;
+    double fx;
+    double fk;
+    int32_t prox_info[2];
+    int32_t fk_answered;
+    int32_t reserved;
+} accbpg_trial_out;
+int accbpg_dopt_burg_trial(accbpg_dopt* h, const double* x_prev_dev, const double* z_prev_dev, double theta, double L,
+                           double eps, int want_fk, double* y_dev, double* g_dev, double* z_dev, double* x_dev,
+                           double* ws_dev, accbpg_trial_out* out_host);
 
 int accbpg_vec_dot_diff(const double* g_dev, const double* x_dev, const double* y_dev, int64_t n,
                         double* out_host, double* ws_dev, void* stream);
```

New measurement: 64.52 iterations/s (median of 6 runs). +1.3%, better.
